# norabelrose/sparse-vae

Hardware: AMD Instinct MI355X
Metric: training tokens/sec + ELBO match vs CPU ref, 512-tok seq, 1/2/4/8 MI355X (higher is better)
Workload: dtype bf16; 1 GPU; c2: TransformerVAE 6L d512 heads 8 seq 512, batch 64/GPU, dense attention, dropout 0.1, fwd+bwd+allreduce+clip+RAdam; model=TransformerVAE-6L-d512, global_batch=64, seq_len=512, parallelism=dp1

## Files before the change

### include/svae.h

```cpp
#ifndef SVAE_H
#define SVAE_H
#include <stdint.h>
#ifdef __cplusplus
extern "C" {
#endif

typedef void* svae_stream_t;

enum svae_epi {
  SVAE_EPI_BF16 = 0,
  SVAE_EPI_F32 = 1,
  SVAE_EPI_F32_ACC = 2,
  SVAE_EPI_F32_ATOMIC = 3,
  SVAE_EPI_GELU = 4,
  SVAE_EPI_GELU_BWD = 5,
  SVAE_EPI_DROPOUT_RESID = 6,
  SVAE_EPI_ROTARY_BF16 = 7,
  SVAE_EPI_CE_STATS = 8,
  SVAE_EPI_CE_PROB = 9,
  SVAE_EPI_ROWSCALE_GATHER = 10
};

typedef struct svae_gemm_desc {
  const void* A;
  const void* B;
  int64_t lda, ldb, batch_stride_a, batch_stride_b;
  int32_t M, N, K;
  int32_t batch, splits;
  int32_t a_t, b_t;
  int32_t epi;
  void* C;
  int64_t ldc, batch_stride_c;
  const float* bias;
  const float* resid;
  int64_t ldr;
  void* aux;
  int64_t ldaux;
  float alpha;
  float drop_p;
  uint64_t seed;
  const float* rot_tab;
  int32_t rot_cols, rot_d, rot_seq;
  const int32_t* labels;
  float* label_logit;
  float* a_rowsum;
  const float* k_weight;
  const float* row_a;
  const float* row_b;
  const void* gather;
  int64_t ldg;
  float* delta;
  const float* delta_o32;
  int64_t ld_o32;
  int32_t delta_hd, delta_seq;
} svae_gemm_desc;

int svae_gemm(const svae_gemm_desc* d, svae_stream_t stream);

int svae_gemm_pair(const svae_gemm_desc* d0, const svae_gemm_desc* d1, svae_stream_t stream);

int svae_resid_ln_fwd(const float* x, const void* y, int32_t y_dtype, int64_t ldy, float drop_p, uint64_t seed,
                      const float* zrows, int32_t zmod, const float* w, const float* b, float* xo, void* h, float* mean,
                      float* rstd, int32_t rows, int32_t D, svae_stream_t stream);
int svae_layernorm_fwd(const void* x, int32_t x_dtype, const float* w, const float* b, void* y,
                       float* mean, float* rstd, int32_t rows, int32_t D, svae_stream_t stream);
int svae_layernorm_bwd(const void* dy, const void* x, int32_t x_dtype, const float* w, const float* mean,
                       const float* rstd, const float* dres, float* dx, void* dx_bf, float* part,
                       int32_t nblk, int32_t rows, int32_t D, int32_t zero_mod, svae_stream_t stream);
int svae_layernorm_bwd_drop(const void* dy, const void* x, int32_t x_dtype, const float* w, const float* mean,
                            const float* rstd, const float* dres, float* dx, void* dx_bf, float* part, int32_t nblk,
                            int32_t rows, int32_t D, int32_t zero_mod, float bf_drop_p, uint64_t bf_seed,
                            int32_t bf_zero_mod, float* zrow, void* zrow_bf, svae_stream_t stream);
int svae_layernorm_bwd_gelu(const void* dy, const void* x, int32_t x_dtype, const float* w, const float* mean,
                            const float* rstd, const void* gp, void* out_bf, float* part, int32_t nblk, int32_t rows,
                            int32_t D, svae_stream_t stream);
int svae_layernorm_fwd_z(float* x, const float* zrows, int32_t zmod, const float* w, const float* b, void* y,
                         float* mean, float* rstd, int32_t rows, int32_t D, svae_stream_t stream);
int svae_layernorm_nblk(int32_t rows);
#define SVAE_LN_MULTI_MAX 4
int svae_layernorm_fwd_multi(const float* x, const float* const* w, const float* const* b, void* const* y, int32_t n,
                             float* mean, float* rstd, int32_t rows, int32_t D, svae_stream_t stream);
int svae_layernorm_bwd_multi(const void* const* dy, const float* x, const float* const* w, const float* mean,
                             const float* rstd, const float* dres, float* dx, float* const* part, int32_t nblk,
                             int32_t n, int32_t rows, int32_t D, svae_stream_t stream);

int svae_colsum(const void* in, int32_t in_dtype, int32_t rows, int32_t cols, int64_t ld, float* out,
                int32_t accumulate, svae_stream_t stream);

#define SVAE_COLSUM_MAX 8
typedef struct svae_colsum_seg {
  const float* in;
  float* out;
  int64_t ld;
  int32_t rows, cols;
} svae_colsum_seg;
int svae_colsum_multi(const svae_colsum_seg* segs, int32_t n, svae_stream_t stream);

typedef struct svae_attn_desc {
  const void* q; const void* k; const void* v; void* o;
  int64_t sq, sk, sv, so, bq, bk, bv, bo;
  const uint8_t* key_pad;
  float* lse;
  int32_t B, H, Lq, Lk, hd, causal;
  float scale;
  const void* dout; int64_t sdo, bdo;
  float* delta;
  float* dq;
  int64_t bdq;
  void* dk; void* dv;
  int64_t sdk, sdv, bdk, bdv;
  const float* rot_tab;
  int32_t rot_d;
  float* o32;
  int64_t so32, bo32;
  float* dq_part;
  void* dq_bf;
  int64_t ldq_bf;
  int32_t window;
  int32_t delta_ready;
  void* o_lo;
  int64_t so_lo, bo_lo;
  float* fwd_ws;
  int64_t fwd_ws_elems;
} svae_attn_desc;

int svae_attn_fwd(const svae_attn_desc* d, svae_stream_t stream);
int64_t svae_attn_fwd_ws_elems(int32_t B, int32_t H, int32_t Lq, int32_t Lk, int32_t hd, int32_t causal, int32_t window);
int svae_attn_bwd(const svae_attn_desc* d, svae_stream_t stream);
int64_t svae_attn_dq_part_elems(int32_t B, int32_t H, int32_t Lq, int32_t Lk, int32_t hd);
int64_t svae_attn_dq_part_elems_w(int32_t B, int32_t H, int32_t Lq, int32_t Lk, int32_t hd, int32_t window);
int svae_dq_finalize(const float* dq, void* out, int64_t ldo, int32_t rows, int32_t D, const float* rot_tab,
                     int32_t seq, svae_stream_t stream);

int svae_embedding_fwd(const int32_t* ids, const void* table_bf, float* out, void* out_bf, int32_t rows,
                       int32_t D, svae_stream_t stream);
int svae_embedding_fwd_dual(const int32_t* ids, const void* table, float* out, float* out2, int32_t rows, int32_t D,
                            svae_stream_t stream);
int svae_embedding_bwd(const int32_t* ids, const float* dout, float* dtable, int32_t rows, int32_t D,
                       svae_stream_t stream);

int svae_reparam_kl_fwd(const float* stats, const float* eps, uint64_t seed, const int64_t* ntok,
                        float* z, void* z_bf, float* eps_out, float* raw_kl, float* kl_out, int32_t B,
                        int32_t Z, svae_stream_t stream);
int svae_reparam_kl_bwd(const float* stats, const float* eps, const float* dz, const int64_t* ntok,
                        const float* gkl, float* dstats, int32_t B, int32_t Z, svae_stream_t stream);

int svae_ce_finalize(const float* part, int32_t ntile, const float* label_logit, const int32_t* labels,
                     int32_t rows, int32_t seq, int32_t nchunks, int32_t chunk_len, float* lse, float* row_loss,
                     float* chunk_w, float* nll_out, float* red_ws, svae_stream_t stream);
int svae_ce_weighted_nll(const float* row_loss, const int32_t* labels, const float* tok_w, int32_t rows,
                         int32_t seq, int32_t nchunks, int32_t chunk_len, float* out, float* red_ws,
                         svae_stream_t stream);
int32_t svae_ce_red_ws_elems(int32_t nchunks);
int svae_ce_grad(void* logits, int64_t ld, const float* lse, const float* chunk_w, const int32_t* labels,
                 const float* gscale, float* dbias, int32_t rows, int32_t V, int32_t seq, int32_t nchunks,
                 int32_t chunk_len, svae_stream_t stream);

int svae_ce_label_logit(const void* hh, int64_t ldh, const void* W, int64_t ldw, const float* bias,
                        const int32_t* labels, int32_t rows, int32_t D, float* out, svae_stream_t stream);
int svae_ce_prob_finalize(const float* part, int32_t ntile, const float* row_off, const int32_t* labels,
                          int32_t rows, int32_t seq, int32_t nchunks, int32_t chunk_len, float* lse, float* row_loss,
                          float* chunk_w, float* nll_out, float* red_ws, svae_stream_t stream);
int svae_ce_prob_finalize_fix(const float* part, int32_t ntile, float* row_off, const int32_t* labels, int32_t rows,
                              int32_t seq, int32_t nchunks, int32_t chunk_len, float* lse, float* row_loss,
                              float* chunk_w, float* nll_out, float* red_ws, const void* hh, int64_t ldh, const void* W,
                              int64_t ldw, const float* bias, void* P, int64_t ldp, int32_t V, int32_t D,
                              int32_t* sat_ws, svae_stream_t stream);
int svae_ce_prob_bwd_prep(const void* hh, int64_t ldh, const float* lse, const float* row_off, const float* chunk_w,
                          const int32_t* labels, const float* gscale, int32_t rows, int32_t seq, int32_t nchunks,
                          int32_t chunk_len, int32_t D, void* hh_out, float* r_out, float* q_out, float* dbias,
                          svae_stream_t stream);
int svae_embedding_bwd_ce(const int32_t* ids, const float* dout, float* dtable, int32_t rows, int32_t D, int32_t seq,
                          const void* hh, const float* q, svae_stream_t stream);

int svae_dropout_bwd_cast(const float* g, void* out, float p, uint64_t seed, int64_t n, int32_t cols,
                          int64_t ld_in, svae_stream_t stream);
int svae_gelu_bwd(const float* dx, const void* gp, void* out, int64_t n, svae_stream_t stream);
int svae_prep_tokens(const int64_t* ids, const void* pad, int32_t pad_mode, int32_t B, int32_t L, int32_t* ids32,
                     int32_t* labels, void* padm, const int64_t* ntok, int64_t* ntok_out, svae_stream_t stream);
int svae_step_scalars(const float* nll, const float* kl, const float* gloss, float kl_weight, float* loss, float* gs,
                      svae_stream_t stream);
int svae_cast_bf16(const float* in, void* out, int64_t n, svae_stream_t stream);
int svae_transpose_blocks(const void* src, void* dst, const int64_t* table, int32_t nblocks, int32_t total_tiles,
                          svae_stream_t stream);
int svae_extract_rows(float* x, int64_t ld, int32_t rows, int32_t mod, int32_t D, float* out,
                      svae_stream_t stream);
int svae_zproj_bwd(const float* g, const void* z, const void* W, float* dW, float* db, float* dz, int32_t B,
                   int32_t d, int32_t Z, svae_stream_t stream);
#define SVAE_ZPROJ_MAX 32
typedef struct svae_zproj_seg {
  const float* g;
  const void* W;
  float* dW;
  float* db;
} svae_zproj_seg;
int svae_zproj_bwd_multi(const svae_zproj_seg* segs, int32_t n, const void* z, float* dz, int32_t B, int32_t d,
                         int32_t Z, svae_stream_t stream);
typedef struct svae_zproj_fwd_seg {
  const void* W;
  const float* bias;
  float* out;
} svae_zproj_fwd_seg;
int svae_zproj_fwd_multi(const svae_zproj_fwd_seg* segs, int32_t n, const void* z, int32_t B, int32_t d, int32_t Z,
                         svae_stream_t stream);

int svae_sumsq(const float* g, int64_t n, float* part, int32_t nblk, svae_stream_t stream);
int svae_radam(float* p, void* pbf, const float* g, float* m, float* v, int64_t n, const float* part,
               int32_t nblk, const float* scal, float* norm_out, svae_stream_t stream);
int svae_clip_grad(float* g, int64_t n, const float* part, int32_t nblk, float max_norm, float* norm_out,
                   svae_stream_t stream);

int svae_gemm_f32(const float* A, const float* W, float* C, int32_t M, int32_t N, int32_t K, int64_t lda, int64_t ldw,
                  int64_t ldc, const float* bias, const float* resid, int64_t ldr, int32_t epi, const float* rot_tab,
                  int32_t rot_cols, int32_t rot_d, int32_t rot_seq, svae_stream_t stream);
int svae_attn_fwd_f32(const float* q, const float* k, const float* v, float* o, int64_t sq, int64_t sk, int64_t sv,
                      int64_t so, int64_t bq, int64_t bk, int64_t bv, int64_t bo, const uint8_t* key_pad, int32_t B,
                      int32_t H, int32_t Lq, int32_t Lk, int32_t hd, int32_t causal, int32_t window, float scale,
                      svae_stream_t stream);
int svae_layernorm_fwd_f32(const float* x, const float* w, const float* b, float* y, int32_t rows, int32_t D,
                           svae_stream_t stream);

int svae_mutual_info(const float* stats, const float* eps, uint64_t seed, const float* kl, int32_t B, int32_t Z,
                     int32_t S, float* ws, float* out, svae_stream_t stream);

int svae_ce_seq_logprob(const float* part, int32_t ntile, const float* label_logit, const int32_t* labels,
                        int32_t rows, int32_t seq, float* out, svae_stream_t stream);

int svae_dec_linear(const float* X, int64_t ldx, const float* W, int64_t ldw, const float* bias, float* Y, int64_t ldy,
                    const float* resid, int64_t ldr, int32_t M, int32_t N, int32_t K, int32_t epi, const float* rot_tab,
                    int32_t rot_cols, int32_t rot_d, const int32_t* cur, float* part_ws, int64_t part_elems,
                    svae_stream_t stream);
int svae_dec_attn(const float* qkv, int64_t ldq, float* kcache, float* vcache, int32_t B, int32_t H, int32_t hd,
                  int32_t T, const int32_t* cur, int32_t window, float scale, float* O, int64_t ldo,
                  svae_stream_t stream);
int svae_dec_embed(const int64_t* out_ids, int32_t T, const int32_t* cur, const float* table, float* x, int32_t B,
                   int32_t D, svae_stream_t stream);
int svae_dec_penalty(float* logits, int64_t ldl, int32_t rows, const int32_t* row_map, const int64_t* out_ids,
                     int32_t T, const int32_t* cur, const uint8_t* live, float penalty, svae_stream_t stream);
int svae_dec_sample(const float* logits, int64_t ldl, int32_t V, int32_t rows, const int32_t* row_map,
                    int64_t* out_ids, int32_t T, const int32_t* cur, uint8_t* live, int32_t end_token,
                    float temperature, int32_t top_k, float top_p, uint64_t seed, int32_t* live_count,
                    svae_stream_t stream);
int svae_dec_advance(int32_t* cur, svae_stream_t stream);

enum svae_latent_metric { SVAE_LATENT_L2 = 0, SVAE_LATENT_COSINE = 1, SVAE_LATENT_KL = 2 };
#define SVAE_LATENT_MAX_BLOCKS 1024
int svae_latent_prepare(const float* mu, const float* scale, float* inv_var, float* logdet, float* inv_norm, int32_t N,
                        int32_t Z, svae_stream_t stream);
int svae_latent_scores(int32_t metric, const float* q_mu, const float* q_scale, const float* q_logdet,
                       const float* q_inv_norm, int32_t Q, const float* mu, const float* inv_var, const float* logdet,
                       const float* inv_norm, int32_t N, int32_t Z, float* out, svae_stream_t stream);
int64_t svae_latent_topk_ws_bytes(int32_t Q, int32_t k);
int svae_latent_topk(int32_t metric, const float* q_mu, const float* q_scale, const float* q_logdet,
                     const float* q_inv_norm, int32_t Q, const float* mu, const float* inv_var, const float* logdet,
                     const float* inv_norm, int32_t N, int32_t Z, int32_t k, void* ws, int64_t ws_bytes, float* scores,
                     int32_t* indices, svae_stream_t stream);

const char* svae_version(void);

#ifdef __cplusplus
}
#endif
#endif
```

### sparse-vae_amd/csrc/gemm.hip

```cpp
#include "common.h"
#include "../../include/svae.h"
#include <stdlib.h>
#include <algorithm>

using namespace svae;

namespace {

constexpr int BM = 128, BN = 128, BK = 64;
constexpr int TILE_BYTES = BM * BK * 2;

struct GP {
  const bf16* A; const bf16* B;
  long long lda, ldb, sA, sB;
  int M, N, K, splits, kchunk, tiles_n, tiles_m;
  void* C; long long ldc, sC;
  const float* bias;
  const float* resid; long long ldr;
  void* aux; long long ldaux;
  float alpha, drop_p;
  unsigned long long seed;
  const float* rot_tab; int rot_cols, rot_d, rot_seq;
  const int* labels; float* label_logit;
  float* a_rowsum;
  const float* k_weight;
  const float* row_a; const float* row_b;
  const bf16* gather; long long ldg;
  int epi;
  int tn2, tm2;
  int group;
  int total3;
  int relaxed;
  int dma_stagger;
  long long slab;
  float* delta; const float* delta_o32; long long ld_o32; int delta_hd, delta_seq;
};

__device__ __forceinline__ int kc_off(int row, int c) { return row * 128 + ((c ^ ((row >> 1) & 7)) << 4); }
__device__ __forceinline__ int mn_off(int k, int u) {
  const int s = (k & 3) | (((k >> 3) & 1) << 2);
  return k * 256 + ((u ^ (s << 2)) << 3);
}

template <bool TRANS>
__device__ __forceinline__ void load_tile(const bf16* __restrict__ g, long long ld, int row0, int nrows, int k0,
                                          int kend, u32x4 (&r)[4], int tid) {
  const bf16* base = TRANS ? g + (long long)k0 * ld + row0 : g + (long long)row0 * ld + k0;
  const __amdgpu_buffer_rsrc_t rsrc = __builtin_amdgcn_make_buffer_rsrc((void*)base, 0, 0x7FFFFFF0, 0x00020000);
#pragma unroll
  for (int i = 0; i < 4; ++i) {
    const int idx = tid + 256 * i;
    int row, k;
    if (!TRANS) { row = idx >> 3; k = (idx & 7) * 8; }
    else { k = idx >> 4; row = (idx & 15) * 8; }
    const bool ok = (row0 + row < nrows) && (k0 + k < kend);
    const int off = TRANS ? (k * (int)ld + row) * 2 : (row * (int)ld + k) * 2;
    r[i] = __builtin_bit_cast(u32x4, __builtin_amdgcn_raw_buffer_load_b128(rsrc, ok ? off : 0x7FFFFFF0, 0, 0));
  }
}

template <bool TRANS>
__device__ __forceinline__ void store_tile(char* lds, const u32x4 (&r)[4], int tid) {
#pragma unroll
  for (int i = 0; i < 4; ++i) {
    const int idx = tid + 256 * i;
    int off;
    if (!TRANS) off = kc_off(idx >> 3, idx & 7);
    else off = mn_off(idx >> 4, (idx & 15) * 2);
    *(u32x4*)(lds + off) = r[i];
  }
}

template <bool TRANS>
__device__ __forceinline__ bf16x8 read_frag(const char* lds, int base, int kk, int lane) {
  if (!TRANS) {
    const int row = base + (lane & 15);
    const int c = (lane >> 4) + 4 * kk;
    return *(const bf16x8*)(lds + kc_off(row, c));
  } else {
    const int q = (lane & 15) >> 2, p = lane & 3;
    const int kb = 32 * kk + 8 * (lane >> 4) + q;
    const int u = (base >> 2) + p;
    short4v lo = lds_read_tr(lds + mn_off(kb, u));
    short4v hi = lds_read_tr(lds + mn_off(kb + 4, u));
    return cat44(lo, hi);
  }
}

__device__ __forceinline__ int cs_swz(int row, int col) { return (((col >> 2) ^ (((row >> 2) & 3) << 2)) << 2) | (col & 3); }
__device__ __forceinline__ int cs_swz8(int row, int col) { return (((col >> 2) ^ (row & 7)) << 2) | (col & 3); }
template <bool SW8>
__device__ __forceinline__ int cs_at(int row, int col) { return SW8 ? cs_swz8(row, col) : cs_swz(row, col); }

__device__ __forceinline__ void group_tile(int t, int tiles_m, int tiles_n, int group, int& bm, int& bn) {
  if (group <= 1) {
    bn = t % tiles_n;
    bm = t / tiles_n;
    return;
  }
  const int per = group * tiles_n, grp = t / per, first = grp * group;
  const int gs = min(group, tiles_m - first), r = t - grp * per;
  bm = first + r % gs;
  bn = r / gs;
}

__device__ __forceinline__ void tile_coords(const GP& p, int& bm, int& bn, int& batch, int& split) {
  const int tiles = p.tiles_n * p.tiles_m;
  const int nwg = gridDim.x;
  int bid = blockIdx.x;
  if (nwg >= 16) {
    const int q = nwg / 8, r = nwg % 8, xcd = bid % 8, idx = bid / 8;
    bid = (xcd < r ? xcd * (q + 1) : r * (q + 1) + (xcd - r) * q) + idx;
  }
  const int z = bid / tiles, t = bid - z * tiles;
  group_tile(t, p.tiles_m, p.tiles_n, p.group, bm, bn);
  batch = z / p.splits;
  split = z - batch * p.splits;
}

__device__ __forceinline__ void store_bf16(bf16* dst, const f32x4& a, const f32x4& b, bool full) {
  if (full)
    *(bf16x8*)dst = (bf16x8){f2bf(a[0]), f2bf(a[1]), f2bf(a[2]), f2bf(a[3]), f2bf(b[0]), f2bf(b[1]), f2bf(b[2]), f2bf(b[3])};
  else
    *(bf16x4*)dst = (bf16x4){f2bf(a[0]), f2bf(a[1]), f2bf(a[2]), f2bf(a[3])};
}

__device__ __forceinline__ void rotary4(const GP& p, f32x4& x, int m, int n) {
  if (n >= p.rot_cols) return;
  const int pos = m % p.rot_seq;
  const int pair = (n % p.rot_d) >> 1;
  const f32x4 cs2 = *(const f32x4*)(p.rot_tab + ((long long)pos * (p.rot_d >> 1) + pair) * 2);
  const float a0 = x[0], b0 = x[1], a1 = x[2], b1 = x[3];
  x[0] = a0 * cs2[0] + (-b0) * cs2[1];
  x[1] = b0 * cs2[0] + a0 * cs2[1];
  x[2] = a1 * cs2[2] + (-b1) * cs2[3];
  x[3] = b1 * cs2[2] + a1 * cs2[3];
}

__device__ __forceinline__ void dropout4(const GP& p, f32x4& x, int m, int n) {
  const float sc = 1.0f / (1.0f - p.drop_p);
  float u[4];
  rand_uniform4(p.seed, ((unsigned long long)m * p.N + n) >> 2, u);
#pragma unroll
  for (int e = 0; e < 4; ++e) x[e] = (u[e] >= p.drop_p) ? x[e] * sc : 0.f;
}

template <int EPI, bool BIAS_DONE = false, bool SW8 = false>
__device__ __forceinline__ void epilogue_half(const GP& p, const float* cs, int m0, int n0, int bn, int rbase,
                                              long long cofs, int tid, int label_pre = -1) {
  if constexpr (EPI == SVAE_EPI_F32_ATOMIC) {
    const int col = tid & 127, n = n0 + col;
    if (n < p.N) {
      for (int it = 0; it < 32; ++it) {
        const int row = (tid >> 7) + 2 * it, m = m0 + rbase + row;
        if (m < p.M) atomicAdd((float*)p.C + cofs + (long long)m * p.ldc + n, cs[row * 128 + cs_at<SW8>(row, col)]);
      }
    }
    return;
  }
  const int cc = (tid & 15) * 8, n = n0 + cc;
  const bool ncol = n < p.N, full = n + 8 <= p.N;
  const f32x4 zero = {0.f, 0.f, 0.f, 0.f};
  f32x4 b0 = zero, b1 = zero;
  if (!BIAS_DONE && p.bias && ncol) {
    b0 = *(const f32x4*)(p.bias + n);
    if (full) b1 = *(const f32x4*)(p.bias + n + 4);
  }
  if constexpr (EPI == SVAE_EPI_CE_STATS) {
    const int row = tid >> 2, qd = tid & 3, m = m0 + rbase + row;
    float v[32];
    float mx = -INFINITY;
#pragma unroll
    for (int u = 0; u < 4; ++u) {
      const int c = 32 * u + 8 * qd;
      f32x4 x0 = *(const f32x4*)(cs + row * 128 + cs_at<SW8>(row, c));
      f32x4 x1 = *(const f32x4*)(cs + row * 128 + cs_at<SW8>(row, c + 4));
      if (!BIAS_DONE && p.bias) {
        x0 += (n0 + c < p.N) ? *(const f32x4*)(p.bias + n0 + c) : zero;
        x1 += (n0 + c + 4 < p.N) ? *(const f32x4*)(p.bias + n0 + c + 4) : zero;
      }
      if (p.C && m < p.M && n0 + c < p.N)
        store_bf16((bf16*)p.C + cofs + (long long)m * p.ldc + n0 + c, x0, x1, n0 + c + 8 <= p.N);
#pragma unroll
      for (int e = 0; e < 4; ++e) {
        const float y0 = (n0 + c + e < p.N) ? x0[e] : -INFINITY;
        const float y1 = (n0 + c + 4 + e < p.N) ? x1[e] : -INFINITY;
        v[8 * u + e] = y0;
        v[8 * u + 4 + e] = y1;
        mx = fmaxf(mx, fmaxf(y0, y1));
      }
    }
    mx = fmaxf(mx, __shfl_xor(mx, 1, 64));
    mx = fmaxf(mx, __shfl_xor(mx, 2, 64));
    float se = 0.f;
#pragma unroll
    for (int e = 0; e < 32; ++e) se += __expf(v[e] - mx);
    se += __shfl_xor(se, 1, 64);
    se += __shfl_xor(se, 2, 64);
    if (m < p.M) {
      const int lc = (BIAS_DONE ? label_pre : p.labels[m]) - n0;
      if (lc >= 0 && lc < 128 && ((lc >> 3) & 3) == qd) {
        const int idx = 8 * (lc >> 5) + (lc & 7);
#pragma unroll
        for (int e = 0; e < 32; ++e)
          if (e == idx) p.label_logit[m] = v[e];
      }
      if (qd == 0) {
        float* part = (float*)p.aux + ((long long)m * p.tiles_n + bn) * 2;
        part[0] = mx;
        part[1] = se;
      }
    }
    return;
  }
  if (!ncol) return;
#pragma unroll
  for (int it = 0; it < 4; ++it) {
    const int row = (tid >> 4) + 16 * it, m = m0 + rbase + row;
    if (m >= p.M) break;
    f32x4 x0 = *(const f32x4*)(cs + row * 128 + cs_at<SW8>(row, cc));
    f32x4 x1 = full ? *(const f32x4*)(cs + row * 128 + cs_at<SW8>(row, cc + 4)) : zero;
    const long long ci = cofs + (long long)m * p.ldc + n;
    if constexpr (EPI == SVAE_EPI_BF16) {
      store_bf16((bf16*)p.C + ci, x0 + b0, x1 + b1, full);
    } else if constexpr (EPI == SVAE_EPI_ROTARY_BF16) {
      x0 += b0;
      x1 += b1;
      rotary4(p, x0, m, n);
      if (full) rotary4(p, x1, m, n + 4);
      store_bf16((bf16*)p.C + ci, x0, x1, full);
    } else if constexpr (EPI == SVAE_EPI_F32 || EPI == SVAE_EPI_F32_ACC || EPI == SVAE_EPI_DROPOUT_RESID) {
      float* c = (float*)p.C + ci;
      if constexpr (EPI == SVAE_EPI_F32) {
        x0 += b0;
        x1 += b1;
        if (p.resid) {
          const float* r = p.resid + (long long)m * p.ldr + n;
          x0 += *(const f32x4*)r;
          if (full) x1 += *(const f32x4*)(r + 4);
        }
      } else if constexpr (EPI == SVAE_EPI_F32_ACC) {
        x0 += *(const f32x4*)c;
        if (full) x1 += *(const f32x4*)(c + 4);
      } else {
        if (p.drop_p > 0.f) {
          dropout4(p, x0, m, n);
          if (full) dropout4(p, x1, m, n + 4);
        }
        const float* r = p.resid + (long long)m * p.ldr + n;
        x0 += *(const f32x4*)r;
        if (full) x1 += *(const f32x4*)(r + 4);
      }
      *(f32x4*)c = x0;
      if (full) *(f32x4*)(c + 4) = x1;
      if constexpr (EPI == SVAE_EPI_DROPOUT_RESID) {
        if (p.aux) store_bf16((bf16*)p.aux + (long long)m * p.ldaux + n, x0, x1, full);
      } else if constexpr (EPI == SVAE_EPI_F32) {
        if (p.aux) {
          if (p.drop_p > 0.f) {
            dropout4(p, x0, m, n);
            if (full) dropout4(p, x1, m, n + 4);
          }
          store_bf16((bf16*)p.aux + (long long)m * p.ldaux + n, x0, x1, full);
        }
      }
    } else if constexpr (EPI == SVAE_EPI_GELU) {
      x0 += b0;
      x1 += b1;
      f32x4 g0, g1, d0, d1;
#pragma unroll
      for (int e = 0; e < 4; ++e) {
        float g, dg;
        gelu_pair(x0[e], g, dg);
        g0[e] = g;
        d0[e] = dg;
        gelu_pair(x1[e], g, dg);
        g1[e] = g;
        d1[e] = dg;
      }
      store_bf16((bf16*)p.C + ci, g0, g1, full);
      store_bf16((bf16*)p.aux + (long long)m * p.ldaux + n, d0, d1, full);
    } else if constexpr (EPI == SVAE_EPI_GELU_BWD) {
      const bf16* a = (const bf16*)p.aux + (long long)m * p.ldaux + n;
      bf16x8 d;
      if (full) d = *(const bf16x8*)a;
      else {
        const bf16x4 h = *(const bf16x4*)a;
        d = (bf16x8){h[0], h[1], h[2], h[3], h[0], h[1], h[2], h[3]};
      }
#pragma unroll
      for (int e = 0; e < 4; ++e) {
        x0[e] *= (float)d[e];
        x1[e] *= (float)d[e + 4];
      }
      store_bf16((bf16*)p.C + ci, x0, x1, full);
    }
  }
}

template <bool AT, bool BT, int EPI>
__global__ __launch_bounds__(256, 2) void gemm_kernel(GP p) {
  __shared__ __attribute__((aligned(16))) char smem[4 * TILE_BYTES];
  const int tid = threadIdx.x, lane = tid & 63, wave = tid >> 6;
  const int wm = wave >> 1, wn = wave & 1;

  int bm, bn, batch, split;
// ... 477 lines not shown
      se = sum_x16_x32(se);
      if (g == 0) {
        sstat[(rl * 4 + wc) * 2] = mx;
        sstat[(rl * 4 + wc) * 2 + 1] = se;
      }
      const int lc = slabel[rl] - (n0 + wc * 64);
      if (m < p.M && lc >= 0 && lc < 64 && ((lc >> 2) & 3) == g) {
        float x = 0.f;
#pragma unroll
        for (int j = 0; j < 4; ++j)
#pragma unroll
          for (int e = 0; e < 4; ++e)
            if (j == (lc >> 4) && e == (lc & 3)) x = v[j][e];
        p.label_logit[m] = x;
      }
    }
  }
  if constexpr (EPI == SVAE_EPI_CE_STATS) {
    asm volatile("s_waitcnt lgkmcnt(0)" ::: "memory");
    __builtin_amdgcn_s_barrier();
    const int row = tid >> 1, hf = tid & 1, m = m0 + row;
    if (m < p.M && n0 + 128 * hf < p.N) {
      const float* s = sstat + (row * 4 + 2 * hf) * 2;
      const float m1 = s[0], s1 = s[1], m2 = s[2], s2 = s[3];
      const float mm = fmaxf(m1, m2);
      const float e1 = m1 == -INFINITY ? 0.f : __builtin_amdgcn_exp2f((m1 - mm) * G3_LOG2E);
      const float e2 = m2 == -INFINITY ? 0.f : __builtin_amdgcn_exp2f((m2 - mm) * G3_LOG2E);
      float* part = (float*)p.aux + ((long long)m * p.tiles_n + bn * 2 + hf) * 2;
      part[0] = mm;
      part[1] = s1 * e1 + s2 * e2;
    }
  }
  if constexpr (EPI == SVAE_EPI_CE_PROB) {
    asm volatile("s_waitcnt lgkmcnt(0)" ::: "memory");
    __builtin_amdgcn_s_barrier();
    const int row = tid & 255, hf = tid >> 8, m = m0 + row;
    if (m < p.M && n0 + 128 * hf < p.N)
      ((float*)p.aux)[(long long)(bn * 2 + hf) * p.M + m] = sstat[row * 4 + 2 * hf] + sstat[row * 4 + 2 * hf + 1];
  }
}

__device__ __forceinline__ void g3_rowscale_gather_epilogue(const GP& p, const f32x4 (&acc)[8][4], const int* slabel,
                                                            const float* sra, const float* srb, int m0, int n0, int wr,
                                                            int wc, int lane) {
  const int g = lane >> 4, li = lane & 15;
  const int nb = n0 + wc * 64;
  const int cs = ((g & 1) ? 16 : 0) + ((g & 2) ? 8 : 0);
  auto ld_row = [&](int i, u32x4 (&r)[2]) {
    const int rl = wr * 128 + i * 16 + li, m = m0 + rl, lab = slabel[rl];
    const bool on = m < p.M && lab != 0 && srb[rl] != 0.f;
#pragma unroll
    for (int jp = 0; jp < 2; ++jp) {
      const int n = nb + 32 * jp + cs;
      r[jp] = (on && n + 8 <= p.N) ? *(const u32x4*)(p.gather + (long long)lab * p.ldg + n) : (u32x4){0u, 0u, 0u, 0u};
    }
  };
  u32x4 cur[2], nxt[2];
  ld_row(0, cur);
#pragma unroll
  for (int i = 0; i < 8; ++i) {
    if (i + 1 < 8) ld_row(i + 1, nxt);
    const int rl = wr * 128 + i * 16 + li, m = m0 + rl;
    const float ra = sra[rl] * p.alpha, rb = srb[rl];
#pragma unroll
    for (int jp = 0; jp < 2; ++jp) {
      const f32x4 x = acc[i][2 * jp], y = acc[i][2 * jp + 1];
      float w[8];
#pragma unroll
      for (int e = 0; e < 4; ++e) {
        const auto sw = __builtin_amdgcn_permlane16_swap(__float_as_uint(x[e]), __float_as_uint(y[e]), false, false);
        w[e] = __uint_as_float(sw[0]);
        w[4 + e] = __uint_as_float(sw[1]);
      }
      const bf16x8 gv = __builtin_bit_cast(bf16x8, cur[jp]);
      const u32x4 o = {pack_bf16x2(ra * w[0] - rb * (float)gv[0], ra * w[1] - rb * (float)gv[1]),
                       pack_bf16x2(ra * w[2] - rb * (float)gv[2], ra * w[3] - rb * (float)gv[3]),
                       pack_bf16x2(ra * w[4] - rb * (float)gv[4], ra * w[5] - rb * (float)gv[5]),
                       pack_bf16x2(ra * w[6] - rb * (float)gv[6], ra * w[7] - rb * (float)gv[7])};
      const int n = nb + 32 * jp + cs;
      if (m < p.M && n + 8 <= p.N) *(u32x4*)((bf16*)p.C + (long long)m * p.ldc + n) = o;
      else if (m < p.M && n < p.N) *(u32x2*)((bf16*)p.C + (long long)m * p.ldc + n) = (u32x2){o[0], o[1]};
    }
    if (i + 1 < 8) {
      cur[0] = nxt[0];
      cur[1] = nxt[1];
    }
  }
}

template <int EPI>
__device__ __forceinline__ void g3_reg_epilogue_ld(const GP& p, const f32x4 (&acc)[8][4], const float* sbias, int m0,
                                                   int n0, int batch, int split, int wr, int wc, int lane) {
  const long long cofs = (long long)batch * p.sC + split * p.slab;
  const int g = lane >> 4, li = lane & 15;
  const int nb = n0 + wc * 64;
  f32x4 b4[4];
#pragma unroll
  for (int j = 0; j < 4; ++j) b4[j] = *(const f32x4*)(sbias + wc * 64 + j * 16 + 4 * g);
  if constexpr (EPI == G3_EPI_BF16_DELTA) {
    const int H = p.N / p.delta_hd;
    const int hA = nb / p.delta_hd;
    auto ld_row = [&](int i, f32x4 (&r)[4]) {
      const int m = m0 + wr * 128 + i * 16 + li;
#pragma unroll
      for (int j = 0; j < 4; ++j) {
        const int n = nb + j * 16 + 4 * g;
        r[j] = (m < p.M && n < p.N) ? *(const f32x4*)(p.delta_o32 + (long long)m * p.ld_o32 + n)
                                    : (f32x4){0.f, 0.f, 0.f, 0.f};
      }
    };
    f32x4 cur[4], nxt[4];
    ld_row(0, cur);
#pragma unroll
    for (int i = 0; i < 8; ++i) {
      if (i + 1 < 8) ld_row(i + 1, nxt);
      const int m = m0 + wr * 128 + i * 16 + li;
      f32x4 x[4];
      float sA = 0.f, sB = 0.f;
#pragma unroll
      for (int j = 0; j < 4; ++j) {
        x[j] = p.alpha * acc[i][j] + b4[j];
        float dj = 0.f;
#pragma unroll
        for (int e = 0; e < 4; ++e) dj = fmaf((float)f2bf(x[j][e]), cur[j][e], dj);
        if ((nb + 16 * j) / p.delta_hd == hA) sA += dj;
        else sB += dj;
      }
      store_rows_bf16<false>((bf16*)p.C + cofs, p.ldc, m0 + wr * 128 + i * 16, p.M, nb, p.N, x, g, li);
      sA = sum_x16_x32(sA);
      sB = sum_x16_x32(sB);
      if (g == 0 && m < p.M && nb < p.N) {
        const int b = m / p.delta_seq, q = m - b * p.delta_seq;
        atomicAdd(p.delta + ((long long)b * H + hA) * p.delta_seq + q, sA);
        if ((nb + 63) / p.delta_hd != hA && hA + 1 < H) atomicAdd(p.delta + ((long long)b * H + hA + 1) * p.delta_seq + q, sB);
      }
      if (i + 1 < 8) {
#pragma unroll
        for (int j = 0; j < 4; ++j) cur[j] = nxt[j];
      }
    }
    return;
  } else if constexpr (EPI == SVAE_EPI_GELU_BWD) {
    const int cs = ((g & 1) ? 16 : 0) + ((g & 2) ? 8 : 0);
    auto ld_row = [&](int i, u32x4 (&r)[2]) {
      const int m = m0 + wr * 128 + i * 16 + li;
#pragma unroll
      for (int jp = 0; jp < 2; ++jp) {
        const int n = nb + 32 * jp + cs;
        r[jp] = (m < p.M && n + 8 <= p.N) ? *(const u32x4*)((const bf16*)p.aux + (long long)m * p.ldaux + n)
                                          : (u32x4){0u, 0u, 0u, 0u};
      }
    };
    u32x4 cur[2], nxt[2];
    ld_row(0, cur);
#pragma unroll
    for (int i = 0; i < 8; ++i) {
      if (i + 1 < 8) ld_row(i + 1, nxt);
      u32x4 o[2];
#pragma unroll
      for (int jp = 0; jp < 2; ++jp) {
        const f32x4 x = p.alpha * acc[i][2 * jp] + b4[2 * jp], y = p.alpha * acc[i][2 * jp + 1] + b4[2 * jp + 1];
        float w[8];
#pragma unroll
        for (int e = 0; e < 4; ++e) {
          const auto s = __builtin_amdgcn_permlane16_swap(__float_as_uint(x[e]), __float_as_uint(y[e]), false, false);
          w[e] = __uint_as_float(s[0]);
          w[4 + e] = __uint_as_float(s[1]);
        }
        const bf16x8 a = __builtin_bit_cast(bf16x8, cur[jp]);
        o[jp] = (u32x4){pack_bf16x2(w[0] * (float)a[0], w[1] * (float)a[1]), pack_bf16x2(w[2] * (float)a[2], w[3] * (float)a[3]),
                        pack_bf16x2(w[4] * (float)a[4], w[5] * (float)a[5]), pack_bf16x2(w[6] * (float)a[6], w[7] * (float)a[7])};
      }
      store_rows_w16<false>((bf16*)p.C + cofs, p.ldc, m0 + wr * 128 + i * 16, p.M, nb, p.N, o, g, li);
      if (i + 1 < 8) {
        cur[0] = nxt[0];
        cur[1] = nxt[1];
      }
    }
    return;
  } else {
    const float* src = EPI == SVAE_EPI_F32_ACC ? (const float*)p.C + cofs : p.resid;
    const long long lds_ = EPI == SVAE_EPI_F32_ACC ? p.ldc : p.ldr;
    const bool ld = EPI != G3_EPI_SLAB && src != nullptr;
    auto ld_row = [&](int i, f32x4 (&r)[4]) {
      const int m = m0 + wr * 128 + i * 16 + li;
#pragma unroll
      for (int j = 0; j < 4; ++j) {
        const int n = nb + j * 16 + 4 * g;
        r[j] = (ld && m < p.M && n < p.N) ? *(const f32x4*)(src + (long long)m * lds_ + n) : (f32x4){0.f, 0.f, 0.f, 0.f};
      }
    };
    f32x4 cur[4], nxt[4];
    if constexpr (EPI != G3_EPI_SLAB) ld_row(0, cur);
#pragma unroll
    for (int i = 0; i < 8; ++i) {
      if (EPI != G3_EPI_SLAB && i + 1 < 8) ld_row(i + 1, nxt);
      const int m = m0 + wr * 128 + i * 16 + li;
      f32x4 x[4];
#pragma unroll
      for (int j = 0; j < 4; ++j) {
        const int n = nb + j * 16 + 4 * g;
        x[j] = p.alpha * acc[i][j] + b4[j];
        if constexpr (EPI == SVAE_EPI_DROPOUT_RESID) {
          if (p.drop_p > 0.f) dropout4(p, x[j], m, n);
        }
        if constexpr (EPI != G3_EPI_SLAB) x[j] += cur[j];
      }
      if constexpr (EPI == SVAE_EPI_F32_ACC) {
#pragma unroll
        for (int j = 0; j < 4; ++j) {
          const int n = nb + j * 16 + 4 * g;
          if (m < p.M && n < p.N) *(f32x4*)((float*)p.C + cofs + (long long)m * p.ldc + n) = x[j];
        }
      } else {
        store_rows_f32((float*)p.C + cofs, p.ldc, m0 + wr * 128 + i * 16, p.M, nb, p.N, x, g, li);
        if constexpr (EPI == SVAE_EPI_DROPOUT_RESID) {
          if (p.aux) store_rows_bf16<false>((bf16*)p.aux, p.ldaux, m0 + wr * 128 + i * 16, p.M, nb, p.N, x, g, li);
        } else if constexpr (EPI == SVAE_EPI_F32) {
          if (p.aux) {
            if (p.drop_p > 0.f) {
#pragma unroll
              for (int j = 0; j < 4; ++j) dropout4(p, x[j], m, nb + j * 16 + 4 * g);
            }
            store_rows_bf16<false>((bf16*)p.aux, p.ldaux, m0 + wr * 128 + i * 16, p.M, nb, p.N, x, g, li);
          }
        }
      }
      if (EPI != G3_EPI_SLAB && i + 1 < 8) {
#pragma unroll
        for (int j = 0; j < 4; ++j) cur[j] = nxt[j];
      }
    }
  }
}

struct G3Tile {
  int m0, n0, bn, batch, split, kbeg, kend, nk;
  const bf16* A; const bf16* B;
};

__device__ __forceinline__ G3Tile g3_tile(const GP& p, int t3) {
  G3Tile T;
  const int tiles = p.tn2 * p.tm2;
  const int z = t3 / tiles, t = t3 - z * tiles;
  T.batch = z / p.splits;
  T.split = z - T.batch * p.splits;
  int bm, bn;
  group_tile(t, p.tm2, p.tn2, p.group, bm, bn);
  T.bn = bn;
  T.m0 = bm * 256;
  T.n0 = bn * 256;
  T.kbeg = T.split * p.kchunk;
  T.kend = min(p.K, T.kbeg + p.kchunk);
  T.nk = T.kend > T.kbeg ? (T.kend - T.kbeg + 63) / 64 : 0;
  T.A = p.A + T.batch * p.sA;
  T.B = p.B + T.batch * p.sB;
  return T;
}

constexpr int G3_EPI_STORES = 16;

#ifdef SVAE_STAMPS
__device__ unsigned long long svae_stamps[8][96][3];
__device__ unsigned long long svae_rt[1024][2];
#define G3_STAMP(k) \
  do { if (blockIdx.x < 8 && tid == 0 && ntile < 96) svae_stamps[blockIdx.x][ntile][k] = __builtin_amdgcn_s_memtime(); } while (0)
#else
#define G3_STAMP(k) ((void)0)
#endif
#ifndef SVAE_KW_FORM
#define SVAE_KW_FORM 0
#endif
#ifndef SVAE_KW_PRE
#define SVAE_KW_PRE 1
#endif

template <int EPI>
constexpr int g3_epi_vmem_ops() {
  switch (EPI) {
    case SVAE_EPI_BF16:
    case G3_EPI_BF16_DELTA:
    case SVAE_EPI_ROTARY_BF16:
    case SVAE_EPI_CE_STATS:
    case SVAE_EPI_ROWSCALE_GATHER:
    case SVAE_EPI_GELU_BWD:
      return 8 * 2;
    case SVAE_EPI_CE_PROB:
      return 8 * 2 + 1;
    case SVAE_EPI_GELU:
      return 8 * 2 * 2;
    case SVAE_EPI_F32:
    case SVAE_EPI_F32_ACC:
    case SVAE_EPI_DROPOUT_RESID:
    case G3_EPI_ACC_KW:
    case G3_EPI_F32_KW:
    case G3_EPI_SLAB:
      return 8 * 4;
    default:
      return 0;
  }
}

template <bool AT, bool BT, int EPI>
__device__ __forceinline__ void gemm256_run(const GP& p, int blk, int nwg) {
  static_assert(g3_epi_vmem_ops<EPI>() >= G3_EPI_STORES, "the relaxed first wait would not cover the prefetch DMA");
  constexpr bool IS_KW = EPI == G3_EPI_ACC_KW || EPI == G3_EPI_F32_KW;
  constexpr int KW_FORM = IS_KW ? SVAE_KW_FORM : 0;
  constexpr int KW_SLOT = KW_FORM == 2 ? 1024 : 256;
  constexpr int KW_BYTES = KW_FORM ? 2 * 8 * KW_SLOT : 0;
  constexpr int RING_OFF = KW_FORM == 3 ? KW_BYTES : 0;
  constexpr int KW_OFF = KW_FORM == 3 ? 0 : 2 * G3_STAGE + 2048 + 8192;
  __shared__ __attribute__((aligned(16))) char smem[2 * G3_STAGE + 2048 + 8192 + KW_BYTES];
  char* ring = smem + RING_OFF;
  float* sbias = (float*)(ring + 2 * G3_STAGE);
  int* slabel = (int*)(ring + 2 * G3_STAGE + 1024);
  float* sstat = (float*)(ring + 2 * G3_STAGE + 2048);
  const int tid = threadIdx.x, lane = tid & 63;
  const int wave = __builtin_amdgcn_readfirstlane(tid >> 6);
  const int wr = wave >> 2, wc = wave & 3;
  int bid = blk;
  if (nwg >= 16) {
    const int q = nwg / 8, r = nwg % 8, xcd = bid % 8, idx = bid / 8;
    bid = (xcd < r ? xcd * (q + 1) : r * (q + 1) + (xcd - r) * q) + idx;
  }
  int t3 = bid;
  if (t3 >= p.total3) return;
  G3Tile T = g3_tile(p, t3);
  char* skw = smem + KW_OFF;
  auto kw_issue = [&](int k0, int kend, int stage) {
    if constexpr (KW_FORM == 1 || KW_FORM == 3) {
      const u32x4 kwr = buffer_rsrc(p.k_weight, 0x7FFFFFF0u);
      const int kk = k0 + lane_id_fresh();
      dma4_lds(kwr, skw + (stage * 8 + wave) * KW_SLOT, kk < kend ? kk * 4 : 0x7FFFFFF0);
    } else if constexpr (KW_FORM == 2) {
      const u32x4 kwr = buffer_rsrc(p.k_weight, 0x7FFFFFF0u);
      const int l = lane_id_fresh(), kk = k0 + 4 * l;
      dma16_lds(kwr, skw + (stage * 8 + wave) * KW_SLOT, l < 16 && kk < kend ? kk * 4 : 0x7FFFFFF0);
    }
  };
  const G3Src sa = g3_src<AT>(p.lda, wave, lane), sb = g3_src<BT>(p.ldb, wave, lane);
  int g = 0;
  if (T.nk > 0) {
    g3_issue<AT, BT>(p, T.A, T.B, sa, sb, T.m0, T.n0, T.kbeg, T.kend, ring, wave);
    kw_issue(T.kbeg, T.kend, 0);
  }

  bool relaxed = false;
  int ntile = 0;
  (void)ntile;
  while (true) {
    G3_STAMP(0);
    const int t3n = t3 + nwg;
    const bool has_next = t3n < p.total3;
    float rsum[4] = {0.f, 0.f, 0.f, 0.f};
    f32x4 acc[8][4];
#pragma unroll
    for (int i = 0; i < 8; ++i)
#pragma unroll
      for (int j = 0; j < 4; ++j) acc[i][j] = (f32x4){0.f, 0.f, 0.f, 0.f};

    const bool next_dma = has_next && g3_tile(p, t3n).nk > 0;
    for (int kt = 0; kt < T.nk; ++kt, ++g) {
      if (kt == 0 && relaxed) asm volatile("s_waitcnt vmcnt(%0)" ::"n"(G3_EPI_STORES) : "memory");
      else asm volatile("s_waitcnt vmcnt(0)" ::: "memory");
      __builtin_amdgcn_s_barrier();
      const char* la = ring + (g & 1) * G3_STAGE;
      const char* lb = la + G3_T;
      char* nxt = ring + ((g + 1) & 1) * G3_STAGE;
      const bool do_rs = AT && p.a_rowsum && T.bn < 2;
      const int ks0 = p.tn2 >= 2 ? T.bn : 0, ks1 = p.tn2 >= 2 ? T.bn + 1 : 2;
      const bool kw_pre = IS_KW && KW_FORM == 0 && SVAE_KW_PRE && do_rs;
      float kw1 = 0.f;
      if (kw_pre) {
        const int kk = T.kbeg + kt * 64 + lane_id_fresh();
        const int off = kk < T.kend ? kk * 4 : 0x7FFFFFF0;
        const u32x4 kwr = buffer_rsrc(p.k_weight, 0x7FFFFFF0u);
        asm volatile("s_nop 4\n\tbuffer_load_dword %0, %1, %2, 0 offen" : "=&v"(kw1) : "v"(off), "s"(kwr) : "memory");
      }
      const bool late = (!IS_KW || KW_FORM > 0 || kw_pre) && p.dma_stagger && wr == 1 && kt + 1 < T.nk;
      if (kt + 1 < T.nk) {
        if (!late) g3_issue<AT, BT>(p, T.A, T.B, sa, sb, T.m0, T.n0, T.kbeg + (kt + 1) * 64, T.kend, nxt, wave);
        kw_issue(T.kbeg + (kt + 1) * 64, T.kend, (g + 1) & 1);
      } else if (next_dma) {
        const G3Tile TN = g3_tile(p, t3n);
        g3_issue<AT, BT>(p, TN.A, TN.B, sa, sb, TN.m0, TN.n0, TN.kbeg, TN.kend, nxt, wave);
        kw_issue(TN.kbeg, TN.kend, (g + 1) & 1);
      } else if (kw_pre) {
        const u32x4 rs = buffer_rsrc(p.A, 0x7FFFFFF0u);
#pragma unroll
        for (int i = 0; i < 8; ++i) dma16_lds(rs, nxt + (wave * 8 + i) * 1024, 0x7FFFFFF0);
      }
      bf16x8 a0[4][2], a1[4][2], b0[2][2], b1[2][2];
      auto rowsum2 = [&](const bf16x8 (&x)[2], const bf16x8 (&y)[2]) {
#pragma unroll
        for (int ks = 0; ks < 2; ++ks) {
          if (ks < ks0 || ks >= ks1) continue;
          f32x4 k0 = {1.f, 1.f, 1.f, 1.f}, k1 = k0;
          if constexpr (KW_FORM > 0) {
            const float* kws = (const float*)(skw + ((g & 1) * 8 + wave) * KW_SLOT) + 32 * ks + 8 * (lane >> 4);
            k0 = *(const f32x4*)kws;
            k1 = *(const f32x4*)(kws + 4);
          } else if constexpr (IS_KW) {
            if (kw_pre) {
              const int src0 = (32 * ks + 8 * (lane_id_fresh() >> 4)) * 4;
#pragma unroll
              for (int e = 0; e < 4; ++e) {
                k0[e] = __builtin_bit_cast(float, __builtin_amdgcn_ds_bpermute(src0 + 4 * e, __builtin_bit_cast(int, kw1)));
                k1[e] = __builtin_bit_cast(float, __builtin_amdgcn_ds_bpermute(src0 + 16 + 4 * e, __builtin_bit_cast(int, kw1)));
              }
            } else {
              const int kk = T.kbeg + kt * 64 + 32 * ks + 8 * (lane_id_fresh() >> 4);
              const int off = kk < T.kend ? kk * 4 : 0x7FFFFFF0;
              const u32x4 kwr = buffer_rsrc(p.k_weight, 0x7FFFFFF0u);
              asm volatile("s_nop 4\n\tbuffer_load_dwordx4 %0, %2, %3, 0 offen\n\t"
                           "buffer_load_dwordx4 %1, %2, %3, 0 offen offset:16\n\ts_waitcnt vmcnt(0)"
                           : "=&v"(k0), "=&v"(k1) : "v"(off), "s"(kwr) : "memory");
            }
          }
#pragma unroll
          for (int e = 0; e < 8; ++e) {
            const float kwe = e < 4 ? k0[e] : k1[e - 4];
            rsum[0] = fmaf((float)x[ks][e], kwe, rsum[0]);
            rsum[1] = fmaf((float)y[ks][e], kwe, rsum[1]);
          }
        }
      };
#pragma unroll
      for (int i = 0; i < 4; ++i)
#pragma unroll
        for (int ks = 0; ks < 2; ++ks) a0[i][ks] = g3_afrag<AT>(la, wr * 128 + i * 16, ks, lane);
#pragma unroll
      for (int j = 0; j < 2; ++j)
#pragma unroll
        for (int ks = 0; ks < 2; ++ks) b0[j][ks] = g3_bfrag<BT>(lb, wc * 64 + j * 16, ks, lane);
#pragma unroll
      for (int j = 0; j < 2; ++j)
#pragma unroll
        for (int ks = 0; ks < 2; ++ks) b1[j][ks] = g3_bfrag<BT>(lb, wc * 64 + 32 + j * 16, ks, lane);
#pragma unroll
      for (int ks = 0; ks < 2; ++ks)
#pragma unroll
        for (int i = 0; i < 4; ++i)
#pragma unroll
          for (int j = 0; j < 2; ++j) acc[i][j] = mfma16(b0[j][ks], a0[i][ks], acc[i][j]);
      if (late) {
        __builtin_amdgcn_sched_barrier(0);
        g3_issue<AT, BT>(p, T.A, T.B, sa, sb, T.m0, T.n0, T.kbeg + (kt + 1) * 64, T.kend, nxt, wave);
        __builtin_amdgcn_sched_barrier(0);
      }
      if constexpr (!AT) {
#pragma unroll
        for (int i = 0; i < 4; ++i)
#pragma unroll
          for (int ks = 0; ks < 2; ++ks) a1[i][ks] = g3_afrag<AT>(la, wr * 128 + 64 + i * 16, ks, lane);
      }
#pragma unroll
      for (int ks = 0; ks < 2; ++ks)
#pragma unroll
        for (int i = 0; i < 4; ++i)
#pragma unroll
          for (int j = 0; j < 2; ++j) acc[i][2 + j] = mfma16(b1[j][ks], a0[i][ks], acc[i][2 + j]);
      if constexpr (AT) {
        if (kw_pre) asm volatile("s_waitcnt vmcnt(8)" : "+v"(kw1) :: "memory");
        if (do_rs) {
          if (wc == 0) rowsum2(a0[0], a0[1]);
          else if (wc == 1) rowsum2(a0[2], a0[3]);
        }
#pragma unroll
        for (int i = 0; i < 4; ++i)
#pragma unroll
          for (int ks = 0; ks < 2; ++ks) a1[i][ks] = g3_afrag<AT>(la, wr * 128 + 64 + i * 16, ks, lane);
      }
#pragma unroll
      for (int ks = 0; ks < 2; ++ks)
#pragma unroll
        for (int i = 0; i < 4; ++i)
#pragma unroll
          for (int j = 0; j < 2; ++j) acc[4 + i][2 + j] = mfma16(b1[j][ks], a1[i][ks], acc[4 + i][2 + j]);
#pragma unroll
      for (int ks = 0; ks < 2; ++ks)
#pragma unroll
        for (int i = 0; i < 4; ++i)
#pragma unroll
          for (int j = 0; j < 2; ++j) acc[4 + i][j] = mfma16(b0[j][ks], a1[i][ks], acc[4 + i][j]);
      if constexpr (AT) {
        if (do_rs) {
          if (wc == 2) rowsum2(a1[0], a1[1]);
          else if (wc == 3) rowsum2(a1[2], a1[3]);
        }
      }
    }
    G3_STAMP(1);
    if (tid < 256) {
      const int n = T.n0 + tid, m = T.m0 + tid;
      sbias[tid] = (p.bias && n < p.N) ? p.bias[n] : 0.f;
      if (EPI == SVAE_EPI_CE_STATS || EPI == SVAE_EPI_CE_PROB || EPI == SVAE_EPI_ROWSCALE_GATHER)
        slabel[tid] = m < p.M ? p.labels[m] : 0;
      if (EPI == SVAE_EPI_CE_PROB) sstat[1024 + tid] = (m < p.M && p.labels[m] != 0) ? p.row_a[m] : INFINITY;
      if (EPI == SVAE_EPI_ROWSCALE_GATHER) sstat[1024 + tid] = m < p.M ? p.row_a[m] : 0.f;
      if (EPI == SVAE_EPI_ROWSCALE_GATHER) sstat[1280 + tid] = m < p.M ? p.row_b[m] : 0.f;
    }
    asm volatile("s_waitcnt lgkmcnt(0)" ::: "memory");
    __builtin_amdgcn_s_barrier();
    if constexpr (AT) {
      if (p.a_rowsum && T.bn < 2) {
#pragma unroll
        for (int h = 0; h < 2; ++h) {
          const float t = sum_x16_x32(rsum[h]);
          const int m = T.m0 + wr * 128 + (2 * wc + h) * 16 + (lane & 15);
          if ((lane >> 4) == 0 && m < p.M) atomicAdd(p.a_rowsum + m, t);
        }
      }
    }
    if constexpr (EPI == SVAE_EPI_BF16 || EPI == SVAE_EPI_GELU || EPI == SVAE_EPI_CE_STATS ||
                  EPI == SVAE_EPI_ROTARY_BF16 || EPI == SVAE_EPI_CE_PROB)
      g3_reg_epilogue<EPI>(p, acc, sbias, slabel, sstat, T.m0, T.n0, T.bn, T.batch, T.split, wr, wc, tid, lane);
    else if constexpr (EPI == SVAE_EPI_ROWSCALE_GATHER)
      g3_rowscale_gather_epilogue(p, acc, slabel, sstat + 1024, sstat + 1280, T.m0, T.n0, wr, wc, lane);
    else if constexpr (EPI == SVAE_EPI_F32 || EPI == SVAE_EPI_F32_ACC || EPI == SVAE_EPI_DROPOUT_RESID ||
                       EPI == SVAE_EPI_GELU_BWD || EPI == G3_EPI_BF16_DELTA)
      g3_reg_epilogue_ld<EPI>(p, acc, sbias, T.m0, T.n0, T.batch, T.split, wr, wc, lane);
    else if constexpr (EPI == G3_EPI_ACC_KW)
      g3_reg_epilogue_ld<SVAE_EPI_F32_ACC>(p, acc, sbias, T.m0, T.n0, T.batch, T.split, wr, wc, lane);
    else if constexpr (EPI == G3_EPI_F32_KW || EPI == G3_EPI_SLAB)
      g3_reg_epilogue_ld<G3_EPI_SLAB>(p, acc, sbias, T.m0, T.n0, T.batch, T.split, wr, wc, lane);
    else
      static_assert(EPI == G3_EPI_SLAB, "no gemm256 epilogue for this EPI");
    relaxed = p.relaxed && T.m0 + 256 <= p.M && T.n0 + 256 <= p.N;
    G3_STAMP(2);
    ++ntile;
    if (!has_next) break;
    const bool prefetched = T.nk > 0;
    t3 = t3n;
    T = g3_tile(p, t3);
    if (!prefetched && T.nk > 0) {
      g3_issue<AT, BT>(p, T.A, T.B, sa, sb, T.m0, T.n0, T.kbeg, T.kend, ring + (g & 1) * G3_STAGE, wave);
      kw_issue(T.kbeg, T.kend, g & 1);
    }
  }
}

template <bool AT, bool BT, int EPI>
__global__ __launch_bounds__(512, 1) void gemm256_kernel(GP p) {
#ifdef SVAE_STAMPS
  if (threadIdx.x == 0 && blockIdx.x < 1024) svae_rt[blockIdx.x][0] = __builtin_amdgcn_s_memrealtime();
#endif
  gemm256_run<AT, BT, EPI>(p, blockIdx.x, gridDim.x);
#ifdef SVAE_STAMPS
  if (threadIdx.x == 0 && blockIdx.x < 1024) svae_rt[blockIdx.x][1] = __builtin_amdgcn_s_memrealtime();
#endif
}

struct GP2 {
  GP p[2];
  int nb0;
};

template <bool AT, bool BT, int EPI>
__global__ __launch_bounds__(512, 1) void gemm256_pair_kernel(GP2 q) {
  const int b = blockIdx.x;
  const int sel = b < q.nb0 ? 0 : 1;
  gemm256_run<AT, BT, EPI>(q.p[sel], sel ? b - q.nb0 : b, sel ? (int)gridDim.x - q.nb0 : q.nb0);
}

constexpr int SK_BN = 32, SK_WAVES = 16;

template <int EPI>
__global__ __launch_bounds__(1024) void gemm_skinny_kernel(GP p) {
  __shared__ __attribute__((aligned(16))) float red[SK_WAVES][64][SK_BN + 4];
  const int tid = threadIdx.x, lane = tid & 63, li = lane & 15, g = lane >> 4;
  const int wave = __builtin_amdgcn_readfirstlane(tid >> 6);
  const int n0 = blockIdx.x * SK_BN;
  const int nks = (p.K + 31) / 32;
  const int per = (nks + SK_WAVES - 1) / SK_WAVES;
  const int ks0 = wave * per, ks1 = min(nks, ks0 + per);
  f32x4 acc[4][2];
#pragma unroll
  for (int i = 0; i < 4; ++i) acc[i][0] = acc[i][1] = (f32x4){0.f, 0.f, 0.f, 0.f};
  auto load = [&](int ks, bf16x8 (&a)[4], bf16x8 (&b)[2]) {
    const int k = ks * 32 + 8 * g;
    const bool kok = k < p.K;
#pragma unroll
    for (int i = 0; i < 4; ++i) {
      const int m = 16 * i + li;
      u32x4 v = {0u, 0u, 0u, 0u};
      if (kok && m < p.M) v = *(const u32x4*)(p.A + (long long)m * p.lda + k);
      a[i] = __builtin_bit_cast(bf16x8, v);
    }
#pragma unroll
    for (int jj = 0; jj < 2; ++jj) {
      const int n = n0 + 16 * jj + li;
      u32x4 v = {0u, 0u, 0u, 0u};
      if (kok && n < p.N) v = *(const u32x4*)(p.B + (long long)n * p.ldb + k);
      b[jj] = __builtin_bit_cast(bf16x8, v);
    }
  };
  if (ks0 < ks1) {
    bf16x8 a[4], b[2], an[4], bn[2];
    load(ks0, a, b);
    for (int ks = ks0; ks < ks1; ++ks) {
      if (ks + 1 < ks1) load(ks + 1, an, bn);
#pragma unroll
      for (int i = 0; i < 4; ++i)
#pragma unroll
        for (int jj = 0; jj < 2; ++jj) acc[i][jj] = mfma16(b[jj], a[i], acc[i][jj]);
      if (ks + 1 < ks1) {
#pragma unroll
        for (int i = 0; i < 4; ++i) a[i] = an[i];
        b[0] = bn[0];
        b[1] = bn[1];
      }
    }
  }
#pragma unroll
  for (int i = 0; i < 4; ++i)
#pragma unroll
    for (int jj = 0; jj < 2; ++jj) *(f32x4*)&red[wave][16 * i + li][16 * jj + 4 * g] = acc[i][jj];
  __syncthreads();
  const int row = tid >> 3, c4 = (tid & 7) * 4, m = row, n = n0 + c4;
  if (tid >= 512 || m >= p.M || n >= p.N) return;
  f32x4 x = *(const f32x4*)&red[0][row][c4];
#pragma unroll
  for (int w = 1; w < SK_WAVES; ++w) x += *(const f32x4*)&red[w][row][c4];
  x *= p.alpha;
  if (p.bias) x += *(const f32x4*)(p.bias + n);
  if constexpr (EPI == SVAE_EPI_F32 || EPI == SVAE_EPI_DROPOUT_RESID) {
    if constexpr (EPI == SVAE_EPI_DROPOUT_RESID) {
      if (p.drop_p > 0.f) dropout4(p, x, m, n);
    }
    if (p.resid) x += *(const f32x4*)(p.resid + (long long)m * p.ldr + n);
    *(f32x4*)((float*)p.C + (long long)m * p.ldc + n) = x;
    if (p.aux) {
      if (EPI == SVAE_EPI_F32 && p.drop_p > 0.f) dropout4(p, x, m, n);
      *(bf16x4*)((bf16*)p.aux + (long long)m * p.ldaux + n) = (bf16x4){f2bf(x[0]), f2bf(x[1]), f2bf(x[2]), f2bf(x[3])};
    }
  } else if constexpr (EPI == SVAE_EPI_GELU) {
    f32x2 g0, d0, g1, d1;
    gelu_pair2((f32x2){x[0], x[1]}, g0, d0);
    gelu_pair2((f32x2){x[2], x[3]}, g1, d1);
    *(bf16x4*)((bf16*)p.C + (long long)m * p.ldc + n) = (bf16x4){f2bf(g0[0]), f2bf(g0[1]), f2bf(g1[0]), f2bf(g1[1])};
    *(bf16x4*)((bf16*)p.aux + (long long)m * p.ldaux + n) = (bf16x4){f2bf(d0[0]), f2bf(d0[1]), f2bf(d1[0]), f2bf(d1[1])};
  } else if constexpr (EPI == SVAE_EPI_GELU_BWD) {
    const bf16x4 a4 = *(const bf16x4*)((const bf16*)p.aux + (long long)m * p.ldaux + n);
    *(bf16x4*)((bf16*)p.C + (long long)m * p.ldc + n) =
        (bf16x4){f2bf(x[0] * (float)a4[0]), f2bf(x[1] * (float)a4[1]), f2bf(x[2] * (float)a4[2]), f2bf(x[3] * (float)a4[3])};
  } else {
    *(bf16x4*)((bf16*)p.C + (long long)m * p.ldc + n) = (bf16x4){f2bf(x[0]), f2bf(x[1]), f2bf(x[2]), f2bf(x[3])};
  }
}

struct SlabRed {
  const float* slab;
  float* C;
  int M, N;
  long long ldc;
  int splits;
};
__device__ __forceinline__ void slab_reduce_range(const SlabRed& r, int blk, int nblk) {
  const int N4 = r.N / 4;
  const long long total = (long long)r.M * N4, plane = (long long)r.M * r.N;
  for (long long i = (long long)blk * 256 + threadIdx.x; i < total; i += (long long)nblk * 256) {
    const long long m = i / N4;
    const int n = (int)(i - m * N4) * 4;
    const float* src = r.slab + m * r.N + n;
    f32x4 acc = *(const f32x4*)src;
    for (int s = 1; s < r.splits; ++s) acc += *(const f32x4*)(src + s * plane);
    f32x4* dst = (f32x4*)(r.C + m * r.ldc + n);
    *dst = *dst + acc;
  }
}
__global__ __launch_bounds__(256) void slab_reduce_kernel(SlabRed r) { slab_reduce_range(r, blockIdx.x, gridDim.x); }
__global__ __launch_bounds__(256) void slab_reduce2_kernel(SlabRed r0, SlabRed r1, int nb0) {
  if ((int)blockIdx.x < nb0) slab_reduce_range(r0, blockIdx.x, nb0);
  else slab_reduce_range(r1, blockIdx.x - nb0, (int)gridDim.x - nb0);
}

}

static SlabRed slab_red(const svae_gemm_desc* d) {
  return SlabRed{(const float*)d->aux, (float*)d->C, d->M, d->N, (long long)d->ldc, d->splits};
}
static long long slab_blocks(const svae_gemm_desc* d) {
  return std::min(4096LL, ((long long)d->M * (d->N / 4) + 255) / 256);
}
static int launch_slab_reduce(const svae_gemm_desc* d, hipStream_t s) {
  hipLaunchKernelGGL(slab_reduce_kernel, dim3((unsigned)slab_blocks(d)), dim3(256), 0, s, slab_red(d));
  SVAE_LAUNCH_CHECK();
  return SVAE_OK;
}

static int validate_desc(const svae_gemm_desc* d) {
  if (!d || !d->A || !d->B || (!d->C && d->epi != SVAE_EPI_CE_STATS)) return SVAE_EINVAL;
  const bool epi_new = d->epi == SVAE_EPI_CE_PROB || d->epi == SVAE_EPI_ROWSCALE_GATHER;
  if (d->M <= 0 || d->N <= 0 || d->K <= 0 || d->batch <= 0 || d->splits <= 0) return SVAE_EINVAL;
  if ((d->K % 8 && !(d->a_t && d->b_t)) || d->lda % 8 || d->ldb % 8) return SVAE_EINVAL;
  if (d->a_t && d->M % 8) return SVAE_EINVAL;
  if (d->b_t && d->N % 8) return SVAE_EINVAL;
  if (((uintptr_t)d->A | (uintptr_t)d->B) & 15) return SVAE_EINVAL;
  if (d->batch_stride_a % 8 || d->batch_stride_b % 8) return SVAE_EINVAL;
  if (d->epi < 0 || d->epi > SVAE_EPI_ROWSCALE_GATHER) return SVAE_EINVAL;
  if (epi_new && (d->a_t || d->splits != 1 || d->batch != 1 || !d->labels || !d->row_a)) return SVAE_EINVAL;
  if (d->epi == SVAE_EPI_CE_PROB && !d->aux) return SVAE_EINVAL;
  if (d->epi == SVAE_EPI_ROWSCALE_GATHER && (!d->row_b || !d->gather || d->ldg % 8 || ((uintptr_t)d->gather & 15)))
    return SVAE_EINVAL;
  if (d->k_weight && (!d->a_rowsum || !d->a_t || (d->splits != 1 && !(d->epi == SVAE_EPI_F32_ATOMIC && d->aux))))
    return SVAE_EINVAL;
  if (d->epi == SVAE_EPI_ROTARY_BF16 && (!d->rot_tab || d->rot_d <= 0 || d->rot_seq <= 0)) return SVAE_EINVAL;
  if ((d->epi == SVAE_EPI_GELU || d->epi == SVAE_EPI_GELU_BWD || d->epi == SVAE_EPI_CE_STATS) && !d->aux)
    return SVAE_EINVAL;
  if (d->epi == SVAE_EPI_DROPOUT_RESID && !d->resid) return SVAE_EINVAL;
  if ((d->epi == SVAE_EPI_DROPOUT_RESID || d->epi == SVAE_EPI_F32) && d->aux &&
      (d->batch != 1 || d->ldaux % 8 || ((uintptr_t)d->aux & 15)))
    return SVAE_EINVAL;
  if (d->epi == SVAE_EPI_CE_STATS && (!d->labels || !d->label_logit || d->splits != 1)) return SVAE_EINVAL;
  if (d->splits > 1 && d->epi != SVAE_EPI_F32_ATOMIC) return SVAE_EINVAL;
  if (d->a_rowsum && !d->a_t) return SVAE_EINVAL;
  if (d->N % 4 || d->ldc % 8 || ((uintptr_t)d->C & 15) || (d->resid && (d->ldr % 4 || ((uintptr_t)d->resid & 15))))
    return SVAE_EINVAL;
  if ((d->epi == SVAE_EPI_GELU || d->epi == SVAE_EPI_GELU_BWD) && (d->ldaux % 8 || ((uintptr_t)d->aux & 15)))
    return SVAE_EINVAL;
  if (d->epi == SVAE_EPI_ROTARY_BF16 && (d->rot_d % 4 || d->rot_cols % 4)) return SVAE_EINVAL;

  return SVAE_OK;
}

static void fill_gp(const svae_gemm_desc* d, GP& p) {
  p.A = (const bf16*)d->A; p.B = (const bf16*)d->B;
  p.lda = d->lda; p.ldb = d->ldb; p.sA = d->batch_stride_a; p.sB = d->batch_stride_b;
  p.M = d->M; p.N = d->N; p.K = d->K; p.splits = d->splits;
  int kchunk = (d->K + d->splits - 1) / d->splits;
  kchunk = (kchunk + BK - 1) / BK * BK;
  p.kchunk = kchunk;
  p.tiles_n = (d->N + BN - 1) / BN;
  p.tiles_m = (d->M + BM - 1) / BM;
  p.C = d->C; p.ldc = d->ldc; p.sC = d->batch_stride_c;
  p.bias = d->bias; p.resid = d->resid; p.ldr = d->ldr;
  p.aux = d->aux; p.ldaux = d->ldaux;
  p.alpha = d->alpha; p.drop_p = d->drop_p; p.seed = d->seed;
  p.rot_tab = d->rot_tab; p.rot_cols = d->rot_cols; p.rot_d = d->rot_d; p.rot_seq = d->rot_seq;
  p.labels = d->labels; p.label_logit = d->label_logit;
  p.a_rowsum = d->a_rowsum;
  p.k_weight = d->k_weight;
  p.row_a = d->row_a; p.row_b = d->row_b;
  p.gather = (const bf16*)d->gather; p.ldg = d->ldg;
  p.epi = d->epi;
  p.slab = 0;
  p.dma_stagger = 0;
  p.delta = d->delta; p.delta_o32 = d->delta_o32; p.ld_o32 = d->ld_o32;
  p.delta_hd = d->delta_hd; p.delta_seq = d->delta_seq;
}

__global__ __launch_bounds__(256) void gemm_delta_kernel(const bf16* __restrict__ C, long long ldc,
                                                         const float* __restrict__ o32, long long ldo, int M, int H,
                                                         int hd, int seq, float* __restrict__ delta) {
  const int gw = blockIdx.x * 4 + (threadIdx.x >> 6), lane = threadIdx.x & 63;
  if (gw >= M * H) return;
  const int m = gw / H, h = gw - m * H;
  float s = 0.f;
  for (int c = lane * 4; c < hd; c += 256) {
    const bf16x4 a = *(const bf16x4*)(C + (long long)m * ldc + h * hd + c);
    const f32x4 o = *(const f32x4*)(o32 + (long long)m * ldo + h * hd + c);
#pragma unroll
    for (int e = 0; e < 4; ++e) s = fmaf((float)a[e], o[e], s);
  }
  s = wave_sum(s);
  const int b = m / seq, q = m - b * seq;
  if (lane == 0) delta[((long long)b * H + h) * seq + q] = s;
}

static int gemm_run(const svae_gemm_desc* d, svae_stream_t stream, bool* fused_delta);

SVAE_EXPORT int svae_gemm(const svae_gemm_desc* d, svae_stream_t stream) {
  if (!d || !d->delta) return gemm_run(d, stream, nullptr);
  if (d->epi != SVAE_EPI_BF16 || d->splits != 1 || d->batch != 1 || d->a_t || !d->delta_o32 || !d->C ||
      d->delta_hd <= 0 || d->delta_hd % 16 || d->N % d->delta_hd || d->delta_seq <= 0 || d->M % d->delta_seq ||
      d->ld_o32 < d->N || d->ld_o32 % 4 || ((uintptr_t)d->delta_o32 & 15) || ((uintptr_t)d->C & 7))
    return SVAE_EINVAL;
  bool fused = false;
  if (const int rc = gemm_run(d, stream, &fused)) return rc;
  if (!fused) {
    const int H = d->N / d->delta_hd;
    hipLaunchKernelGGL(gemm_delta_kernel, dim3((unsigned)(((long long)d->M * H + 3) / 4)), dim3(256), 0,
                       (hipStream_t)stream, (const bf16*)d->C, (long long)d->ldc, d->delta_o32, (long long)d->ld_o32,
                       d->M, H, d->delta_hd, d->delta_seq, d->delta);
    SVAE_LAUNCH_CHECK();
  }
  return SVAE_OK;
}

static int gemm_run(const svae_gemm_desc* d, svae_stream_t stream, bool* fused_delta) {
  if (const int rc = validate_desc(d)) return rc;
  const bool epi_new = d->epi == SVAE_EPI_CE_PROB || d->epi == SVAE_EPI_ROWSCALE_GATHER;
  GP p;
  fill_gp(d, p);
  const bool slab = d->epi == SVAE_EPI_F32_ATOMIC && d->splits > 1 && d->aux;
  int epi_run = d->epi;
  if (slab) {
    if (d->batch != 1 || ((uintptr_t)d->aux & 15) || d->N % 4) return SVAE_EINVAL;
    p.C = d->aux; p.ldc = d->N; p.sC = 0; p.slab = (long long)d->M * d->N;
    p.bias = nullptr; p.resid = nullptr; p.aux = nullptr;
    epi_run = SVAE_EPI_F32;
  }

  const long long nblocks = (long long)p.tiles_n * p.tiles_m * d->batch * d->splits;
  if (nblocks > 0x7FFFFFFF) return SVAE_EINVAL;
  dim3 grid((unsigned)nblocks);
  hipStream_t s = (hipStream_t)stream;
  static const int skinny_env = [] { const char* e = getenv("SVAE_GEMM_SKINNY"); return e ? atoi(e) : 1; }();
  if (skinny_env && d->M <= 64 && !d->a_t && !d->b_t && d->batch == 1 && d->splits == 1 && !d->a_rowsum &&
      d->C && d->K % 8 == 0 && d->lda % 8 == 0 && d->ldb % 8 == 0 && ((uintptr_t)d->A & 15) == 0 &&
      ((uintptr_t)d->B & 15) == 0 &&
      (d->epi == SVAE_EPI_BF16 || d->epi == SVAE_EPI_F32 || d->epi == SVAE_EPI_GELU || d->epi == SVAE_EPI_GELU_BWD ||
       d->epi == SVAE_EPI_DROPOUT_RESID)) {
    const dim3 gs((unsigned)((d->N + SK_BN - 1) / SK_BN));
    switch (d->epi) {
      case SVAE_EPI_BF16: hipLaunchKernelGGL(gemm_skinny_kernel<SVAE_EPI_BF16>, gs, dim3(1024), 0, s, p); break;
      case SVAE_EPI_F32: hipLaunchKernelGGL(gemm_skinny_kernel<SVAE_EPI_F32>, gs, dim3(1024), 0, s, p); break;
      case SVAE_EPI_GELU: hipLaunchKernelGGL(gemm_skinny_kernel<SVAE_EPI_GELU>, gs, dim3(1024), 0, s, p); break;
      case SVAE_EPI_GELU_BWD: hipLaunchKernelGGL(gemm_skinny_kernel<SVAE_EPI_GELU_BWD>, gs, dim3(1024), 0, s, p); break;
      default: hipLaunchKernelGGL(gemm_skinny_kernel<SVAE_EPI_DROPOUT_RESID>, gs, dim3(1024), 0, s, p); break;
    }
    SVAE_LAUNCH_CHECK();
    return SVAE_OK;
  }
  const int lay = (d->a_t ? 2 : 0) | (d->b_t ? 1 : 0);
  static const int forced = [] { const char* e = getenv("SVAE_GEMM_IMPL"); return e ? atoi(e) : 0; }();
  const int kslice = (d->K + d->splits - 1) / d->splits;
  p.tn2 = (d->N + 255) / 256;
  p.tm2 = (d->M + 255) / 256;
  static const int group_env = [] { const char* e = getenv("SVAE_GEMM_GROUP"); return e ? atoi(e) : -1; }();
  p.group = group_env >= 0 ? group_env : (p.tn2 >= 32 ? 4 : 0);
  const long long blocks256 = (long long)p.tn2 * p.tm2 * d->batch * d->splits;
  const bool acc_epi = d->epi == SVAE_EPI_F32_ACC;
  const bool ok3 = !(d->a_t && !d->b_t) || acc_epi;
  int impl = forced ? forced : ((ok3 && blocks256 >= 192) ? 3 : ((kslice <= 2048 && !(d->a_t && d->b_t)) ? 2 : 1));
  if (epi_new || d->k_weight || (d->a_t && !d->b_t && acc_epi && blocks256 >= 192)) impl = 3;
  if (d->k_weight) {
    if (d->epi == SVAE_EPI_F32_ACC && d->splits == 1) epi_run = G3_EPI_ACC_KW;
    else if (slab) epi_run = G3_EPI_F32_KW;
    else return SVAE_EINVAL;
  }
  if (impl == 3 && !ok3) impl = 1;
  if (impl == 3 && epi_run == SVAE_EPI_F32_ATOMIC) impl = (kslice <= 2048 && !(d->a_t && d->b_t)) ? 2 : 1;
  if (impl == 3) {
    if (slab && epi_run == SVAE_EPI_F32 && d->a_t && d->b_t) epi_run = G3_EPI_SLAB;
    int kc3 = (d->K + d->splits - 1) / d->splits;
    p.kchunk = (kc3 + 63) / 64 * 64;
    static const int persist_env = [] { const char* e = getenv("SVAE_GEMM_PERSIST"); return e ? atoi(e) : 1; }();
    static const int ncu = [] {
      int dev = 0, n = 0;
      if (hipGetDevice(&dev) != hipSuccess || hipDeviceGetAttribute(&n, hipDeviceAttributeMultiprocessorCount, dev) != hipSuccess)
        n = 256;
      return n > 0 ? n : 256;
    }();
    p.total3 = (int)blocks256;
    const long long nb3 = persist_env ? std::min<long long>(blocks256, ncu) : blocks256;
    static const int relax_env = [] { const char* e = getenv("SVAE_GEMM_RELAX"); return e ? atoi(e) : 1; }();
    p.relaxed = relax_env && !(d->epi == SVAE_EPI_CE_STATS && !d->C);
    static const int stagger_env = [] { const char* e = getenv("SVAE_GEMM_STAGGER"); return e ? atoi(e) : 1; }();
    p.dma_stagger = stagger_env;
    dim3 grid3((unsigned)nb3);
    if (fused_delta && epi_run == SVAE_EPI_BF16 && d->delta_hd >= 64) {
      const long long n = (long long)d->M * (d->N / d->delta_hd);
      if (hipMemsetAsync(d->delta, 0, n * sizeof(float), s) != hipSuccess) return SVAE_ELAUNCH;
      epi_run = G3_EPI_BF16_DELTA;
      *fused_delta = true;
    }
#define SVAE_GEMM3_CASE(E)                                                                                   \
  case E:                                                                                                    \
    if (d->a_t && !d->b_t) {                                                                                 \
      if constexpr (E == SVAE_EPI_F32_ACC) hipLaunchKernelGGL((gemm256_kernel<true, false, E>), grid3, dim3(512), 0, s, p); \
      else return SVAE_EINVAL;                                                                               \
    } else if (d->a_t) hipLaunchKernelGGL((gemm256_kernel<true, true, E>), grid3, dim3(512), 0, s, p);       \
    else if (d->b_t) hipLaunchKernelGGL((gemm256_kernel<false, true, E>), grid3, dim3(512), 0, s, p);        \
    else hipLaunchKernelGGL((gemm256_kernel<false, false, E>), grid3, dim3(512), 0, s, p);                   \
    break;
    switch (epi_run) {
      SVAE_GEMM3_CASE(SVAE_EPI_BF16)
      SVAE_GEMM3_CASE(SVAE_EPI_F32)
      SVAE_GEMM3_CASE(SVAE_EPI_F32_ACC)
      SVAE_GEMM3_CASE(SVAE_EPI_GELU)
      SVAE_GEMM3_CASE(SVAE_EPI_GELU_BWD)
      SVAE_GEMM3_CASE(SVAE_EPI_DROPOUT_RESID)
      SVAE_GEMM3_CASE(SVAE_EPI_ROTARY_BF16)
      SVAE_GEMM3_CASE(SVAE_EPI_CE_STATS)
      case G3_EPI_ACC_KW:
        if (d->b_t) hipLaunchKernelGGL((gemm256_kernel<true, true, G3_EPI_ACC_KW>), grid3, dim3(512), 0, s, p);
        else hipLaunchKernelGGL((gemm256_kernel<true, false, G3_EPI_ACC_KW>), grid3, dim3(512), 0, s, p);
        break;
      case G3_EPI_SLAB:
        hipLaunchKernelGGL((gemm256_kernel<true, true, G3_EPI_SLAB>), grid3, dim3(512), 0, s, p);
        break;
      case G3_EPI_F32_KW:
        if (!d->b_t) return SVAE_EINVAL;
        hipLaunchKernelGGL((gemm256_kernel<true, true, G3_EPI_F32_KW>), grid3, dim3(512), 0, s, p);
        break;
      case SVAE_EPI_CE_PROB:
        hipLaunchKernelGGL((gemm256_kernel<false, false, SVAE_EPI_CE_PROB>), grid3, dim3(512), 0, s, p);
        break;
      case G3_EPI_BF16_DELTA:
        if (d->b_t) hipLaunchKernelGGL((gemm256_kernel<false, true, G3_EPI_BF16_DELTA>), grid3, dim3(512), 0, s, p);
        else hipLaunchKernelGGL((gemm256_kernel<false, false, G3_EPI_BF16_DELTA>), grid3, dim3(512), 0, s, p);
        break;
      case SVAE_EPI_ROWSCALE_GATHER:
        if (d->b_t) hipLaunchKernelGGL((gemm256_kernel<false, true, SVAE_EPI_ROWSCALE_GATHER>), grid3, dim3(512), 0, s, p);
        else hipLaunchKernelGGL((gemm256_kernel<false, false, SVAE_EPI_ROWSCALE_GATHER>), grid3, dim3(512), 0, s, p);
        break;
      default: return SVAE_EINVAL;
    }
#undef SVAE_GEMM3_CASE
    SVAE_LAUNCH_CHECK();
    return slab ? launch_slab_reduce(d, s) : SVAE_OK;
  }
  if (impl == 2) {
    int kchunk2 = (d->K + d->splits - 1) / d->splits;
    p.kchunk = (kchunk2 + BK2 - 1) / BK2 * BK2;
#define SVAE_GEMM2_CASE(E)                                                                             \
  case E:                                                                                              \
    if (lay == 0) hipLaunchKernelGGL((gemm_glds_kernel<false, false, E>), grid, dim3(256), 0, s, p);    \
    else if (lay == 1) hipLaunchKernelGGL((gemm_glds_kernel<false, true, E>), grid, dim3(256), 0, s, p); \
    else if (lay == 2) hipLaunchKernelGGL((gemm_glds_kernel<true, false, E>), grid, dim3(256), 0, s, p); \
    else hipLaunchKernelGGL((gemm_glds_kernel<true, true, E>), grid, dim3(256), 0, s, p);                \
    break;
    switch (epi_run) {
      SVAE_GEMM2_CASE(SVAE_EPI_BF16)
      SVAE_GEMM2_CASE(SVAE_EPI_F32)
      SVAE_GEMM2_CASE(SVAE_EPI_F32_ACC)
      SVAE_GEMM2_CASE(SVAE_EPI_F32_ATOMIC)
      SVAE_GEMM2_CASE(SVAE_EPI_GELU)
      SVAE_GEMM2_CASE(SVAE_EPI_GELU_BWD)
      SVAE_GEMM2_CASE(SVAE_EPI_DROPOUT_RESID)
      SVAE_GEMM2_CASE(SVAE_EPI_ROTARY_BF16)
      SVAE_GEMM2_CASE(SVAE_EPI_CE_STATS)
      default: return SVAE_EINVAL;
    }
#undef SVAE_GEMM2_CASE
    SVAE_LAUNCH_CHECK();
    return slab ? launch_slab_reduce(d, s) : SVAE_OK;
  }
#define SVAE_GEMM_CASE(E)                                                                             \
  case E:                                                                                             \
    if (lay == 0) hipLaunchKernelGGL((gemm_kernel<false, false, E>), grid, dim3(256), 0, s, p);        \
    else if (lay == 1) hipLaunchKernelGGL((gemm_kernel<false, true, E>), grid, dim3(256), 0, s, p);    \
    else if (lay == 2) hipLaunchKernelGGL((gemm_kernel<true, false, E>), grid, dim3(256), 0, s, p);    \
    else hipLaunchKernelGGL((gemm_kernel<true, true, E>), grid, dim3(256), 0, s, p);                   \
    break;
  switch (epi_run) {
    SVAE_GEMM_CASE(SVAE_EPI_BF16)
    SVAE_GEMM_CASE(SVAE_EPI_F32)
    SVAE_GEMM_CASE(SVAE_EPI_F32_ACC)
    SVAE_GEMM_CASE(SVAE_EPI_F32_ATOMIC)
    SVAE_GEMM_CASE(SVAE_EPI_GELU)
    SVAE_GEMM_CASE(SVAE_EPI_GELU_BWD)
    SVAE_GEMM_CASE(SVAE_EPI_DROPOUT_RESID)
    SVAE_GEMM_CASE(SVAE_EPI_ROTARY_BF16)
    SVAE_GEMM_CASE(SVAE_EPI_CE_STATS)
    default: return SVAE_EINVAL;
  }
#undef SVAE_GEMM_CASE
  SVAE_LAUNCH_CHECK();
  return slab ? launch_slab_reduce(d, s) : SVAE_OK;
}

SVAE_EXPORT int svae_gemm_pair(const svae_gemm_desc* d0, const svae_gemm_desc* d1, svae_stream_t stream) {
  const svae_gemm_desc* d[2] = {d0, d1};
  GP2 q;
  long long nb[2];
  for (int i = 0; i < 2; ++i) {
    if (const int rc = validate_desc(d[i])) return rc;
    if (!d[i]->a_t || !d[i]->b_t || d[i]->epi != SVAE_EPI_F32_ATOMIC || d[i]->splits < 2 || !d[i]->aux ||
        d[i]->batch != 1 || d[i]->k_weight || ((uintptr_t)d[i]->aux & 15))
      return SVAE_EINVAL;
    GP& p = q.p[i];
    fill_gp(d[i], p);
    p.C = d[i]->aux; p.ldc = d[i]->N; p.sC = 0; p.slab = (long long)d[i]->M * d[i]->N;
    p.bias = nullptr; p.resid = nullptr; p.aux = nullptr;
    const int kc3 = (d[i]->K + d[i]->splits - 1) / d[i]->splits;
    p.kchunk = (kc3 + 63) / 64 * 64;
    p.tn2 = (d[i]->N + 255) / 256;
    p.tm2 = (d[i]->M + 255) / 256;
    p.group = 0;
    nb[i] = (long long)p.tn2 * p.tm2 * d[i]->splits;
    if (nb[i] > (1 << 24)) return SVAE_EINVAL;
    p.total3 = (int)nb[i];
    p.relaxed = 1;
  }
  q.nb0 = (int)((nb[0] + 7) / 8 * 8);
  hipStream_t s = (hipStream_t)stream;
  hipLaunchKernelGGL((gemm256_pair_kernel<true, true, G3_EPI_SLAB>), dim3((unsigned)(q.nb0 + nb[1])), dim3(512), 0, s,
                     q);
  SVAE_LAUNCH_CHECK();
  static const int two_env = [] { const char* e = getenv("SVAE_SLAB2"); return e ? atoi(e) : 1; }();
  if (!two_env) {
    if (const int rc = launch_slab_reduce(d0, s)) return rc;
    return launch_slab_reduce(d1, s);
  }
  const long long b0 = slab_blocks(d0), b1 = slab_blocks(d1);
  hipLaunchKernelGGL(slab_reduce2_kernel, dim3((unsigned)(b0 + b1)), dim3(256), 0, s, slab_red(d0), slab_red(d1), (int)b0);
  SVAE_LAUNCH_CHECK();
  return SVAE_OK;
}

#ifdef SVAE_STAMPS
extern "C" __attribute__((visibility("default"))) int svae_debug_stamps(unsigned long long* host) {
  return hipMemcpyFromSymbol(host, HIP_SYMBOL(svae_stamps), sizeof(svae_stamps)) == hipSuccess ? 0 : -1;
}
extern "C" __attribute__((visibility("default"))) int svae_debug_rt(unsigned long long* host) {
  return hipMemcpyFromSymbol(host, HIP_SYMBOL(svae_rt), sizeof(svae_rt)) == hipSuccess ? 0 : -1;
}
extern "C" __attribute__((visibility("default"))) int svae_debug_stamps_clear() {
  static unsigned long long zeros[8 * 96 * 3];
  return hipMemcpyToSymbol(HIP_SYMBOL(svae_stamps), zeros, sizeof(zeros)) == hipSuccess ? 0 : -1;
}
#endif
```

### sparse-vae_amd/sparse_vae/_native.py

```python
import ctypes
import os

import torch

_HERE = os.path.dirname(os.path.abspath(__file__))
LIB_PATH = os.environ.get('SVAE_LIB') or os.path.join(_HERE, 'libsvae.so')

c_void_p, c_int32, c_int64, c_float, c_uint64 = (ctypes.c_void_p, ctypes.c_int32, ctypes.c_int64,
                                                  ctypes.c_float, ctypes.c_uint64)
c_fptr = ctypes.c_void_p

EPI_BF16, EPI_F32, EPI_F32_ACC, EPI_F32_ATOMIC, EPI_GELU, EPI_GELU_BWD, EPI_DROPOUT_RESID, \
    EPI_ROTARY_BF16, EPI_CE_STATS, EPI_CE_PROB, EPI_ROWSCALE_GATHER = range(11)

LATENT_L2, LATENT_COSINE, LATENT_KL = range(3)
LATENT_METRICS = {'l2': LATENT_L2, 'cosine': LATENT_COSINE, 'kl': LATENT_KL}
LATENT_MAX_BLOCKS = 1024


class GemmDesc(ctypes.Structure):
    _fields_ = [
        ('A', c_void_p), ('B', c_void_p),
        ('lda', c_int64), ('ldb', c_int64), ('batch_stride_a', c_int64), ('batch_stride_b', c_int64),
        ('M', c_int32), ('N', c_int32), ('K', c_int32),
        ('batch', c_int32), ('splits', c_int32),
        ('a_t', c_int32), ('b_t', c_int32),
        ('epi', c_int32),
        ('C', c_void_p),
        ('ldc', c_int64), ('batch_stride_c', c_int64),
        ('bias', c_void_p), ('resid', c_void_p), ('ldr', c_int64),
        ('aux', c_void_p), ('ldaux', c_int64),
        ('alpha', c_float), ('drop_p', c_float), ('seed', c_uint64),
        ('rot_tab', c_void_p), ('rot_cols', c_int32), ('rot_d', c_int32), ('rot_seq', c_int32),
        ('labels', c_void_p), ('label_logit', c_void_p),
        ('a_rowsum', c_void_p),
        ('k_weight', c_void_p), ('row_a', c_void_p), ('row_b', c_void_p), ('gather', c_void_p), ('ldg', c_int64),
        ('delta', c_void_p), ('delta_o32', c_void_p), ('ld_o32', c_int64), ('delta_hd', c_int32), ('delta_seq', c_int32),
    ]


class AttnDesc(ctypes.Structure):
    _fields_ = [
        ('q', c_void_p), ('k', c_void_p), ('v', c_void_p), ('o', c_void_p),
        ('sq', c_int64), ('sk', c_int64), ('sv', c_int64), ('so', c_int64),
        ('bq', c_int64), ('bk', c_int64), ('bv', c_int64), ('bo', c_int64),
        ('key_pad', c_void_p), ('lse', c_void_p),
        ('B', c_int32), ('H', c_int32), ('Lq', c_int32), ('Lk', c_int32), ('hd', c_int32), ('causal', c_int32),
        ('scale', c_float),
        ('dout', c_void_p), ('sdo', c_int64), ('bdo', c_int64),
        ('delta', c_void_p), ('dq', c_void_p), ('bdq', c_int64),
        ('dk', c_void_p), ('dv', c_void_p),
        ('sdk', c_int64), ('sdv', c_int64), ('bdk', c_int64), ('bdv', c_int64),
        ('rot_tab', c_void_p), ('rot_d', c_int32),
        ('o32', c_void_p), ('so32', c_int64), ('bo32', c_int64),
        ('dq_part', c_void_p), ('dq_bf', c_void_p), ('ldq_bf', c_int64),
        ('window', c_int32),
        ('delta_ready', c_int32),
        ('o_lo', c_void_p), ('so_lo', c_int64), ('bo_lo', c_int64),
        ('fwd_ws', c_void_p), ('fwd_ws_elems', c_int64),
    ]


COLSUM_MAX = 8
LN_MULTI_MAX = 4


ZPROJ_MAX = 32


class ZprojSeg(ctypes.Structure):
    _fields_ = [('g', c_void_p), ('W', c_void_p), ('dW', c_void_p), ('db', c_void_p)]


class ZprojFwdSeg(ctypes.Structure):
    _fields_ = [('W', c_void_p), ('bias', c_void_p), ('out', c_void_p)]


class ColsumSeg(ctypes.Structure):
    _fields_ = [('inp', c_void_p), ('out', c_void_p), ('ld', c_int64), ('rows', c_int32), ('cols', c_int32)]


_SIGS = {
    'svae_gemm': [ctypes.POINTER(GemmDesc), c_void_p],
    'svae_gemm_pair': [ctypes.POINTER(GemmDesc), ctypes.POINTER(GemmDesc), c_void_p],
    'svae_resid_ln_fwd': [c_void_p, c_void_p, c_int32, c_int64, c_float, c_uint64, c_void_p, c_int32, c_void_p,
                          c_void_p, c_void_p, c_void_p, c_void_p, c_void_p, c_int32, c_int32, c_void_p],
    'svae_layernorm_fwd': [c_void_p, c_int32, c_void_p, c_void_p, c_void_p, c_void_p, c_void_p, c_int32, c_int32,
                           c_void_p],
    'svae_layernorm_bwd': [c_void_p, c_void_p, c_int32, c_void_p, c_void_p, c_void_p, c_void_p, c_void_p, c_void_p,
                           c_void_p, c_int32, c_int32, c_int32, c_int32, c_void_p],
    'svae_layernorm_bwd_drop': [c_void_p, c_void_p, c_int32, c_void_p, c_void_p, c_void_p, c_void_p, c_void_p,
                                c_void_p, c_void_p, c_int32, c_int32, c_int32, c_int32, c_float, c_uint64, c_int32,
                                c_void_p, c_void_p, c_void_p],
    'svae_layernorm_bwd_gelu': [c_void_p, c_void_p, c_int32, c_void_p, c_void_p, c_void_p, c_void_p, c_void_p,
                                c_void_p, c_int32, c_int32, c_int32, c_void_p],
    'svae_layernorm_nblk': [c_int32],
    'svae_colsum': [c_void_p, c_int32, c_int32, c_int32, c_int64, c_void_p, c_int32, c_void_p],
    'svae_colsum_multi': [c_void_p, c_int32, c_void_p],
    'svae_attn_fwd': [ctypes.POINTER(AttnDesc), c_void_p],
    'svae_attn_bwd': [ctypes.POINTER(AttnDesc), c_void_p],
    'svae_attn_dq_part_elems': [c_int32, c_int32, c_int32, c_int32, c_int32],
    'svae_attn_dq_part_elems_w': [c_int32, c_int32, c_int32, c_int32, c_int32, c_int32],
    'svae_attn_fwd_ws_elems': [c_int32, c_int32, c_int32, c_int32, c_int32, c_int32, c_int32],
    'svae_transpose_blocks': [c_void_p, c_void_p, c_void_p, c_int32, c_int32, c_void_p],
    'svae_dq_finalize': [c_void_p, c_void_p, c_int64, c_int32, c_int32, c_void_p, c_int32, c_void_p],
    'svae_embedding_fwd': [c_void_p, c_void_p, c_void_p, c_void_p, c_int32, c_int32, c_void_p],
    'svae_embedding_fwd_dual': [c_void_p, c_void_p, c_void_p, c_void_p, c_int32, c_int32, c_void_p],
    'svae_embedding_bwd': [c_void_p, c_void_p, c_void_p, c_int32, c_int32, c_void_p],
    'svae_reparam_kl_fwd': [c_void_p, c_void_p, c_uint64, c_void_p, c_void_p, c_void_p, c_void_p, c_void_p,
                            c_void_p, c_int32, c_int32, c_void_p],
    'svae_reparam_kl_bwd': [c_void_p, c_void_p, c_void_p, c_void_p, c_void_p, c_void_p, c_int32, c_int32, c_void_p],
    'svae_ce_finalize': [c_void_p, c_int32, c_void_p, c_void_p, c_int32, c_int32, c_int32, c_int32, c_void_p,
                         c_void_p, c_void_p, c_void_p, c_void_p, c_void_p],
    'svae_ce_weighted_nll': [c_void_p, c_void_p, c_void_p, c_int32, c_int32, c_int32, c_int32, c_void_p, c_void_p,
                             c_void_p],
    'svae_ce_red_ws_elems': [c_int32],
    'svae_clip_grad': [c_void_p, c_int64, c_void_p, c_int32, c_float, c_void_p, c_void_p],
    'svae_ce_label_logit': [c_void_p, c_int64, c_void_p, c_int64, c_void_p, c_void_p, c_int32, c_int32, c_void_p,
                            c_void_p],
    'svae_ce_prob_finalize': [c_void_p, c_int32, c_void_p, c_void_p, c_int32, c_int32, c_int32, c_int32, c_void_p,
                              c_void_p, c_void_p, c_void_p, c_void_p, c_void_p],
    'svae_ce_prob_finalize_fix': [c_void_p, c_int32, c_void_p, c_void_p, c_int32, c_int32, c_int32, c_int32, c_void_p,
                                  c_void_p, c_void_p, c_void_p, c_void_p, c_void_p, c_int64, c_void_p, c_int64, c_void_p,
                                  c_void_p, c_int64, c_int32, c_int32, c_void_p, c_void_p],
    'svae_ce_prob_bwd_prep': [c_void_p, c_int64, c_void_p, c_void_p, c_void_p, c_void_p, c_void_p, c_int32, c_int32,
                              c_int32, c_int32, c_int32, c_void_p, c_void_p, c_void_p, c_void_p, c_void_p],
    'svae_embedding_bwd_ce': [c_void_p, c_void_p, c_void_p, c_int32, c_int32, c_int32, c_void_p, c_void_p, c_void_p],
    'svae_ce_grad': [c_void_p, c_int64, c_void_p, c_void_p, c_void_p, c_void_p, c_void_p, c_int32, c_int32, c_int32,
                     c_int32, c_int32, c_void_p],
    'svae_dropout_bwd_cast': [c_void_p, c_void_p, c_float, c_uint64, c_int64, c_int32, c_int64, c_void_p],
    'svae_gelu_bwd': [c_void_p, c_void_p, c_void_p, c_int64, c_void_p],
    'svae_prep_tokens': [c_void_p, c_void_p, c_int32, c_int32, c_int32, c_void_p, c_void_p, c_void_p, c_void_p,
                         c_void_p, c_void_p],
    'svae_step_scalars': [c_void_p, c_void_p, c_void_p, c_float, c_void_p, c_void_p, c_void_p],
    'svae_zproj_bwd_multi': [c_void_p, c_int32, c_void_p, c_void_p, c_int32, c_int32, c_int32, c_void_p],
    'svae_zproj_fwd_multi': [c_void_p, c_int32, c_void_p, c_int32, c_int32, c_int32, c_void_p],
    'svae_layernorm_fwd_multi': [c_void_p, c_void_p, c_void_p, c_void_p, c_int32, c_void_p, c_void_p, c_int32, c_int32,
                                 c_void_p],
    'svae_layernorm_bwd_multi': [c_void_p, c_void_p, c_void_p, c_void_p, c_void_p, c_void_p, c_void_p, c_void_p,
                                 c_int32, c_int32, c_int32, c_int32, c_void_p],
    'svae_layernorm_fwd_z': [c_void_p, c_void_p, c_int32, c_void_p, c_void_p, c_void_p, c_void_p, c_void_p, c_int32,
                             c_int32, c_void_p],
    'svae_cast_bf16': [c_void_p, c_void_p, c_int64, c_void_p],
    'svae_extract_rows': [c_void_p, c_int64, c_int32, c_int32, c_int32, c_void_p, c_void_p],
    'svae_zproj_bwd': [c_void_p, c_void_p, c_void_p, c_void_p, c_void_p, c_void_p, c_int32, c_int32, c_int32, c_void_p],
    'svae_sumsq': [c_void_p, c_int64, c_void_p, c_int32, c_void_p],
    'svae_radam': [c_void_p, c_void_p, c_void_p, c_void_p, c_void_p, c_int64, c_void_p, c_int32, c_void_p,
                   c_void_p, c_void_p],
    'svae_gemm_f32': [c_void_p, c_void_p, c_void_p, c_int32, c_int32, c_int32, c_int64, c_int64, c_int64, c_void_p,
                      c_void_p, c_int64, c_int32, c_void_p, c_int32, c_int32, c_int32, c_void_p],
    'svae_attn_fwd_f32': [c_void_p, c_void_p, c_void_p, c_void_p, c_int64, c_int64, c_int64, c_int64, c_int64, c_int64,
                          c_int64, c_int64, c_void_p, c_int32, c_int32, c_int32, c_int32, c_int32, c_int32, c_int32,
                          c_float, c_void_p],
    'svae_layernorm_fwd_f32': [c_void_p, c_void_p, c_void_p, c_void_p, c_int32, c_int32, c_void_p],
    'svae_ce_seq_logprob': [c_void_p, c_int32, c_void_p, c_void_p, c_int32, c_int32, c_void_p, c_void_p],
    'svae_dec_linear': [c_void_p, c_int64, c_void_p, c_int64, c_void_p, c_void_p, c_int64, c_void_p, c_int64, c_int32,
                        c_int32, c_int32, c_int32, c_void_p, c_int32, c_int32, c_void_p, c_void_p, c_int64, c_void_p],
    'svae_dec_attn': [c_void_p, c_int64, c_void_p, c_void_p, c_int32, c_int32, c_int32, c_int32, c_void_p, c_int32,
                      c_float, c_void_p, c_int64, c_void_p],
    'svae_dec_embed': [c_void_p, c_int32, c_void_p, c_void_p, c_void_p, c_int32, c_int32, c_void_p],
    'svae_dec_penalty': [c_void_p, c_int64, c_int32, c_void_p, c_void_p, c_int32, c_void_p, c_void_p, c_float,
                         c_void_p],
    'svae_dec_sample': [c_void_p, c_int64, c_int32, c_int32, c_void_p, c_void_p, c_int32, c_void_p, c_void_p, c_int32,
                        c_float, c_int32, c_float, c_uint64, c_void_p, c_void_p],
    'svae_dec_advance': [c_void_p, c_void_p],
    'svae_mutual_info': [c_void_p, c_void_p, c_uint64, c_void_p, c_int32, c_int32, c_int32, c_void_p, c_void_p,
                         c_void_p],
    'svae_latent_prepare': [c_void_p, c_void_p, c_void_p, c_void_p, c_void_p, c_int32, c_int32, c_void_p],
    'svae_latent_scores': [c_int32, c_void_p, c_void_p, c_void_p, c_void_p, c_int32, c_void_p, c_void_p, c_void_p,
                           c_void_p, c_int32, c_int32, c_void_p, c_void_p],
    'svae_latent_topk_ws_bytes': [c_int32, c_int32],
    'svae_latent_topk': [c_int32, c_void_p, c_void_p, c_void_p, c_void_p, c_int32, c_void_p, c_void_p, c_void_p,
                         c_void_p, c_int32, c_int32, c_int32, c_void_p, c_int64, c_void_p, c_void_p, c_void_p],
    'svae_version': [],
}


def _load():
    if not os.path.exists(LIB_PATH):
        raise RuntimeError(f'libsvae.so not found at {LIB_PATH}: build it with `make -C sparse-vae_amd` '
                           f'(or __graft_entry__.build()). There is no CPU fallback.')
    lib = ctypes.CDLL(LIB_PATH)
    for name, argtypes in _SIGS.items():
        fn = getattr(lib, name)
        fn.argtypes = argtypes
        fn.restype = {'svae_version': ctypes.c_char_p, 'svae_attn_dq_part_elems': c_int64,
                      'svae_attn_dq_part_elems_w': c_int64, 'svae_attn_fwd_ws_elems': c_int64,
                      'svae_latent_topk_ws_bytes': c_int64}.get(name, ctypes.c_int)
    return lib


lib = _load()
EXPORTED = tuple(_SIGS)


def check(status, name):
    if status != 0:
        raise RuntimeError(f'{name} failed with status {status}')


def ptr(t):
    return None if t is None else t.data_ptr()


def stream():
    return torch.cuda.current_stream().cuda_stream
```

### sparse-vae_amd/sparse_vae/engine.py

```python
import math
import os
from collections import OrderedDict

import torch

from . import kernels as K
from ._native import COLSUM_MAX, LN_MULTI_MAX, ZPROJ_MAX
from ._native import EPI_BF16, EPI_F32, EPI_F32_ACC, EPI_GELU, EPI_GELU_BWD, EPI_DROPOUT_RESID, \
    EPI_ROTARY_BF16, EPI_CE_STATS, EPI_F32_ATOMIC, EPI_CE_PROB, EPI_ROWSCALE_GATHER

bf16, f32 = torch.bfloat16, torch.float32
ALIGN = 64
CE_CHUNK_NUMEL = 2 ** 30


def _attn_entries(pre, d, learned):
    out = []
    if learned:
        out.append((pre + 'learned_queries', (1, learned, d)))
        names = ['k_linear', 'v_linear']
    else:
        names = ['q_linear', 'k_linear', 'v_linear']
    out += [(pre + n + '.weight', (d, d)) for n in names]
    out += [(pre + n + '.bias', (d,)) for n in names]
    out += [(pre + 'output_linear.weight', (d, d)), (pre + 'output_linear.bias', (d,))]
    return out


def _ctx_ln_entries(pre, d):
    return [(pre + 'context_layer_norm.weight', (d,)), (pre + 'context_layer_norm.bias', (d,))]


def _layer_entries(pre, d, learned=None, cross=False, ctx_ln=True):
    out = _attn_entries(pre + 'attention.', d, learned)
    out += [(pre + 'attn_layer_norm.weight', (d,)), (pre + 'attn_layer_norm.bias', (d,))]
    if cross:
        out += _attn_entries(pre + 'cross_attention.', d, None)
        out += [(pre + 'cross_attn_layer_norm.weight', (d,)), (pre + 'cross_attn_layer_norm.bias', (d,))]
        if ctx_ln:
            out += _ctx_ln_entries(pre, d)
    out += [(pre + 'ffn.0.weight', (4 * d, d)), (pre + 'ffn.0.bias', (4 * d,)), (pre + 'ffn.2.weight', (d, 4 * d)),
            (pre + 'ffn_layer_norm.weight', (d,)), (pre + 'ffn_layer_norm.bias', (d,))]
    return out


def _pos_linear_entries(pre, d):
    return [(pre + 'pos_linear.weight', (d, d)), (pre + 'pos_linear.bias', (d,))]


def ctx_ln_batched(hp):
    return hp.enc_layers - 2 >= 2 and os.environ.get('SVAE_CTX_LN_BATCH', '1') != '0'


def layout_entries(hp):
    d, V, Z, N = hp.d_model, hp.vocab_size, hp.latent_depth, hp.num_latents
    live = [('output_layer.0.weight', (d, d)), ('output_layer.0.bias', (d,)),
            ('output_layer.2.weight', (d,)), ('output_layer.2.bias', (d,)), ('output_layer.3.bias', (V,))]
    dead = []
    for i in reversed(range(hp.num_layers)):
        live += _layer_entries(f'decoder_layers.{i}.', d)
        live += [(f'z_projections.{i}.weight', (d, Z)), (f'z_projections.{i}.bias', (d,))]
        dead += _pos_linear_entries(f'decoder_layers.{i}.attention.', d)
    live += [('q_of_z_given_x.linear.weight', (2 * Z, d)), ('q_of_z_given_x.linear.bias', (2 * Z,))]
    live += _layer_entries('encoder.bottleneck.', d, learned=1)
    dead += _pos_linear_entries('encoder.bottleneck.attention.', d)
    nmid = hp.enc_layers - 2
    batched = ctx_ln_batched(hp)
    for j in reversed(range(nmid)):
        live += _layer_entries(f'encoder.middle_layers.{j}.', d, cross=True, ctx_ln=not batched)
        dead += _pos_linear_entries(f'encoder.middle_layers.{j}.attention.', d)
        dead += _pos_linear_entries(f'encoder.middle_layers.{j}.cross_attention.', d)
    if batched:
        for j in reversed(range(nmid)):
            live += _ctx_ln_entries(f'encoder.middle_layers.{j}.', d)
    live += _layer_entries('encoder.first_layer.', d, learned=N)
    dead += _pos_linear_entries('encoder.first_layer.attention.', d)
    live += [('input_layer.0.weight', (V, d))]
    return live, dead


class FlatParams:

    def __init__(self, hp, device):
        live, dead = layout_entries(hp)
        self.ctx_batched = ctx_ln_batched(hp)
        self.offsets = OrderedDict()
        off = 0
        for name, shape in live + dead:
            n = math.prod(shape)
            self.offsets[name] = (off, shape)
            off += -(-n // ALIGN) * ALIGN
            if name == live[-1][0]:
                self.n_live = off
        self.total = off
        self.live_names = [n for n, _ in live]
        self.device = torch.device(device)
        self.master = torch.zeros(self.total, dtype=f32, device=self.device)
        self.shadow = torch.zeros(self.total, dtype=bf16, device=self.device) if self.device.type == 'cuda' else None
        self.shadow_t = torch.zeros_like(self.shadow) if self.shadow is not None else None
        self.t_blocks = OrderedDict()
        self._t_table = None
        self.grad = torch.zeros(self.total, dtype=f32, device=self.device)
        self.shadow_version = -1

    def end(self, name):
        off, shape = self.offsets[name]
        return off + -(-math.prod(shape) // ALIGN) * ALIGN

    def view(self, name, buf=None):
        off, shape = self.offsets[name]
        buf = self.master if buf is None else buf
        return buf[off:off + math.prod(shape)].view(shape)

    def w(self, name):
        return self.view(name, self.shadow)

    def f(self, name):
        return self.view(name)

    def g(self, name):
        return self.view(name, self.grad)

    def wT(self, name, rows, cols):
        key = (name, rows, cols)
        off = self.offsets[name][0]
        if key not in self.t_blocks:
            assert rows % 8 == 0 and cols % 8 == 0, key
            for o, r, c in self.t_blocks.values():
                assert off + rows * cols <= o or o + r * c <= off, f'overlapping transposed blocks at {name}'
            self.t_blocks[key] = (off, rows, cols)
            self._t_table = None
            self.refresh_transposed([key])
        return self.shadow_t[off:off + rows * cols].view(cols, rows)

    def refresh_transposed(self, keys=None):
        if not self.t_blocks:
            return
        if keys is None and self._t_table is not None:
            table, nb, tiles = self._t_table
        else:
            rows_tab, tiles = [], 0
            for k in (keys if keys is not None else self.t_blocks):
                o, r, c = self.t_blocks[k]
                rows_tab.append([o, r, c, tiles])
                tiles += -(-r // 64) * -(-c // 64)
            table = torch.tensor(rows_tab, dtype=torch.int64).to(self.device)
            nb = len(rows_tab)
            if keys is None:
                self._t_table = (table, nb, tiles)
        K.transpose_blocks(self.shadow, self.shadow_t, table, nb, tiles)

    def sync_shadow(self, force=False):
        if force or self.master._version != self.shadow_version:
            K.cast_bf16(self.master, self.shadow)
            self.refresh_transposed()
            self.shadow_version = self.master._version


class Workspace:

    def __init__(self, device):
        self.device = device
        self.bufs = {}
        self.busy = {}

    def fence(self, t):
        ev = self.busy.pop(t.untyped_storage().data_ptr(), None)
        if ev is not None:
            torch.cuda.current_stream().wait_event(ev)

    def get(self, name, shape, dtype=bf16, zero=False):
        t = self.bufs.get(name)
        if t is None or t.shape != torch.Size(shape) or t.dtype != dtype:
            t = torch.empty(shape, dtype=dtype, device=self.device)
            self.bufs[name] = t
        if self.busy:
            self.fence(t)
        if zero:
            t.zero_()
        return t


def rotary_table(positions, d, max_pos=10000):
    half = d // 2
    freqs = torch.arange(half, dtype=f32)
    pos = torch.arange(0, positions, dtype=f32)
    theta = max_pos ** (-freqs / half)
    ang = pos[:, None] * theta
    return torch.stack([ang.cos(), ang.sin()], dim=-1).contiguous()


def _mix_seed(a, b):
    x = (a * 0x9E3779B97F4A7C15 + b * 0xBF58476D1CE4E5B9 + 0x94D049BB133111EB) & 0xFFFFFFFFFFFFFFFF
    x ^= x >> 31
    return x


class VAEEngine:
    def __init__(self, hp, flat: FlatParams):
        self.hp = hp
        self.P = flat
        self.ws = Workspace(flat.device)
        self.d = hp.d_model
        self.H = hp.num_heads
        self.He = hp.d_model // 64
        assert self.d % self.H == 0 and self.d % 64 == 0
        self.hd = self.d // self.H
        self._rot = {}
        self.window = getattr(hp, 'attn_window', 0)
        self.saved = None
        self.probe = None
        self.head_mode = os.environ.get('SVAE_HEAD', 'prob')
        assert self.head_mode in ('prob', 'logits'), self.head_mode
        self.dw_pair = os.environ.get('SVAE_DW_PAIR', '1') != '0'
        self.fuse_ln = os.environ.get('SVAE_FUSE_LN', '0') != '0'
        self.delta_fused = os.environ.get('SVAE_DELTA_FUSED', '0') != '0'
        self.o32_mode = os.environ.get('SVAE_ATTN_O32', '0') != '0'
        self.resid_bf16 = os.environ.get('SVAE_RESID_BF16', '1') != '0'
        self.head_g2 = os.environ.get('SVAE_HEAD_G2', '1') != '0'
        self.ln_gelu = os.environ.get('SVAE_LN_GELU', '1') != '0'
        self.small_fused = os.environ.get('SVAE_SMALL_FUSED', '1') != '0'
        self.zp_batch = os.environ.get('SVAE_ZPROJ_BATCH', '1') != '0'
        self.zf_batch = os.environ.get('SVAE_ZPROJ_FWD_BATCH', '1') != '0'
        self._zp_pending, self._zp_ctx = [], None
        self.cs_batch = os.environ.get('SVAE_COLSUM_BATCH', '1') != '0'
        self._cs_pending = []
        self.ncu = (torch.cuda.get_device_properties(flat.device).multi_processor_count
                    if flat.device.type == 'cuda' else 256)
        self.side = None
        if flat.device.type == 'cuda' and os.environ.get('SVAE_DW_STREAM', '0') != '0':
            self.side = torch.cuda.Stream(device=flat.device)

    def rot(self, L, window=0):
        need = max(L, self.hp.num_latents)
        base = 2 * window * 32 if window else 10000
        t = self._rot.get(base)
        if t is None or t.shape[0] < need:
            t = rotary_table(max(need, 512), self.d, base).to(self.P.device)
            self._rot[base] = t
        return t

    def _ln_fwd(self, name, x, rows, tag, zsplice=None):
        D = self.d
        y = self.ws.get(tag + '.y', (rows, D))
        mean = self.ws.get(tag + '.mean', (rows,), f32)
        rstd = self.ws.get(tag + '.rstd', (rows,), f32)
        if zsplice is not None:
            K.layernorm_fwd_z(x, zsplice[0], zsplice[1], self.P.f(name + '.weight'), self.P.f(name + '.bias'), y, mean,
                              rstd, rows, D)
        else:
            K.layernorm_fwd(x, self.P.f(name + '.weight'), self.P.f(name + '.bias'), y, mean, rstd, rows, D)
        return y, (x, mean, rstd)

    def _ln_bwd(self, name, dy, st, rows, dres, dx, dx_bf=None, bf_drop=None, zsplice=None, gelu=None):
        x, mean, rstd = st
        D = self.d
        wg = self.P.grad[self.P.offsets[name + '.weight'][0]:][:2 * D]
        if not self.cs_batch:
            part = self.ws.get('ln.part', (1024 * 2 * D,), f32)
            if gelu is not None:
                K.layernorm_bwd_gelu(dy, x, self.P.f(name + '.weight'), mean, rstd, gelu, dx_bf, wg, rows, D, part)
                return
            K.layernorm_bwd(dy, x, self.P.f(name + '.weight'), mean, rstd, dres, dx, dx_bf, wg, rows, D, part,
                            bf_drop=bf_drop, zsplice=zsplice)
            return
        if len(self._cs_pending) == COLSUM_MAX:
            self.flush_colsum()
        k, n1 = len(self._cs_pending), 1024 * 2 * D
        part = self.ws.get('ln.parts', (COLSUM_MAX * n1,), f32)[k * n1:(k + 1) * n1]
        if gelu is not None:
            K.layernorm_bwd_gelu(dy, x, self.P.f(name + '.weight'), mean, rstd, gelu, dx_bf, wg, rows, D, part,
                                 defer=self._cs_pending)
            return
        K.layernorm_bwd(dy, x, self.P.f(name + '.weight'), mean, rstd, dres, dx, dx_bf, wg, rows, D, part,
                        bf_drop=bf_drop, zsplice=zsplice, defer=self._cs_pending)

    def flush_zproj(self):
        if self._zp_pending:
            z_bf, dz, B, d, Z = self._zp_ctx
            K.zproj_bwd_multi(self._zp_pending, z_bf, dz, B, d, Z)
            self._zp_pending = []

    def flush_colsum(self):
        if self._cs_pending:
            K.colsum_multi(self._cs_pending)
            self._cs_pending = []

    def _dw(self, dY, X, wname, rows, n_out, n_in, ldy=None, ldx=None, bias=None, on_side=True):
        bg = None
        if bias is not None:
            off = self.P.offsets[bias][0]
            bg = self.P.grad[off:off + n_out]
        side = self.side if on_side else None
        if side is None:
            K.linear_dw(dY, X, self.P.g(wname), rows, n_out, n_in, ldy, ldx, bgrad=bg)
            return
        side.wait_stream(torch.cuda.current_stream())
        with torch.cuda.stream(side):
            K.linear_dw(dY, X, self.P.g(wname), rows, n_out, n_in, ldy, ldx, bgrad=bg)
        ev = torch.cuda.Event()
        ev.record(side)
        self.ws.busy[dY.untyped_storage().data_ptr()] = ev

    def _head_dw_splits(self, V, d):
        env = int(os.environ.get('SVAE_HEAD_DW_SPLITS', '0') or 0)
        if env > 0:
            return env
        tiles = -(-V // 256) * -(-d // 256)
        ncu = self.ncu
        eff = lambda s: tiles * s / (ncu * -(-(tiles * s) // ncu))
        return 2 if tiles >= ncu and eff(2) > eff(1) + 0.1 else 1

    def _dw_pair(self, j0, j1):
        if self.side is not None or not self.dw_pair:
            for j in (j0, j1):
                self._dw(*j[:6], *(tuple(j[6:]) + (None,) * (9 - len(j))))
            return
        args = []
        for j in (j0, j1):
            dY, X, wname, rows, n_out, n_in = j[:6]
            ldy, ldx, bias = tuple(j[6:]) + (None,) * (9 - len(j))
            bg = None
            if bias is not None:
                off = self.P.offsets[bias][0]
                bg = self.P.grad[off:off + n_out]
            args.append((dY, X, self.P.g(wname), rows, n_out, n_in, ldy, ldx, bg))
        K.linear_dw_pair(*args)

    def join_side(self):
        if self.side is not None:
            torch.cuda.current_stream().wait_stream(self.side)
            self.ws.busy.clear()

    def _db(self, dY, bname, rows, cols, ld=None):
        off = self.P.offsets[bname][0]
        K.colsum(dY, rows, cols, ld or cols, self.P.grad[off:off + cols])

    def layer_fwd(self, pre, x, B, Sx, L, pad, *, learned=0, cross=False, causal=False, ctx=None, heads, hd,
                  drop_p=0.0, seed=0, tag, out=None, window=0, fuse=False, h_in=None, next_ln=None, out_bf=None,
                  zsplice=None, ctx_ln=None):
        d, ws, P = self.d, self.ws, self.P
        rows_x = B * Sx
        rot = self.rot(max(Sx, L), window)
        st = {'pre': pre, 'B': B, 'Sx': Sx, 'L': L, 'learned': learned, 'cross': cross, 'causal': causal,
              'heads': heads, 'hd': hd, 'drop_p': drop_p, 'seed': seed, 'x': x, 'tag': tag, 'window': window}
        a = pre + 'attention.'
        fuse = fuse and not cross
        if h_in is not None:
            h, st['ln_a'] = h_in
        else:
            h, st['ln_a'] = self._ln_fwd(pre + 'attn_layer_norm', x, rows_x, tag + '.ln_a', zsplice=zsplice)
        st['h'] = h
        pad_k = pad if Sx == L else None
        if learned:
            Lq = learned
            kv = ws.get(tag + '.kv', (rows_x, 2 * d))
            K.gemm(h, P.w(a + 'k_linear.weight'), kv, rows_x, 2 * d, d, epi=EPI_ROTARY_BF16,
                   bias=P.f(a + 'k_linear.bias'), rot=rot, rot_cols=d, rot_d=d, rot_seq=Sx)
            q = P.w(a + 'learned_queries').view(Lq, d)
            qargs = dict(sq=d, bq=0)
            kt, vt, sk = kv, kv[:, d:], 2 * d
            st['kv'] = kv
        else:
            Lq = Sx
            qkv = ws.get(tag + '.qkv', (rows_x, 3 * d))
            K.gemm(h, P.w(a + 'q_linear.weight'), qkv, rows_x, 3 * d, d, epi=EPI_ROTARY_BF16,
                   bias=P.f(a + 'q_linear.bias'), rot=rot, rot_cols=2 * d, rot_d=d, rot_seq=Sx)
            q = qkv
            qargs = dict(sq=3 * d, bq=Sx * 3 * d)
            kt, vt, sk = qkv[:, d:], qkv[:, 2 * d:], 3 * d
            st['qkv'] = qkv
        rows_q = B * Lq
        O = ws.get(tag + '.O', (rows_q, d))
        Ox = self._o_extra(tag + '.O', rows_q, d, Lq)
        lse = ws.get(tag + '.lse', (B, heads, Lq), f32)
        K.attention(q, kt, vt, O, lse, B=B, H=heads, Lq=Lq, Lk=Sx, hd=hd, so=d, bo=Lq * d, sk=sk, sv=sk,
                    bk=Sx * sk, bv=Sx * sk, key_pad=pad_k, causal=causal, window=window, **Ox, **qargs)
        st.update(O=O, Ox=Ox, lse=lse, Lq=Lq, pad_k=pad_k)
        resid = Lq == Sx
        x1 = ws.get(tag + '.x1', (rows_q, d), f32)
        if fuse:
            ya = ws.get('fuse.y', (rows_q, d), f32)
            K.gemm(O, P.w(a + 'output_linear.weight'), ya, rows_q, d, d, epi=EPI_F32, bias=P.f(a + 'output_linear.bias'))
            nm = pre + 'ffn_layer_norm'
            h2 = ws.get(tag + '.ln_f.y', (rows_q, d))
            mf, rf = ws.get(tag + '.ln_f.mean', (rows_q,), f32), ws.get(tag + '.ln_f.rstd', (rows_q,), f32)
            K.resid_ln_fwd(x if resid else None, ya, h2, rows_q, d, w=P.f(nm + '.weight'), b=P.f(nm + '.bias'), mean=mf,
                           rstd=rf, xo=x1)
            st['ln_f'] = (x1, mf, rf)
        else:
            K.gemm(O, P.w(a + 'output_linear.weight'), x1, rows_q, d, d, epi=EPI_F32,
                   bias=P.f(a + 'output_linear.bias'), resid=x if resid else None, ldr=d)
        st['resid'] = resid
        st['x1'] = x1
        xc = x1
        if cross:
            c = pre + 'cross_attention.'
            rows_c = B * L
            if ctx_ln is not None:
                cx, st['ln_ctx'] = ctx_ln
                st['ctx_deferred'] = True
            else:
                cx, st['ln_ctx'] = self._ln_fwd(pre + 'context_layer_norm', ctx, rows_c, tag + '.ln_ctx')
            hq, st['ln_cross'] = self._ln_fwd(pre + 'cross_attn_layer_norm', x1, rows_q, tag + '.ln_cross')
            qc = ws.get(tag + '.qc', (rows_q, d))
            K.gemm(hq, P.w(c + 'q_linear.weight'), qc, rows_q, d, d, epi=EPI_ROTARY_BF16, bias=P.f(c + 'q_linear.bias'),
                   rot=rot, rot_cols=d, rot_d=d, rot_seq=Lq)
            kvc = ws.get(tag + '.kvc', (rows_c, 2 * d))
            K.gemm(cx, P.w(c + 'k_linear.weight'), kvc, rows_c, 2 * d, d, epi=EPI_ROTARY_BF16,
                   bias=P.f(c + 'k_linear.bias'), rot=rot, rot_cols=d, rot_d=d, rot_seq=L)
            Oc = ws.get(tag + '.Oc', (rows_q, d))
            Ocx = self._o_extra(tag + '.Oc', rows_q, d, Lq)
            lsec = ws.get(tag + '.lsec', (B, heads, Lq), f32)
            K.attention(qc, kvc, kvc[:, d:], Oc, lsec, B=B, H=heads, Lq=Lq, Lk=L, hd=hd, sq=d, bq=Lq * d, sk=2 * d,
                        sv=2 * d, bk=L * 2 * d, bv=L * 2 * d, so=d, bo=Lq * d, key_pad=pad, causal=False, **Ocx)
            st['Ocx'] = Ocx
            x2 = ws.get(tag + '.x2', (rows_q, d), f32)
            K.gemm(Oc, P.w(c + 'output_linear.weight'), x2, rows_q, d, d, epi=EPI_F32,
                   bias=P.f(c + 'output_linear.bias'), resid=x1, ldr=d)
            st.update(cx=cx, hq=hq, qc=qc, kvc=kvc, Oc=Oc, lsec=lsec, x2=x2, pad_ctx=pad)
            xc = x2
        if not fuse:
            h2, st['ln_f'] = self._ln_fwd(pre + 'ffn_layer_norm', xc, rows_q, tag + '.ln_f')
        gprime = ws.get(tag + '.gprime', (rows_q, 4 * d))
        f = ws.get(tag + '.f', (rows_q, 4 * d))
        K.gemm(h2, P.w(pre + 'ffn.0.weight'), f, rows_q, 4 * d, d, epi=EPI_GELU, bias=P.f(pre + 'ffn.0.bias'),
               aux=gprime, ldaux=4 * d)
        if fuse:
            yf = ws.get('fuse.y', (rows_q, d), f32)
            K.gemm(f, P.w(pre + 'ffn.2.weight'), yf, rows_q, d, 4 * d, epi=EPI_F32)
            if next_ln is not None:
                nm, zrows, zmod, ntag = next_ln
                out = ws.get(tag + '.out', (rows_q, d), f32) if out is None else out
                hn = ws.get(ntag + '.ln_a.y', (rows_q, d))
                mn, rn = ws.get(ntag + '.ln_a.mean', (rows_q,), f32), ws.get(ntag + '.ln_a.rstd', (rows_q,), f32)
                K.resid_ln_fwd(xc, yf, hn, rows_q, d, w=P.f(nm + '.weight'), b=P.f(nm + '.bias'), mean=mn, rstd=rn,
                               xo=out, drop_p=drop_p, seed=seed, zrows=zrows, zmod=zmod)
                st['next_h'] = (hn, (out, mn, rn))
            else:
                assert out_bf is not None, 'the last fused layer writes the bf16 copy of its output'
                K.resid_ln_fwd(xc, yf, out_bf, rows_q, d, xo=out, drop_p=drop_p, seed=seed)
        else:
            out = ws.get(tag + '.out', (rows_q, d), f32) if out is None else out
            K.gemm(f, P.w(pre + 'ffn.2.weight'), out, rows_q, d, 4 * d, epi=EPI_DROPOUT_RESID, resid=xc, ldr=d,
                   drop_p=drop_p, seed=seed, aux=out_bf, ldaux=d if out_bf is not None else 0)
        st.update(h2=h2, gprime=gprime, f=f, xc=xc, rows_q=rows_q)
        return out, st

    def _o_extra(self, tag, rows_q, d, Lq):
        if self.delta_fused or self.o32_mode:
            return dict(o32=self.ws.get(tag + '32', (rows_q, d), f32), so32=d, bo32=Lq * d)
        return dict(o_lo=self.ws.get(tag + 'lo', (rows_q, d)), so_lo=d, bo_lo=Lq * d)

    def _dq_part(self, B, H, Lq, Lk, hd, window=0):
        n = K.attn_dq_part_elems(B, H, Lq, Lk, hd, window)
        t = self.ws.bufs.get('b.dqpart')
        return t if t is not None and t.numel() >= n else self.ws.get('b.dqpart', (n,), f32)

    def layer_bwd(self, st, dout, dx_out, *, dx_accumulate=False, dctx=None, g2_ready=False, next_drop=None,
                  zsplice=None):
        d, ws, P = self.d, self.ws, self.P
        pre, B, Sx, L, Lq = st['pre'], st['B'], st['Sx'], st['L'], st['Lq']
        heads, hd = st['heads'], st['hd']
        rows_x, rows_q = B * Sx, st['rows_q']
        rot = self.rot(max(Sx, L), st['window'])
        a = pre + 'attention.'
        g2 = ws.get('b.g2', (rows_q, d))
        if not g2_ready:
            K.dropout_bwd_cast(dout, g2, st['drop_p'], st['seed'], rows_q, d)
        dpre = ws.get('b.dpre', (rows_q, 4 * d))
        K.gemm(g2, P.wT(pre + 'ffn.2.weight', d, 4 * d), dpre, rows_q, 4 * d, d, epi=EPI_GELU_BWD, aux=st['gprime'],
               ldaux=4 * d)
        self._dw_pair((g2, st['f'], pre + 'ffn.2.weight', rows_q, d, 4 * d),
                      (dpre, st['h2'], pre + 'ffn.0.weight', rows_q, 4 * d, d, None, None, pre + 'ffn.0.bias'))
        dh2 = ws.get('b.dh2', (rows_q, d))
        K.gemm(dpre, P.wT(pre + 'ffn.0.weight', 4 * d, d), dh2, rows_q, d, 4 * d, epi=EPI_BF16)
        dxc = ws.get('b.dxc', (rows_q, d), f32)
        gxc = ws.get('b.gxc', (rows_q, d))
        self._ln_bwd(pre + 'ffn_layer_norm', dh2, st['ln_f'], rows_q, dout, dxc, gxc)
        dx1, gx1 = dxc, gxc
        if st['cross']:
            c = pre + 'cross_attention.'
            rows_c = B * L
            dOc = ws.get('b.dO', (rows_q, d))
            delta = ws.get('b.delta', (B, heads, Lq), f32)
            K.gemm(gxc, P.wT(c + 'output_linear.weight', d, d), dOc, rows_q, d, d, epi=EPI_BF16, delta=delta if self.delta_fused else None,
                   delta_o32=st['Ocx'].get('o32'), ld_o32=d, delta_hd=hd, delta_seq=Lq)
            dqc = ws.get('b.dqc', (rows_q, d))
            dkvc = ws.get('b.dkvc', (rows_c, 2 * d))
            K.attention(st['qc'], st['kvc'], st['kvc'][:, d:], st['Oc'], st['lsec'], B=B, H=heads, Lq=Lq, Lk=L,
                        hd=hd, sq=d, bq=Lq * d, sk=2 * d, sv=2 * d, bk=L * 2 * d, bv=L * 2 * d, so=d, bo=Lq * d,
                        key_pad=st['pad_ctx'], causal=False, backward=True, delta_ready=self.delta_fused,
                        dout=dOc, sdo=d, bdo=Lq * d, delta=delta, dq_bf=dqc, ldq_bf=d, dk=dkvc, dv=dkvc[:, d:],
                        sdk=2 * d, sdv=2 * d, bdk=L * 2 * d, bdv=L * 2 * d, rot=rot, rot_d=d, **st['Ocx'],
                        dq_part=self._dq_part(B, heads, Lq, L, hd))
            self._dw_pair((gxc, st['Oc'], c + 'output_linear.weight', rows_q, d, d, None, None,
                           c + 'output_linear.bias'),
                          (dqc, st['hq'], c + 'q_linear.weight', rows_q, d, d, None, None, c + 'q_linear.bias'))
            dhq = ws.get('b.dhq', (rows_q, d))
            K.gemm(dqc, P.wT(c + 'q_linear.weight', d, d), dhq, rows_q, d, d, epi=EPI_BF16)
            self._dw(dkvc, st['cx'], c + 'k_linear.weight', rows_c, 2 * d, d, bias=c + 'k_linear.bias')
            dcx = ws.get('b.dcx.' + st['tag'] if st.get('ctx_deferred') else 'b.dcx', (rows_c, d))
            K.gemm(dkvc, P.wT(c + 'k_linear.weight', 2 * d, d), dcx, rows_c, d, 2 * d, epi=EPI_BF16)
            dx1 = ws.get('b.dx1', (rows_q, d), f32)
            gx1 = ws.get('b.gx1', (rows_q, d))
            self._ln_bwd(pre + 'cross_attn_layer_norm', dhq, st['ln_cross'], rows_q, dxc, dx1, gx1)
            if st.get('ctx_deferred'):
                st['dcx'] = dcx
            else:
                self._ln_bwd(pre + 'context_layer_norm', dcx, st['ln_ctx'], rows_c, dctx, dctx)
        wo_dw = (gx1, st['O'], a + 'output_linear.weight', rows_q, d, d, None, None, a + 'output_linear.bias')
        dO = ws.get('b.dO', (rows_q, d))
        delta = ws.get('b.delta', (B, heads, Lq), f32)
        K.gemm(gx1, P.wT(a + 'output_linear.weight', d, d), dO, rows_q, d, d, epi=EPI_BF16, delta=delta if self.delta_fused else None,
               delta_o32=st['Ox'].get('o32'), ld_o32=d, delta_hd=hd, delta_seq=Lq)
        if st['learned']:
            kv = st['kv']
            dq32 = ws.get('b.dq32', (B * Lq, d), f32)
            dkv = ws.get('b.dkv', (rows_x, 2 * d))
            K.attention(P.w(a + 'learned_queries').view(Lq, d), kv, kv[:, d:], st['O'], st['lse'], B=B, H=heads,
                        Lq=Lq, Lk=Sx, hd=hd, sq=d, bq=0, sk=2 * d, sv=2 * d, bk=Sx * 2 * d, bv=Sx * 2 * d, so=d,
                        bo=Lq * d, key_pad=st['pad_k'], causal=False, backward=True, dout=dO, sdo=d, bdo=Lq * d,
                        delta=delta, delta_ready=self.delta_fused, dq=dq32, bdq=Lq * d, dk=dkv, dv=dkv[:, d:], sdk=2 * d, sdv=2 * d,
                        bdk=Sx * 2 * d, bdv=Sx * 2 * d, rot=rot, rot_d=d, **st['Ox'],
                        dq_part=self._dq_part(B, heads, Lq, Sx, hd))
            K.colsum(dq32, B, Lq * d, Lq * d, P.g(a + 'learned_queries').view(-1))
            self._dw_pair(wo_dw, (dkv, st['h'], a + 'k_linear.weight', rows_x, 2 * d, d, None, None,
                                  a + 'k_linear.bias'))
            dh = ws.get('b.dh', (rows_x, d))
            K.gemm(dkv, P.wT(a + 'k_linear.weight', 2 * d, d), dh, rows_x, d, 2 * d, epi=EPI_BF16)
        else:
            qkv = st['qkv']
            dqkv = ws.get('b.dqkv', (rows_x, 3 * d))
            K.attention(qkv, qkv[:, d:], qkv[:, 2 * d:], st['O'], st['lse'], B=B, H=heads, Lq=Lq, Lk=Sx, hd=hd,
                        sq=3 * d, bq=Sx * 3 * d, sk=3 * d, sv=3 * d, bk=Sx * 3 * d, bv=Sx * 3 * d, so=d, bo=Lq * d,
                        key_pad=st['pad_k'], causal=st['causal'], window=st['window'], backward=True, dout=dO,
                        sdo=d, bdo=Lq * d,
                        delta=delta, delta_ready=self.delta_fused, dq_bf=dqkv, ldq_bf=3 * d, dk=dqkv[:, d:], dv=dqkv[:, 2 * d:], sdk=3 * d,
                        sdv=3 * d, bdk=Sx * 3 * d, bdv=Sx * 3 * d, rot=rot, rot_d=d, **st['Ox'],
                        dq_part=self._dq_part(B, heads, Lq, Sx, hd, st['window']))
            self._dw_pair(wo_dw, (dqkv, st['h'], a + 'q_linear.weight', rows_x, 3 * d, d, None, None,
                                  a + 'q_linear.bias'))
            dh = ws.get('b.dh', (rows_x, d))
            K.gemm(dqkv, P.wT(a + 'q_linear.weight', 3 * d, d), dh, rows_x, d, 3 * d, epi=EPI_BF16)
        if st['resid']:
            self._ln_bwd(pre + 'attn_layer_norm', dh, st['ln_a'], rows_x, dx1, dx_out,
                         dx_bf=ws.get('b.g2', (rows_x, d)) if next_drop is not None else None, bf_drop=next_drop,
                         zsplice=zsplice)
            if dx_accumulate:
                raise NotImplementedError('residual + accumulate is handled by the caller')
        else:
            self._ln_bwd(pre + 'attn_layer_norm', dh, st['ln_a'], rows_x, dx_out if dx_accumulate else None, dx_out)

    def forward(self, ids, ntok, *, pad=True, eps=None, seed=0, kl_weight=1.0, dropout=0.1, need_logits=False):
        hp, d, ws, P = self.hp, self.d, self.ws, self.P
        if not ids.is_cuda:
            raise RuntimeError('VAEEngine needs device tensors (no CPU fallback)')
        P.sync_shadow()
        B, L = ids.shape
        T, V, Z, N = B * L, hp.vocab_size, hp.latent_depth, hp.num_latents
        ids32 = ws.get('ids', (B, L), torch.int32)
        padm = None
        if pad is not None and pad is not False:
            padm = ws.get('pad', (B, L), torch.uint8)
        labels = ws.get('labels', (B, L), torch.int32)
        ntok64 = ws.get('ntok', (B,), torch.int64)
        if (self.small_fused and ids.dtype == torch.int64 and ids.is_contiguous() and isinstance(ntok, torch.Tensor) and ntok.is_cuda
                and ntok.dtype == torch.int64 and ntok.is_contiguous() and ntok.numel() == B
                and (padm is None or pad is True or (pad.dtype == torch.bool and pad.is_contiguous()))):
            K.prep_tokens(ids, pad if padm is not None else None, B, L, ids32, labels, padm, ntok, ntok64)
        else:
            ids32.copy_(ids)
            if padm is not None:
                padm.copy_(ids.eq(0) if pad is True else pad)
            labels[:, :-1].copy_(ids32[:, 1:])
            labels[:, -1] = 0
            ntok64.copy_(ntok)
        sv = {'B': B, 'L': L, 'dropout': dropout, 'seed': seed}

        x_emb = ws.get('x_emb', (T, d), f32)
        K.embedding_fwd(ids32, P.f('input_layer.0.weight'), x_emb, T, d, out2=ws.get('x_dec0', (T, d), f32))

        enc_bf, stats, sv['enc_layers'] = self._encode(x_emb, B, L, padm, dropout, seed)

        zf = ws.get('z', (B, Z), f32)
        zb = ws.get('z_bf', (B, Z))
        eps_buf = ws.get('eps', (B, Z), f32)
        raw_kl = ws.get('raw_kl', (B,), f32)
        kl = ws.get('kl', (2,), f32)
        if eps is not None:
            eps_buf.copy_(eps.reshape(B, Z))
        K.reparam_fwd(stats, eps_buf if eps is not None else None, _mix_seed(seed, 7), ntok64, zf, zb, eps_buf,
                      raw_kl, kl, B, Z)
        sv.update(enc_bf=enc_bf, stats=stats, z_bf=zb, eps=eps_buf)

        xf, sv['dec_layers'] = self._decode(x_emb, zb, padm, B, L, dropout, seed, x_ready=True)

        gp0 = ws.get('h0_gprime', (T, d))
        h0 = ws.get('h0', (T, d))
        K.gemm(xf, P.w('output_layer.0.weight'), h0, T, d, d, epi=EPI_GELU, bias=P.f('output_layer.0.bias'),
               aux=gp0, ldaux=d)
        hh, ln_h = self._ln_fwd('output_layer.2', h0, T, 'head.ln')
        nchunks, chunk_len = K.ce_chunking(B, L, V, CE_CHUNK_NUMEL)
        lse = ws.get('ce.lse', (T,), f32)
        row_loss = ws.get('ce.row_loss', (T,), f32)
        chunk_w = ws.get('ce.chunk_w', (max(8, nchunks),), f32)
        nll = ws.get('nll', (1,), f32)
        ntile = -(-V // 128)
        head = 'logits' if need_logits else self.head_mode
        W, bias = P.w('input_layer.0.weight'), P.f('output_layer.3.bias')
        logits = ws.get('logits', (T, V))
        probe = self.probe
        if probe is not None:
            e0 = torch.cuda.Event(enable_timing=True)
            e0.record()
        if head == 'prob':
            coff = ws.get('ce.off', (T,), f32)
            K.ce_label_logit(hh, W, bias, labels, T, d, coff)
            part = ws.get('ce.psum', (ntile, T), f32)
            K.gemm(hh, W, logits, T, V, d, epi=EPI_CE_PROB, bias=bias, aux=part, labels=labels, row_a=coff)
        else:
            coff = None
            part = ws.get('ce.part', (T, ntile, 2), f32)
            lab_logit = ws.get('ce.label_logit', (T,), f32)
            K.gemm(hh, W, logits, T, V, d, epi=EPI_CE_STATS, bias=bias, aux=part, labels=labels, label_logit=lab_logit)
        if probe is not None:
            e1 = torch.cuda.Event(enable_timing=True)
            e1.record()
            probe.append((e0, e1))
        if head == 'prob':
            sat = ws.get('ce.sat', (T + 1,), torch.int32)
            K.ce_prob_finalize(part, ntile, coff, labels, T, L, nchunks, chunk_len, lse, row_loss, chunk_w, nll,
                               fix=(hh, W, bias, logits, sat))
        else:
            K.ce_finalize(part, ntile, lab_logit, labels, T, L, nchunks, chunk_len, lse, row_loss, chunk_w, nll)
        sv.update(xf=xf, gp0=gp0, h0=h0, hh=hh, ln_h=ln_h, logits=logits, lse=lse, chunk_w=chunk_w,
                  nchunks=nchunks, chunk_len=chunk_len, labels=labels, ids32=ids32, ntok=ntok64, x_emb=x_emb,
                  row_loss=row_loss, head=head, coff=coff)
        if self.small_fused:
            lbuf = ws.get('loss', (1,), f32)
            K.step_scalars(kl_weight, nll=nll, kl=kl, loss=lbuf)
            loss = lbuf[0]
        else:
            loss = nll[0] + kl_weight * kl[0]
        self.saved = sv
        return {'loss': loss, 'nll': nll[0], 'kl': kl[0], 'train_kl': kl[1], 'raw_kl': raw_kl,
                'mu': stats[:, :Z], 'logvar': stats[:, Z:], 'stats': stats, 'kl_buf': kl, 'z': zf, 'eps': eps_buf,
                'logits': logits if need_logits else None,
                'ce_saturated': sat[0] if head == 'prob' else None}

    def weighted_nll(self, tok_w):
        sv = self.saved
        out = torch.empty(1, dtype=f32, device=self.P.device)
        B, L = sv['B'], sv['L']
        K.ce_weighted_nll(sv['row_loss'], sv['labels'], tok_w, B * L, L, sv['nchunks'], sv['chunk_len'], out)
        return out[0]

    def _encode(self, x_emb, B, L, padm, dropout, seed):
        hp, d, ws, P = self.hp, self.d, self.ws, self.P
        N, Z = hp.num_latents, hp.latent_depth
        lay = []
        z, st = self.layer_fwd('encoder.first_layer.', x_emb, B, L, L, padm, learned=N, heads=self.He, hd=64,
                               drop_p=dropout, seed=_mix_seed(seed, 1000), tag='e0')
        lay.append(st)
        nmid = hp.enc_layers - 2
        cxs = self._ctx_ln_fwd(x_emb, B * L, nmid) if P.ctx_batched else [None] * nmid
        for j in range(nmid):
            z, st = self.layer_fwd(f'encoder.middle_layers.{j}.', z, B, N, L, padm, cross=True, ctx=x_emb,
                                   heads=self.He, hd=64, drop_p=dropout, seed=_mix_seed(seed, 1001 + j), tag=f'e{j + 1}',
                                   ctx_ln=cxs[j])
            lay.append(st)
        enc, st = self.layer_fwd('encoder.bottleneck.', z, B, N, L, padm, learned=1, heads=self.He, hd=64,
                                 drop_p=dropout, seed=_mix_seed(seed, 1999), tag='eb')
        lay.append(st)
        enc_bf = ws.get('enc_bf', (B, d))
        K.cast_bf16(enc, enc_bf)
        stats = ws.get('stats', (B, 2 * Z), f32)
        K.gemm(enc_bf, P.w('q_of_z_given_x.linear.weight'), stats, B, 2 * Z, d, epi=EPI_F32,
               bias=P.f('q_of_z_given_x.linear.bias'))
        return enc_bf, stats, lay

    def _ctx_ln_fwd(self, x, rows, nmid):
        D, ws, P = self.d, self.ws, self.P
        mean = ws.get('ctx.ln.mean', (rows,), f32)
        rstd = ws.get('ctx.ln.rstd', (rows,), f32)
        out = []
        for j0 in range(0, nmid, LN_MULTI_MAX):
            js = range(j0, min(nmid, j0 + LN_MULTI_MAX))
            names = [f'encoder.middle_layers.{j}.context_layer_norm' for j in js]
            ys = [ws.get(f'e{j + 1}.ln_ctx.y', (rows, D)) for j in js]
            K.layernorm_fwd_multi(x, [P.f(n + '.weight') for n in names], [P.f(n + '.bias') for n in names], ys, mean,
                                  rstd, rows, D)
            out += [(y, (x, mean, rstd)) for y in ys]
        return out

    def _ctx_ln_bwd(self, sts, dctx):
        D, P = self.d, self.P
        for j0 in range(0, len(sts), LN_MULTI_MAX):
            grp = sts[j0:j0 + LN_MULTI_MAX]
            x, mean, rstd = grp[0]['ln_ctx']
            rows = x.shape[0]
            names = [g['pre'] + 'context_layer_norm' for g in grp]
            wgs = [P.grad[P.offsets[n + '.weight'][0]:][:2 * D] for n in names]
            n1 = 1024 * 2 * D
            if self.cs_batch:
                if len(self._cs_pending) + len(grp) > COLSUM_MAX:
                    self.flush_colsum()
                k = len(self._cs_pending)
                part = self.ws.get('ln.parts', (COLSUM_MAX * n1,), f32)[k * n1:(k + len(grp)) * n1]
                defer = self._cs_pending
            else:
                part = self.ws.get('ln.partm', (LN_MULTI_MAX * n1,), f32)
                defer = None
            K.layernorm_bwd_multi([g['dcx'] for g in grp], x, [P.f(n + '.weight') for n in names], mean, rstd, dctx,
                                  dctx, wgs, rows, D, part, defer=defer)

    def _inputs(self, ids, pad):
        B, L = ids.shape
        ids32 = self.ws.get('ids', (B, L), torch.int32)
        ids32.copy_(ids)
        padm = None
        if pad is not None and pad is not False:
            padm = self.ws.get('pad', (B, L), torch.uint8)
            padm.copy_(ids.eq(0) if pad is True else pad)
        return ids32, padm

    def mutual_info(self, out, eps=None, num_samples=10):
        stats = out['stats']
        B, Z = stats.shape[0], stats.shape[1] // 2
        if eps is not None:
            eps = eps.to(stats.device, f32).reshape(num_samples, B, Z).contiguous()
        ws = self.ws.get('mi_ws', (2 * num_samples * B,), f32)
        res = torch.empty((), dtype=f32, device=stats.device)
        seed = int(torch.randint(0, 2 ** 62, (1,)).item())
        K.mutual_info(stats, out['kl_buf'], B, Z, seed, res, ws, eps=eps, S=num_samples)
        return res

    def posterior(self, ids, pad=True):
        if not ids.is_cuda:
            raise RuntimeError('VAEEngine needs device tensors (no CPU fallback)')
        self.P.sync_shadow()
        B, L = ids.shape
        ids32, padm = self._inputs(ids, pad)
        x_emb = self.ws.get('x_emb', (B * L, self.d), f32)
        K.embedding_fwd(ids32, self.P.f('input_layer.0.weight'), x_emb, B * L, self.d)
        _, stats, _ = self._encode(x_emb, B, L, padm, 0.0, 0)
        return stats

    def seq_log_prob(self, x_emb, labels, z, pad=None, max_tokens=32768):
        hp, d, ws, P = self.hp, self.d, self.ws, self.P
        if not x_emb.is_cuda:
            raise RuntimeError('VAEEngine needs device tensors (no CPU fallback)')
        P.sync_shadow()
        G, Bt, L = x_emb.shape[0], x_emb.shape[1], x_emb.shape[2]
        V, Z = hp.vocab_size, hp.latent_depth
        out = torch.empty(G, Bt, dtype=f32, device=P.device)
        ntile = -(-V // 128)
        if Bt * L <= max_tokens:
            gstep, bstep = max(1, max_tokens // (Bt * L)), Bt
        else:
            gstep, bstep = 1, max(1, max_tokens // L)
        for g0 in range(0, G, gstep):
            g1 = min(G, g0 + gstep)
            for b0 in range(0, Bt, bstep):
                b1 = min(Bt, b0 + bstep)
                ng, nb = g1 - g0, b1 - b0
                B = ng * nb
                T = B * L
                padm = None
                if pad is not None:
                    padm = ws.get('pad', (B, L), torch.uint8)
                    padm.view(ng, nb, L).copy_(pad[g0:g1, b0:b1])
                lab = ws.get('labels', (B, L), torch.int32)
                lab.view(ng, nb, L)[:, :, :-1].copy_(labels[g0:g1, b0:b1])
                lab[:, -1] = 0
                xe = ws.get('x_emb', (T, d), f32)
                xe.view(ng, nb, L, d).copy_(x_emb[g0:g1, b0:b1])
                zf = ws.get('z_f32', (B, Z), f32)
                zf.view(ng, nb, Z).copy_(z[g0:g1, b0:b1])
                zb = ws.get('z_bf', (B, Z))
                K.cast_bf16(zf, zb)
                xf, _ = self._decode(xe, zb, padm, B, L, 0.0, 0)
                hh = self._head_hidden(xf, T)
                part = ws.get('ce.part', (T, ntile, 2), f32)
                lab_logit = ws.get('ce.label_logit', (T,), f32)
                K.gemm(hh, P.w('input_layer.0.weight'), None, T, V, d, epi=EPI_CE_STATS,
                       bias=P.f('output_layer.3.bias'), aux=part, labels=lab, label_logit=lab_logit)
                res = ws.get('seq_lp', (B,), f32)
                K.ce_seq_logprob(part, ntile, lab_logit, lab, T, L, res)
                out[g0:g1, b0:b1].copy_(res.view(ng, nb))
        return out

    def _head_hidden(self, xf, T):
        d, ws, P = self.d, self.ws, self.P
        gp0 = ws.get('h0_gprime', (T, d))
        h0 = ws.get('h0', (T, d))
        K.gemm(xf, P.w('output_layer.0.weight'), h0, T, d, d, epi=EPI_GELU, bias=P.f('output_layer.0.bias'),
               aux=gp0, ldaux=d)
        hh, _ = self._ln_fwd('output_layer.2', h0, T, 'head.ln')
        return hh

    def _decode(self, x_emb, zb, padm, B, L, dropout, seed, x_ready=False):
        hp, d, ws, P = self.hp, self.d, self.ws, self.P
        T, Z = B * L, hp.latent_depth
        if self.window and L % 32:
            raise ValueError(f'sparse decoder attention needs seq_len % 32 == 0 (SparseAttention block_size 32, '
                             f'sparse_attention.py:81), got {L}')
        fuse = self.fuse_ln
        xs = ws.get('x_dec0', (T, d), f32)
        if not x_ready:
            xs.copy_(x_emb)
        xf = ws.get('xf_bf', (T, d))
        dec = []
        h_in = None
        zf_batch = self.zf_batch and not fuse and d % 8 == 0 and Z <= 1024
        if zf_batch:
            zall = ws.get('zproj_all', (hp.num_layers, B, d), f32)
            segs = [(P.w(f'z_projections.{i}.weight'), P.f(f'z_projections.{i}.bias'), zall[i])
                    for i in range(hp.num_layers)]
            for c0 in range(0, len(segs), ZPROJ_MAX):
                K.zproj_fwd_multi(segs[c0:c0 + ZPROJ_MAX], zb, B, d, Z)
        else:
            K.gemm(zb, P.w('z_projections.0.weight'), xs, B, d, Z, ldc=L * d, epi=EPI_F32,
                   bias=P.f('z_projections.0.bias'))
        for i in range(hp.num_layers):
            last = i + 1 == hp.num_layers
            if fuse:
                nxt = None
                if not last:
                    zrows = ws.get('zrows', (B, d), f32)
                    K.gemm(zb, P.w(f'z_projections.{i + 1}.weight'), zrows, B, d, Z, epi=EPI_F32,
                           bias=P.f(f'z_projections.{i + 1}.bias'))
                    nxt = (f'decoder_layers.{i + 1}.attn_layer_norm', zrows, L, f'd{i + 1}')
                out = None if last else ws.get(f'x_dec{i + 1}', (T, d), f32)
            else:
                if i > 0 and not zf_batch:
                    K.gemm(zb, P.w(f'z_projections.{i}.weight'), xs, B, d, Z, ldc=L * d, epi=EPI_F32,
                           bias=P.f(f'z_projections.{i}.bias'))
                nxt, out = None, ws.get(f'x_dec{i + 1}', (T, d), f32)
            xs, st = self.layer_fwd(f'decoder_layers.{i}.', xs, B, L, L, padm, causal=True, heads=self.H,
                                    hd=self.hd, drop_p=dropout, seed=_mix_seed(seed, i), tag=f'd{i}', out=out,
                                    window=self.window, fuse=fuse, h_in=h_in, next_ln=nxt,
                                    out_bf=xf if last and (fuse or self.resid_bf16) else None,
                                    zsplice=(zall[i], L) if zf_batch else None)
            h_in = st.pop('next_h', None)
            dec.append(st)
        if not fuse and not self.resid_bf16:
            K.cast_bf16(xs, xf)
        return xf, dec

    def reconstruct_f32(self, x_emb, z, pad=None):
        hp, d, P = self.hp, self.d, self.P
        dev = P.device
        B, L = x_emb.shape[0], x_emb.shape[1]
        T, V, Z, H, hd = B * L, hp.vocab_size, hp.latent_depth, self.H, self.hd
        rot = self.rot(L, self.window)
        padm = None
        if pad is not None:
            padm = torch.empty(B, L, dtype=torch.uint8, device=dev)
            padm.copy_(pad)
        x = x_emb.reshape(T, d).clone()
        h = torch.empty(T, d, device=dev)
        qkv = torch.empty(T, 3 * d, device=dev)
        o = torch.empty(T, d, device=dev)
        x1 = torch.empty(T, d, device=dev)
        f = torch.empty(T, 4 * d, device=dev)
        for i in range(hp.num_layers):
            pre = f'decoder_layers.{i}.'
            a = pre + 'attention.'
            K.gemm_f32(z, P.f(f'z_projections.{i}.weight'), x, B, d, Z, ldc=L * d, bias=P.f(f'z_projections.{i}.bias'))
            K.layernorm_fwd_f32(x, P.f(pre + 'attn_layer_norm.weight'), P.f(pre + 'attn_layer_norm.bias'), h, T, d)
            K.gemm_f32(h, P.f(a + 'q_linear.weight'), qkv, T, 3 * d, d, epi=EPI_ROTARY_BF16, bias=P.f(a + 'q_linear.bias'),
                       rot=rot, rot_cols=2 * d, rot_d=d, rot_seq=L)
            K.attention_f32(qkv, qkv[:, d:], qkv[:, 2 * d:], o, B=B, H=H, Lq=L, Lk=L, hd=hd, sq=3 * d, sk=3 * d,
                            sv=3 * d, so=d, bq=L * 3 * d, bk=L * 3 * d, bv=L * 3 * d, bo=L * d, key_pad=padm, causal=True,
                            window=self.window)
            K.gemm_f32(o, P.f(a + 'output_linear.weight'), x1, T, d, d, bias=P.f(a + 'output_linear.bias'), resid=x, ldr=d)
            K.layernorm_fwd_f32(x1, P.f(pre + 'ffn_layer_norm.weight'), P.f(pre + 'ffn_layer_norm.bias'), h, T, d)
            K.gemm_f32(h, P.f(pre + 'ffn.0.weight'), f, T, 4 * d, d, epi=EPI_GELU, bias=P.f(pre + 'ffn.0.bias'))
            K.gemm_f32(f, P.f(pre + 'ffn.2.weight'), x, T, d, 4 * d, resid=x1, ldr=d)
        h0 = torch.empty(T, d, device=dev)
        K.gemm_f32(x, P.f('output_layer.0.weight'), h0, T, d, d, epi=EPI_GELU, bias=P.f('output_layer.0.bias'))
        K.layernorm_fwd_f32(h0, P.f('output_layer.2.weight'), P.f('output_layer.2.bias'), h, T, d)
        logits = torch.empty(B, L, V, device=dev)
        K.gemm_f32(h, P.f('input_layer.0.weight'), logits, T, V, d, bias=P.f('output_layer.3.bias'))
        return logits

    def reconstruct(self, x_emb, z, pad=None):
        hp, d, ws, P = self.hp, self.d, self.ws, self.P
        P.sync_shadow()
        B, L = x_emb.shape[0], x_emb.shape[1]
        T, V, Z = B * L, hp.vocab_size, hp.latent_depth
        padm = None
        if pad is not None:
            padm = ws.get('pad', (B, L), torch.uint8)
            padm.copy_(pad)
        zb = ws.get('z_bf', (B, Z))
        K.cast_bf16(z, zb)
        xf, _ = self._decode(x_emb.reshape(T, d), zb, padm, B, L, 0.0, 0)
        gp0 = ws.get('h0_gprime', (T, d))
        h0 = ws.get('h0', (T, d))
        K.gemm(xf, P.w('output_layer.0.weight'), h0, T, d, d, epi=EPI_GELU, bias=P.f('output_layer.0.bias'),
               aux=gp0, ldaux=d)
        hh, _ = self._ln_fwd('output_layer.2', h0, T, 'head.ln')
        logits = torch.empty(B, L, V, dtype=bf16, device=P.device)
        K.gemm(hh, P.w('input_layer.0.weight'), logits, T, V, d, epi=EPI_BF16, bias=P.f('output_layer.3.bias'))
        return logits

    def backward(self, gloss, kl_weight, ready=None):
        sv, hp, d, ws, P = self.saved, self.hp, self.d, self.ws, self.P
        user_ready = ready

        def ready(end):
            if user_ready is not None:
                self.flush_colsum()
                self.flush_zproj()
                self.join_side()
                user_ready(end)
        if sv is None:
            raise RuntimeError('backward() without a saved forward')
        B, L = sv['B'], sv['L']
        T, V, Z, N = B * L, hp.vocab_size, hp.latent_depth, hp.num_latents
        gs = ws.get('gscale', (2,), f32)
        gl = gloss.reshape(1)
        if self.small_fused and gl.is_cuda and gl.dtype == f32:
            K.step_scalars(kl_weight, gloss=gl, gs=gs)
        else:
            gs[0:1].copy_(gl)
            gs[1:2].copy_(gl * kl_weight)

        logits = sv['logits']
        dhh = ws.get('b.dhh', (T, d))
        nch, clen = sv['nchunks'], sv['chunk_len']
        if sv['head'] == 'prob':
            hh = sv['hh']
            hh_r = ws.get('b.hh_r', (T, d))
            r_t = ws.get('b.ce_r', (T,), f32)
            q_t = ws.get('b.ce_q', (T,), f32)
            dbias = P.g('output_layer.3.bias')
            K.ce_prob_bwd_prep(hh, sv['lse'], sv['coff'], sv['chunk_w'], sv['labels'], gs[0:1], T, L, nch, clen, d, hh_r,
                               r_t, q_t, dbias)
            s = self._head_dw_splits(V, d)
            if s == 1:
                K.gemm(logits, hh_r, P.g('input_layer.0.weight'), V, d, T, a_t=True, b_t=True, lda=V, ldb=d, ldc=d,
                       epi=EPI_F32_ACC, a_rowsum=dbias, k_weight=r_t)
            else:
                slab = ws.get('b.head_dw_slab', (s * V * d,), f32)
                K.gemm(logits, hh_r, P.g('input_layer.0.weight'), V, d, T, a_t=True, b_t=True, lda=V, ldb=d, ldc=d,
                       epi=EPI_F32_ATOMIC, splits=s, aux=slab, a_rowsum=dbias, k_weight=r_t)
            W = P.w('input_layer.0.weight')
            K.gemm(logits, P.wT('input_layer.0.weight', V, d), dhh, T, d, V, epi=EPI_ROWSCALE_GATHER,
                   labels=sv['labels'], row_a=r_t, row_b=q_t, gather=W, ldg=d)
            sv['ce_q'] = q_t
        else:
            K.ce_grad(logits, V, sv['lse'], sv['chunk_w'], sv['labels'], gs[0:1], T, V, L, nch, clen)
            self._dw(logits, sv['hh'], 'input_layer.0.weight', T, V, d, bias='output_layer.3.bias', on_side=False)
            K.gemm(logits, P.wT('input_layer.0.weight', V, d), dhh, T, d, V, epi=EPI_BF16)
        dpre0 = ws.get('b.dpre0', (T, d))
        if self.ln_gelu:
            self._ln_bwd('output_layer.2', dhh, sv['ln_h'], T, None, None, dx_bf=dpre0, gelu=sv['gp0'])
        else:
            dh0 = ws.get('b.dh0', (T, d), f32)
            self._ln_bwd('output_layer.2', dhh, sv['ln_h'], T, None, dh0)
            K.gelu_bwd(dh0, sv['gp0'], dpre0, T * d)
        self._dw(dpre0, sv['xf'], 'output_layer.0.weight', T, d, d, bias='output_layer.0.bias')
        dx = ws.get('b.dx_dec', (T, d), f32)
        top = sv['dec_layers'][-1]
        g2_pre = self.head_g2 and top['rows_q'] == T
        K.gemm(dpre0, P.wT('output_layer.0.weight', d, d), dx, T, d, d, epi=EPI_F32,
               aux=ws.get('b.g2', (T, d)) if g2_pre else None, ldaux=d if g2_pre else 0,
               drop_p=top['drop_p'] if g2_pre else 0.0, seed=top['seed'] if g2_pre else 0)
        ready(P.end('output_layer.3.bias'))

        dz = ws.get('b.dz', (B, Z), f32, zero=True)
        dzh = ws.get('b.dzh', (B, d), f32)
        dzh_bf = ws.get('b.dzh_bf', (B, d))
        dx_prev = ws.get('b.dx_prev', (T, d), f32)
        g2_ready = g2_pre
        for i in reversed(range(hp.num_layers)):
            st = sv['dec_layers'][i]
            nd = None
            if i > 0 and st['resid'] and sv['dec_layers'][i - 1]['rows_q'] == T:
                nst = sv['dec_layers'][i - 1]
                nd = (nst['drop_p'], nst['seed'], L)
            dzh_i = ws.get('b.dzh_all', (hp.num_layers, B, d), f32)[i] if self.zp_batch else dzh
            zs = (L, dzh_i, None) if st['resid'] and st['rows_q'] == T else None
            self.layer_bwd(st, dx, dx_prev, g2_ready=g2_ready, next_drop=nd, zsplice=zs)
            g2_ready = nd is not None
            wz, bz = f'z_projections.{i}.weight', f'z_projections.{i}.bias'
            if zs is not None and self.zp_batch:
                if len(self._zp_pending) == ZPROJ_MAX:
                    self.flush_zproj()
                self._zp_ctx = (sv['z_bf'], dz, B, d, Z)
                self._zp_pending.append((dzh_i, P.w(wz), P.g(wz), P.g(bz)))
            elif zs is not None:
                K.zproj_bwd(dzh, sv['z_bf'], P.w(wz), P.g(wz), P.g(bz), dz, B, d, Z)
            else:
                self.flush_zproj()
                K.extract_rows(dx_prev, d, T, L, d, dzh)
                K.cast_bf16(dzh, dzh_bf)
                self._dw(dzh_bf, sv['z_bf'], wz, B, d, Z, bias=bz)
                K.gemm(dzh_bf, P.w(wz), dz, B, Z, d, b_t=True, epi=EPI_F32_ATOMIC, splits=max(1, min(8, d // 64)))
            ready(P.end(f'z_projections.{i}.bias'))
            dx, dx_prev = dx_prev, dx
        self.flush_zproj()
        dx_emb = dx

        dstats = ws.get('b.dstats', (B, 2 * Z), f32)
        K.reparam_bwd(sv['stats'], sv['eps'], dz, sv['ntok'], gs[1:2], dstats, B, Z)
        dstats_bf = ws.get('b.dstats_bf', (B, 2 * Z))
        K.cast_bf16(dstats, dstats_bf)
        self._dw(dstats_bf, sv['enc_bf'], 'q_of_z_given_x.linear.weight', B, 2 * Z, d)
        self._db(dstats, 'q_of_z_given_x.linear.bias', B, 2 * Z)
        denc = ws.get('b.denc', (B, d), f32)
        K.gemm(dstats_bf, P.w('q_of_z_given_x.linear.weight'), denc, B, d, 2 * Z, b_t=True, epi=EPI_F32)
        ready(P.end('q_of_z_given_x.linear.bias'))

        enc = sv['enc_layers']
        dcur = denc
        for k in reversed(range(1, len(enc))):
            st = enc[k]
            nxt = ws.get(f'b.denc{k}', (B * N, d), f32)
            self.layer_bwd(st, dcur, nxt, dctx=dx_emb)
            ready(P.end(st['pre'] + 'ffn_layer_norm.bias'))
            dcur = nxt
        deferred = [st for st in enc if st.get('ctx_deferred')]
        if deferred:
            self._ctx_ln_bwd(deferred[::-1], dx_emb)
            ready(P.end(deferred[0]['pre'] + 'context_layer_norm.bias'))
        st0 = enc[0]
        if st0['resid']:
            tmp = ws.get('b.dfirst', (T, d), f32)
            self.layer_bwd(st0, dcur, tmp)
            self.join_side()
            K.embedding_bwd(sv['ids32'], tmp, P.g('input_layer.0.weight'), T, d)
        else:
            self.layer_bwd(st0, dcur, dx_emb, dx_accumulate=True)

        ready(P.end('encoder.first_layer.ffn_layer_norm.bias'))
        self.join_side()
        self._embedding_bwd(sv, dx_emb, T, d)
        ready(P.n_live)
        self.flush_colsum()
        self.join_side()

    def _embedding_bwd(self, sv, dx, T, d):
        if sv['head'] == 'prob':
            K.embedding_bwd_ce(sv['ids32'], dx, self.P.g('input_layer.0.weight'), T, d, sv['L'], sv['hh'], sv['ce_q'])
        else:
            K.embedding_bwd(sv['ids32'], dx, self.P.g('input_layer.0.weight'), T, d)
```

### sparse-vae_amd/sparse_vae/kernels.py

```python
import ctypes
import os

import torch

from . import _native as N
from ._native import lib, check, ptr, stream

bf16, f32 = torch.bfloat16, torch.float32

_gemm_desc = N.GemmDesc()


def _dev(*ts):
    for t in ts:
        if t is not None and not t.is_cuda:
            raise RuntimeError('libsvae kernels need device tensors (no CPU fallback)')


def gemm(A, B, C, M, N_, K, *, a_t=False, b_t=False, lda=None, ldb=None, ldc=None, epi=N.EPI_BF16, bias=None,
         resid=None, ldr=0, aux=None, ldaux=0, alpha=1.0, splits=1, drop_p=0.0, seed=0, rot=None, rot_cols=0,
         rot_d=0, rot_seq=0, labels=None, label_logit=None, batch=1, sA=0, sB=0, sC=0, a_rowsum=None, k_weight=None,
         row_a=None, row_b=None, gather=None, ldg=0, delta=None, delta_o32=None, ld_o32=0, delta_hd=0, delta_seq=0):
    d = _fill_desc(_gemm_desc, A, B, C, M, N_, K, a_t=a_t, b_t=b_t, lda=lda, ldb=ldb, ldc=ldc, epi=epi, bias=bias,
                   resid=resid, ldr=ldr, aux=aux, ldaux=ldaux, alpha=alpha, splits=splits, drop_p=drop_p, seed=seed,
                   rot=rot, rot_cols=rot_cols, rot_d=rot_d, rot_seq=rot_seq, labels=labels, label_logit=label_logit,
                   batch=batch, sA=sA, sB=sB, sC=sC, a_rowsum=a_rowsum, k_weight=k_weight, row_a=row_a, row_b=row_b,
                   gather=gather, ldg=ldg)
    if delta is not None:
        _dev(delta, delta_o32)
        assert delta.dtype == f32 and delta_o32.dtype == f32 and delta.numel() >= M * (N_ // delta_hd)
    d.delta, d.delta_o32, d.ld_o32 = ptr(delta), ptr(delta_o32), ld_o32
    d.delta_hd, d.delta_seq = delta_hd, delta_seq
    check(lib.svae_gemm(ctypes.byref(d), stream()), 'svae_gemm')


def _fill_desc(d, A, B, C, M, N_, K, *, a_t=False, b_t=False, lda=None, ldb=None, ldc=None, epi=N.EPI_BF16,
               bias=None, resid=None, ldr=0, aux=None, ldaux=0, alpha=1.0, splits=1, drop_p=0.0, seed=0, rot=None,
               rot_cols=0, rot_d=0, rot_seq=0, labels=None, label_logit=None, batch=1, sA=0, sB=0, sC=0,
               a_rowsum=None, k_weight=None, row_a=None, row_b=None, gather=None, ldg=0):
    _dev(A, B, C)
    assert A.dtype == bf16 and B.dtype == bf16
    d.A, d.B = A.data_ptr(), B.data_ptr()
    d.lda = lda if lda is not None else (M if a_t else K)
    d.ldb = ldb if ldb is not None else (N_ if b_t else K)
    d.batch_stride_a, d.batch_stride_b = sA, sB
    d.M, d.N, d.K = M, N_, K
    d.batch, d.splits = batch, splits
    d.a_t, d.b_t = int(a_t), int(b_t)
    d.epi = epi
    d.C = ptr(C)
    d.ldc = ldc if ldc is not None else N_
    d.batch_stride_c = sC
    d.bias = ptr(bias)
    d.resid = ptr(resid)
    d.ldr = ldr
    d.aux = ptr(aux)
    d.ldaux = ldaux
    d.alpha = alpha
    d.drop_p = drop_p
    d.seed = seed & 0xFFFFFFFFFFFFFFFF
    d.rot_tab = ptr(rot)
    d.rot_cols, d.rot_d, d.rot_seq = rot_cols, rot_d, rot_seq
    d.labels = ptr(labels)
    d.label_logit = ptr(label_logit)
    d.a_rowsum = ptr(a_rowsum)
    d.k_weight = ptr(k_weight)
    d.row_a, d.row_b = ptr(row_a), ptr(row_b)
    d.gather, d.ldg = ptr(gather), ldg
    d.delta, d.delta_o32, d.ld_o32, d.delta_hd, d.delta_seq = None, None, 0, 0, 0
    return d


_pair_desc = (N.GemmDesc(), N.GemmDesc())


def gemm_pair(g0, g1):
    d0 = _fill_desc(_pair_desc[0], *g0[0], **g0[1])
    d1 = _fill_desc(_pair_desc[1], *g1[0], **g1[1])
    check(lib.svae_gemm_pair(ctypes.byref(d0), ctypes.byref(d1), stream()), 'svae_gemm_pair')


def auto_splits(M, N_, K, target=512):
    t256 = -(-M // 256) * -(-N_ // 256)
    if t256 >= 192:
        return 1
    if t256 >= 4:
        s3 = min(256 // t256, max(1, K // 512))
        if t256 * s3 >= 192:
            return s3
    tiles = -(-M // 128) * -(-N_ // 128)
    if tiles >= 256 or K < 1024:
        return 1
    s = min(-(-target // tiles), K // 512)
    return max(1, s)


def linear_dw(dY, X, Wgrad, rows, n_out, n_in, ldy=None, ldx=None, bgrad=None):
    s = auto_splits(n_out, n_in, rows)
    slab = _slab_workspace(s * n_out * n_in, dY.device) if s > 1 else None
    gemm(dY, X, Wgrad, n_out, n_in, rows, a_t=True, b_t=True, lda=ldy or n_out, ldb=ldx or n_in, ldc=n_in,
         epi=N.EPI_F32_ATOMIC if s > 1 else N.EPI_F32_ACC, splits=s, a_rowsum=bgrad, aux=slab)


def pair_splits(shapes):
    tiles = [-(-m // 256) * -(-n // 256) for m, n, _ in shapes]
    rows = [r for _, _, r in shapes]
    if not all(tiles):
        return None
    if os.environ.get('SVAE_DW_PAIR_EQUAL', '0') != '0':
        c = min([256 // sum(tiles)] + [r // 512 for r in rows])
        return (c, c) if c >= 2 else None
    cap = [r // 512 for r in rows]
    if min(cap) < 2:
        return None
    work = sum(t * r for t, r in zip(tiles, rows))
    slice_rows = max(512.0, work / 256.0)
    sp = [min(c, max(2, round(r / slice_rows))) for r, c in zip(rows, cap)]
    while sum(t * x for t, x in zip(tiles, sp)) > 256:
        i = min((k for k in range(2) if sp[k] > 2), key=lambda k: rows[k] / sp[k], default=None)
        if i is None:
            return None
        sp[i] -= 1
    sp = [-(-r // (-(-(-(-r // x)) // 64) * 64)) for r, x in zip(rows, sp)]
    longest = max(r / x for r, x in zip(rows, sp))
    for k in range(2):
        while sp[k] > 2 and rows[k] / (sp[k] - 1) <= longest:
            sp[k] -= 1
    return tuple(sp)


def linear_dw_pair(j0, j1):
    sp = pair_splits([(j[4], j[5], j[3]) for j in (j0, j1)])
    if sp is None:
        linear_dw(*j0[:8], bgrad=j0[8])
        linear_dw(*j1[:8], bgrad=j1[8])
        return
    n0, n1 = sp[0] * j0[4] * j0[5], sp[1] * j1[4] * j1[5]
    slab = _slab_workspace(n0 + n1, j0[0].device)
    gs = []
    for j, aux, s in ((j0, slab[:n0], sp[0]), (j1, slab[n0:n0 + n1], sp[1])):
        dY, X, Wg, rows, n_out, n_in, ldy, ldx, bg = j
        gs.append(((dY, X, Wg, n_out, n_in, rows),
                   dict(a_t=True, b_t=True, lda=ldy or n_out, ldb=ldx or n_in, ldc=n_in, epi=N.EPI_F32_ATOMIC,
                        splits=s, a_rowsum=bg, aux=aux)))
    gemm_pair(*gs)


_slabs = {}


def _slab_workspace(n, device):
    t = _slabs.get(device)
    if t is None or t.numel() < n:
        t = torch.empty(n, dtype=torch.float32, device=device)
        _slabs[device] = t
    return t


def resid_ln_fwd(x, y, h, rows, D, *, w=None, b=None, mean=None, rstd=None, xo=None, drop_p=0.0, seed=0, zrows=None,
                 zmod=0):
    _dev(h, *(t for t in (x, y, xo, zrows, w, b, mean, rstd) if t is not None))
    assert h.dtype == bf16 and (y is None or y.dtype in (bf16, f32)) and (x is None or x.dtype == f32)
    for t in (x, xo, zrows, h, w, b):
        assert t is None or t.is_contiguous(), 'resid_ln_fwd: x, xo, zrows, h, w, b must be contiguous'
    check(lib.svae_resid_ln_fwd(ptr(x), ptr(y), 1 if y is not None and y.dtype == bf16 else 0,
                                y.stride(0) if y is not None else 0, float(drop_p), int(seed) & (2 ** 64 - 1),
                                ptr(zrows), int(zmod), ptr(w), ptr(b), ptr(xo), h.data_ptr(), ptr(mean), ptr(rstd), rows,
                                D, stream()), 'svae_resid_ln_fwd')


def layernorm_fwd(x, w, b, y, mean, rstd, rows, D):
    _dev(x, w, b, y, mean, rstd)
    check(lib.svae_layernorm_fwd(x.data_ptr(), 0 if x.dtype == f32 else 1, w.data_ptr(), b.data_ptr(), y.data_ptr(),
                                 mean.data_ptr(), rstd.data_ptr(), rows, D, stream()), 'svae_layernorm_fwd')


def layernorm_bwd(dy, x, w, mean, rstd, dres, dx, dx_bf, wgrad2, rows, D, part_ws, bf_drop=None, zsplice=None,
                  defer=None):
    nblk = lib.svae_layernorm_nblk(rows)
    part = part_ws[: nblk * 2 * D]
    if bf_drop is None and zsplice is None:
        check(lib.svae_layernorm_bwd(dy.data_ptr(), x.data_ptr(), 0 if x.dtype == f32 else 1, w.data_ptr(),
                                     mean.data_ptr(), rstd.data_ptr(), ptr(dres), dx.data_ptr(), ptr(dx_bf),
                                     part.data_ptr(), nblk, rows, D, 0, stream()), 'svae_layernorm_bwd')
    else:
        p, seed, zmod = bf_drop if bf_drop is not None else (0.0, 0, 0)
        zm, zrow, zrow_bf = zsplice if zsplice is not None else (0, None, None)
        check(lib.svae_layernorm_bwd_drop(dy.data_ptr(), x.data_ptr(), 0 if x.dtype == f32 else 1, w.data_ptr(),
                                          mean.data_ptr(), rstd.data_ptr(), ptr(dres), dx.data_ptr(), ptr(dx_bf),
                                          part.data_ptr(), nblk, rows, D, int(zm), float(p),
                                          int(seed) & 0xFFFFFFFFFFFFFFFF, int(zmod), ptr(zrow), ptr(zrow_bf),
                                          stream()), 'svae_layernorm_bwd_drop')
    if defer is not None:
        defer.append((part, nblk, 2 * D, 2 * D, wgrad2))
    else:
        colsum(part, nblk, 2 * D, 2 * D, wgrad2, accumulate=True)


def layernorm_bwd_gelu(dy, x, w, mean, rstd, gp, out_bf, wgrad2, rows, D, part_ws, defer=None):
    nblk = lib.svae_layernorm_nblk(rows)
    part = part_ws[: nblk * 2 * D]
    check(lib.svae_layernorm_bwd_gelu(dy.data_ptr(), x.data_ptr(), 0 if x.dtype == f32 else 1, w.data_ptr(),
                                      mean.data_ptr(), rstd.data_ptr(), gp.data_ptr(), out_bf.data_ptr(),
                                      part.data_ptr(), nblk, rows, D, stream()), 'svae_layernorm_bwd_gelu')
    if defer is not None:
        defer.append((part, nblk, 2 * D, 2 * D, wgrad2))
    else:
        colsum(part, nblk, 2 * D, 2 * D, wgrad2, accumulate=True)


def _ptrs(ts):
    return (ctypes.c_void_p * N.LN_MULTI_MAX)(*[t.data_ptr() for t in ts])


def layernorm_fwd_multi(x, ws, bs, ys, mean, rstd, rows, D):
    n = len(ys)
    assert 0 < n <= N.LN_MULTI_MAX and len(ws) == n and len(bs) == n and x.dtype == f32
    _dev(x, mean, rstd, *ws, *bs, *ys)
    check(lib.svae_layernorm_fwd_multi(x.data_ptr(), _ptrs(ws), _ptrs(bs), _ptrs(ys), n, mean.data_ptr(),
                                       rstd.data_ptr(), rows, D, stream()), 'svae_layernorm_fwd_multi')


def layernorm_bwd_multi(dys, x, ws, mean, rstd, dres, dx, wgrads, rows, D, part_ws, defer=None):
    n = len(dys)
    assert 0 < n <= N.LN_MULTI_MAX and len(ws) == n and len(wgrads) == n and x.dtype == f32
    _dev(x, mean, rstd, dx, *dys, *ws)
    nblk = lib.svae_layernorm_nblk(rows)
    parts = [part_ws[j * nblk * 2 * D:(j + 1) * nblk * 2 * D] for j in range(n)]
    assert parts[-1].numel() == nblk * 2 * D
    check(lib.svae_layernorm_bwd_multi(_ptrs(dys), x.data_ptr(), _ptrs(ws), mean.data_ptr(), rstd.data_ptr(),
                                       ptr(dres), dx.data_ptr(), _ptrs(parts), nblk, n, rows, D, stream()),
          'svae_layernorm_bwd_multi')
    for part, wg in zip(parts, wgrads):
        if defer is not None:
            defer.append((part, nblk, 2 * D, 2 * D, wg))
        else:
            colsum(part, nblk, 2 * D, 2 * D, wg, accumulate=True)


_colsum_segs = (N.ColsumSeg * N.COLSUM_MAX)()


def colsum_multi(segs):
    assert 0 < len(segs) <= N.COLSUM_MAX
    for i, (inp, rows, cols, ld, out) in enumerate(segs):
        _dev(inp, out)
        assert inp.dtype == f32 and out.dtype == f32
        _colsum_segs[i].inp, _colsum_segs[i].out = inp.data_ptr(), out.data_ptr()
        _colsum_segs[i].ld, _colsum_segs[i].rows, _colsum_segs[i].cols = ld, rows, cols
    check(lib.svae_colsum_multi(ctypes.addressof(_colsum_segs), len(segs), stream()), 'svae_colsum_multi')


def colsum(inp, rows, cols, ld, out, accumulate=True):
    check(lib.svae_colsum(inp.data_ptr(), 0 if inp.dtype == f32 else 1, rows, cols, ld, out.data_ptr(),
                          int(accumulate), stream()), 'svae_colsum')


_attn_desc = N.AttnDesc()


def attention(q, k, v, o, lse, *, B, H, Lq, Lk, hd, sq, sk, sv, so, bq, bk, bv, bo, key_pad=None, causal=False,
              window=0, scale=None, backward=False, dout=None, sdo=0, bdo=0, delta=None, dq=None, bdq=0, dk=None, dv=None,
              sdk=0, sdv=0, bdk=0, bdv=0, rot=None, rot_d=0, o32=None, so32=0, bo32=0, dq_part=None, dq_bf=None,
              ldq_bf=0, delta_ready=False, o_lo=None, so_lo=0, bo_lo=0):
    d = _attn_desc
    d.q, d.k, d.v, d.o = q.data_ptr(), k.data_ptr(), v.data_ptr(), o.data_ptr()
    d.sq, d.sk, d.sv, d.so, d.bq, d.bk, d.bv, d.bo = sq, sk, sv, so, bq, bk, bv, bo
    d.key_pad = ptr(key_pad)
    d.lse = lse.data_ptr()
    d.B, d.H, d.Lq, d.Lk, d.hd, d.causal = B, H, Lq, Lk, hd, int(causal)
    d.window = int(window)
    d.delta_ready = int(bool(delta_ready))
    d.scale = hd ** -0.5 if scale is None else scale
    d.o32, d.so32, d.bo32 = ptr(o32), so32, bo32
    d.o_lo, d.so_lo, d.bo_lo = ptr(o_lo), so_lo, bo_lo
    if backward:
        d.fwd_ws, d.fwd_ws_elems = None, 0
        d.dout, d.sdo, d.bdo = dout.data_ptr(), sdo, bdo
        d.delta, d.bdq = delta.data_ptr(), bdq
        d.dk, d.dv, d.sdk, d.sdv, d.bdk, d.bdv = dk.data_ptr(), dv.data_ptr(), sdk, sdv, bdk, bdv
        d.rot_tab, d.rot_d = ptr(rot), rot_d
        if dq_part is None:
            dq_part = torch.empty(attn_dq_part_elems(B, H, Lq, Lk, hd, window), device=q.device, dtype=torch.float32)
        assert dq_part.numel() >= attn_dq_part_elems(B, H, Lq, Lk, hd, window) and dq_part.dtype == torch.float32
        d.dq_part, d.dq_bf, d.ldq_bf = dq_part.data_ptr(), ptr(dq_bf), ldq_bf
        d.dq = ptr(dq)
        check(lib.svae_attn_bwd(ctypes.byref(d), stream()), 'svae_attn_bwd')
    else:
        d.dout = None
        n = lib.svae_attn_fwd_ws_elems(B, H, Lq, Lk, hd, int(causal), int(window))
        if n > 0:
            ws = _fwd_workspace(n, q.device)
            d.fwd_ws, d.fwd_ws_elems = ws.data_ptr(), ws.numel()
        else:
            d.fwd_ws, d.fwd_ws_elems = None, 0
        check(lib.svae_attn_fwd(ctypes.byref(d), stream()), 'svae_attn_fwd')


_fwd_ws = {}


def _fwd_workspace(n, device):
    t = _fwd_ws.get(device)
    if t is None or t.numel() < n:
        t = torch.empty(n, dtype=torch.float32, device=device)
        _fwd_ws[device] = t
    return t


def attn_dq_part_elems(B, H, Lq, Lk, hd, window=0):
    return lib.svae_attn_dq_part_elems_w(B, H, Lq, Lk, hd, int(window))


def dq_finalize(dq, out, ldo, rows, D, rot=None, seq=0):
    check(lib.svae_dq_finalize(dq.data_ptr(), out.data_ptr(), ldo, rows, D, ptr(rot), seq, stream()),
          'svae_dq_finalize')


def embedding_fwd(ids, table, out, rows, D, out2=None):
    if out2 is not None:
        _dev(ids, table, out, out2)
        check(lib.svae_embedding_fwd_dual(ids.data_ptr(), table.data_ptr(), out.data_ptr(), out2.data_ptr(), rows, D,
                                          stream()), 'svae_embedding_fwd_dual')
        return
    check(lib.svae_embedding_fwd(ids.data_ptr(), table.data_ptr(), out.data_ptr(), None, rows, D, stream()),
          'svae_embedding_fwd')


def embedding_bwd(ids, dout, dtable, rows, D):
    check(lib.svae_embedding_bwd(ids.data_ptr(), dout.data_ptr(), dtable.data_ptr(), rows, D, stream()),
          'svae_embedding_bwd')


def reparam_fwd(stats, eps, seed, ntok, z, z_bf, eps_out, raw_kl, kl_out, B, Z):
    check(lib.svae_reparam_kl_fwd(stats.data_ptr(), ptr(eps), seed & 0xFFFFFFFFFFFFFFFF, ntok.data_ptr(),
                                  z.data_ptr(), ptr(z_bf), ptr(eps_out), raw_kl.data_ptr(), kl_out.data_ptr(), B, Z,
                                  stream()), 'svae_reparam_kl_fwd')


def reparam_bwd(stats, eps, dz, ntok, gkl, dstats, B, Z):
    check(lib.svae_reparam_kl_bwd(stats.data_ptr(), eps.data_ptr(), ptr(dz), ntok.data_ptr(), gkl.data_ptr(),
                                  dstats.data_ptr(), B, Z, stream()), 'svae_reparam_kl_bwd')


def ce_red_ws(device, nchunks):
    n = max(1024, lib.svae_ce_red_ws_elems(nchunks))
    t = _ce_red.get(device)
    if t is None or t.numel() < n:
        t = _ce_red[device] = torch.empty(n, dtype=f32, device=device)
    return t


_ce_red = {}


def ce_finalize(part, ntile, label_logit, labels, rows, seq, nchunks, chunk_len, lse, row_loss, chunk_w, nll):
    assert chunk_w.numel() >= nchunks and chunk_w.dtype == f32
    red = ce_red_ws(part.device, nchunks)
    check(lib.svae_ce_finalize(part.data_ptr(), ntile, label_logit.data_ptr(), labels.data_ptr(), rows, seq,
                               nchunks, chunk_len, lse.data_ptr(), row_loss.data_ptr(), chunk_w.data_ptr(),
                               nll.data_ptr(), red.data_ptr(), stream()), 'svae_ce_finalize')


def ce_weighted_nll(row_loss, labels, tok_w, rows, seq, nchunks, chunk_len, out):
    _dev(row_loss, labels, tok_w, out)
    assert tok_w.dtype == f32 and tok_w.is_contiguous()
    red = ce_red_ws(row_loss.device, nchunks)
    check(lib.svae_ce_weighted_nll(row_loss.data_ptr(), labels.data_ptr(), tok_w.data_ptr(), rows, seq, nchunks,
                                   chunk_len, out.data_ptr(), red.data_ptr(), stream()), 'svae_ce_weighted_nll')


def ce_chunking(B, L, V, chunk_numel=2 ** 30):
    chunks = -(-(B * (L - 1) * V) // chunk_numel)
    chunk_len = -(-(L - 1) // chunks)
    return -(-(L - 1) // chunk_len), chunk_len


def ce_label_logit(hh, W, bias, labels, rows, D, out):
    _dev(hh, W, labels, out)
    check(lib.svae_ce_label_logit(hh.data_ptr(), hh.stride(0), W.data_ptr(), W.stride(0), ptr(bias), labels.data_ptr(),
                                  rows, D, out.data_ptr(), stream()), 'svae_ce_label_logit')


def ce_prob_finalize(part, ntile, row_off, labels, rows, seq, nchunks, chunk_len, lse, row_loss, chunk_w, nll,
                     fix=None):
    assert chunk_w.numel() >= nchunks and chunk_w.dtype == f32
    red = ce_red_ws(part.device, nchunks)
    if fix is None:
        check(lib.svae_ce_prob_finalize(part.data_ptr(), ntile, row_off.data_ptr(), labels.data_ptr(), rows, seq,
                                        nchunks, chunk_len, lse.data_ptr(), row_loss.data_ptr(), chunk_w.data_ptr(),
                                        nll.data_ptr(), red.data_ptr(), stream()), 'svae_ce_prob_finalize')
        return
    hh, W, bias, P, sat = fix
    _dev(hh, W, P, sat)
    assert sat.dtype == torch.int32 and sat.numel() >= rows + 1 and P.shape[0] >= rows
    check(lib.svae_ce_prob_finalize_fix(part.data_ptr(), ntile, row_off.data_ptr(), labels.data_ptr(), rows, seq,
                                        nchunks, chunk_len, lse.data_ptr(), row_loss.data_ptr(), chunk_w.data_ptr(),
                                        nll.data_ptr(), red.data_ptr(), hh.data_ptr(), hh.stride(0), W.data_ptr(),
                                        W.stride(0), ptr(bias), P.data_ptr(), P.stride(0), W.shape[0], hh.shape[1],
                                        sat.data_ptr(), stream()), 'svae_ce_prob_finalize_fix')


def ce_prob_bwd_prep(hh, lse, row_off, chunk_w, labels, gscale, rows, seq, nchunks, chunk_len, D, hh_out, r_out,
                     q_out, dbias=None):
    _dev(hh, lse, row_off, chunk_w, labels, gscale, hh_out, r_out, q_out)
    check(lib.svae_ce_prob_bwd_prep(hh.data_ptr(), hh.stride(0), lse.data_ptr(), row_off.data_ptr(),
                                    chunk_w.data_ptr(), labels.data_ptr(), gscale.data_ptr(), rows, seq, nchunks,
                                    chunk_len, D, hh_out.data_ptr(), r_out.data_ptr(), q_out.data_ptr(), ptr(dbias),
                                    stream()), 'svae_ce_prob_bwd_prep')


def embedding_bwd_ce(ids, dout, dtable, rows, D, seq, hh, q):
    check(lib.svae_embedding_bwd_ce(ids.data_ptr(), dout.data_ptr(), dtable.data_ptr(), rows, D, seq, hh.data_ptr(),
                                    q.data_ptr(), stream()), 'svae_embedding_bwd_ce')


def mutual_info(stats, kl, B, Z, seed, out, ws, eps=None, S=10):
    _dev(stats, kl, out, ws)
    assert ws.numel() >= 2 * S * B
    check(lib.svae_mutual_info(stats.data_ptr(), ptr(eps), seed & 0xFFFFFFFFFFFFFFFF, kl.data_ptr(), B, Z, S,
                               ws.data_ptr(), out.data_ptr(), stream()), 'svae_mutual_info')


def ce_seq_logprob(part, ntile, label_logit, labels, rows, seq, out):
    _dev(part, label_logit, labels, out)
    assert out.dtype == f32 and out.numel() == rows // seq and out.is_contiguous()
    check(lib.svae_ce_seq_logprob(part.data_ptr(), ntile, label_logit.data_ptr(), labels.data_ptr(), rows, seq,
                                  out.data_ptr(), stream()), 'svae_ce_seq_logprob')


def ce_grad(logits, ld, lse, chunk_w, labels, gscale, rows, V, seq, nchunks, chunk_len, dbias=None):
    check(lib.svae_ce_grad(logits.data_ptr(), ld, lse.data_ptr(), chunk_w.data_ptr(), labels.data_ptr(),
                           gscale.data_ptr(), ptr(dbias), rows, V, seq, nchunks, chunk_len, stream()), 'svae_ce_grad')


def prep_tokens(ids, pad, B, L, ids32, labels, padm=None, ntok=None, ntok_out=None):
    assert ids.dtype == torch.int64 and ids.is_contiguous() and ids.numel() == B * L
    mode = 0 if pad is None or pad is False else (1 if pad is True else 2)
    if mode == 2:
        assert pad.dtype == torch.bool and pad.is_contiguous() and pad.numel() == B * L
    if ntok is not None:
        assert ntok.dtype == torch.int64 and ntok.is_contiguous() and ntok.numel() == B
    _dev(ids, ids32, labels)
    check(lib.svae_prep_tokens(ids.data_ptr(), pad.data_ptr() if mode == 2 else None, mode, B, L, ids32.data_ptr(),
                               labels.data_ptr(), ptr(padm), ptr(ntok), ptr(ntok_out), stream()), 'svae_prep_tokens')


def step_scalars(kl_weight, nll=None, kl=None, loss=None, gloss=None, gs=None):
# ... 210 lines not shown
```

Measured before the change: 2.677 million tokens/s.

## Defer backward weight-gradient GEMMs and launch them as grouped kernels

During backward, weight-gradient GEMMs are queued instead of launched one by one, then flushed at the end as a few grouped launches. The launches are driven by a device-side table of GEMM parameters and a block-to-GEMM map that spreads blocks across XCDs, with a single list kernel reducing the split-K slabs. Activation-gradient workspace buffers get per-layer names so the deferred GEMMs still read valid data. This removes many small launches and improves CU occupancy for the dW GEMMs, at the cost of extra workspace memory, lost overlap with the side stream, and a host sync whenever the table changes.

New measurement: 2.826 million tokens/s, median of 6. +5.6%, better.

```diff
diff --git a/include/svae.h b/include/svae.h
--- a/include/svae.h
+++ b/include/svae.h
@@ -59,6 +59,12 @@
 
 int svae_gemm_pair(const svae_gemm_desc* d0, const svae_gemm_desc* d1, svae_stream_t stream);
 
+#define SVAE_GROUP_MAX 256
+#define SVAE_GROUP_MAX_BLOCKS 1024
+int64_t svae_gemm_group_table_bytes(int32_t n);
+int svae_gemm_group(const svae_gemm_desc* d, int32_t n, int32_t max_blocks, void* table, void* table_host,
+                    int64_t table_bytes, svae_stream_t stream);
+
 int svae_resid_ln_fwd(const float* x, const void* y, int32_t y_dtype, int64_t ldy, float drop_p, uint64_t seed,
                       const float* zrows, int32_t zmod, const float* w, const float* b, float* xo, void* h, float* mean,
                       float* rstd, int32_t rows, int32_t D, svae_stream_t stream);
diff --git a/sparse-vae_amd/csrc/gemm.hip b/sparse-vae_amd/csrc/gemm.hip
--- a/sparse-vae_amd/csrc/gemm.hip
+++ b/sparse-vae_amd/csrc/gemm.hip
@@ -1,7 +1,9 @@
 #include "common.h"
 #include "../../include/svae.h"
 #include <stdlib.h>
+#include <string.h>
 #include <algorithm>
+#include <vector>
 
 using namespace svae;
 
@@ -1085,7 +1087,7 @@
 }
 
 template <bool AT, bool BT, int EPI>
-__device__ __forceinline__ void gemm256_run(const GP& p, int blk, int nwg) {
+__device__ __forceinline__ void gemm256_run(const GP& p, int blk, int nwg, bool remap = true) {
   static_assert(g3_epi_vmem_ops<EPI>() >= G3_EPI_STORES, "the relaxed first wait would not cover the prefetch DMA");
   constexpr bool IS_KW = EPI == G3_EPI_ACC_KW || EPI == G3_EPI_F32_KW;
   constexpr int KW_FORM = IS_KW ? SVAE_KW_FORM : 0;
@@ -1102,7 +1104,7 @@
   const int wave = __builtin_amdgcn_readfirstlane(tid >> 6);
   const int wr = wave >> 2, wc = wave & 3;
   int bid = blk;
-  if (nwg >= 16) {
+  if (remap && nwg >= 16) {
     const int q = nwg / 8, r = nwg % 8, xcd = bid % 8, idx = bid / 8;
     bid = (xcd < r ? xcd * (q + 1) : r * (q + 1) + (xcd - r) * q) + idx;
   }
@@ -1346,6 +1348,35 @@
   gemm256_run<AT, BT, EPI>(q.p[sel], sel ? b - q.nb0 : b, sel ? (int)gridDim.x - q.nb0 : q.nb0);
 }
 
+struct alignas(16) GPSlot {
+  GP p;
+};
+struct alignas(16) GMap {
+  int gemm, blk, nblk, pad;
+};
+
+template <class T>
+__device__ __forceinline__ T load_uniform(const T* src) {
+  static_assert(sizeof(T) % 4 == 0, "whole dwords");
+  typedef const unsigned __attribute__((address_space(4))) * cu32p;
+  struct W {
+    unsigned w[sizeof(T) / 4];
+  } r;
+  const cu32p c = (cu32p)(uintptr_t)src;
+#pragma unroll
+  for (unsigned i = 0; i < sizeof(T) / 4; ++i) r.w[i] = c[i];
+  return __builtin_bit_cast(T, r);
+}
+
+template <int EPI>
+__global__ __launch_bounds__(512, 1) void gemm256_group_kernel(const GPSlot* __restrict__ tab,
+                                                               const GMap* __restrict__ map) {
+  const GMap e = load_uniform(map + blockIdx.x);
+  if (e.gemm < 0) return;
+  const GP p = load_uniform(&tab[e.gemm].p);
+  gemm256_run<true, true, EPI>(p, e.blk, e.nblk, false);
+}
+
 constexpr int SK_BN = 32, SK_WAVES = 16;
 
 template <int EPI>
@@ -1456,6 +1487,15 @@
 __global__ __launch_bounds__(256) void slab_reduce2_kernel(SlabRed r0, SlabRed r1, int nb0) {
   if ((int)blockIdx.x < nb0) slab_reduce_range(r0, blockIdx.x, nb0);
   else slab_reduce_range(r1, blockIdx.x - nb0, (int)gridDim.x - nb0);
+}
+struct alignas(16) SlabRedSlot {
+  SlabRed r;
+};
+__global__ __launch_bounds__(256) void slab_reduce_list_kernel(const SlabRedSlot* __restrict__ list, int n) {
+  for (int e = 0; e < n; ++e) {
+    const SlabRed r = load_uniform(&list[e].r);
+    slab_reduce_range(r, blockIdx.x, gridDim.x);
+  }
 }
 
 }
@@ -1784,6 +1824,157 @@
   return SVAE_OK;
 }
 
+namespace {
+
+struct GroupHeader {
+  unsigned long long bytes, dev;
+  int n, grid_a, grid_b, nred;
+};
+static_assert(sizeof(GroupHeader) == 32, "table header");
+
+constexpr long long group_align(long long x) { return (x + 15) / 16 * 16; }
+
+void place_blocks(const std::vector<int>& gemm, const std::vector<int>& nb, std::vector<GMap>& map) {
+  long long total = 0;
+  for (int x : nb) total += x;
+  const int grid = (int)((total + 7) / 8 * 8), per = grid / 8;
+  map.assign(grid, GMap{-1, 0, 0, 0});
+  int used[8] = {0, 0, 0, 0, 0, 0, 0, 0};
+  std::vector<int> order(nb.size());
+  for (size_t i = 0; i < order.size(); ++i) order[i] = (int)i;
+  std::stable_sort(order.begin(), order.end(), [&](int a, int b) { return nb[a] > nb[b]; });
+  for (int i : order) {
+    int x = 0;
+    while (x < 8 && per - used[x] < nb[i]) ++x;
+    int blk = 0;
+    for (int y = x < 8 ? x : 0; blk < nb[i] && y < 8; ++y)
+      while (blk < nb[i] && used[y] < per) map[(size_t)used[y]++ * 8 + y] = GMap{gemm[i], blk++, nb[i], 0};
+  }
+}
+
+int device_cus() {
+  static const int ncu = [] {
+    int dev = 0, n = 0;
+    if (hipGetDevice(&dev) != hipSuccess || hipDeviceGetAttribute(&n, hipDeviceAttributeMultiprocessorCount, dev) != hipSuccess)
+      n = 256;
+    return n > 0 ? n : 256;
+  }();
+  return ncu;
+}
+
+}
+
+SVAE_EXPORT int64_t svae_gemm_group_table_bytes(int32_t n) {
+  if (n <= 0 || n > SVAE_GROUP_MAX) return 0;
+  return (int64_t)(sizeof(GroupHeader) + n * (sizeof(GPSlot) + sizeof(SlabRedSlot)) +
+                   2 * (SVAE_GROUP_MAX_BLOCKS + 8) * sizeof(GMap));
+}
+
+SVAE_EXPORT int svae_gemm_group(const svae_gemm_desc* d, int32_t n, int32_t max_blocks, void* table, void* table_host,
+                                int64_t table_bytes, svae_stream_t stream) {
+  if (!d || n <= 0 || n > SVAE_GROUP_MAX || max_blocks < 0 || max_blocks > SVAE_GROUP_MAX_BLOCKS || !table ||
+      !table_host || ((uintptr_t)table & 15) || table_bytes < svae_gemm_group_table_bytes(n))
+    return SVAE_EINVAL;
+  const int cap = max_blocks ? max_blocks : std::min(device_cus(), (int)SVAE_GROUP_MAX_BLOCKS);
+  std::vector<GPSlot> gp(n);
+  std::vector<SlabRedSlot> red;
+  std::vector<int> idx[2], units[2], nb[2];
+  std::vector<double> work[2];
+  long long red_elems = 0;
+  for (int i = 0; i < n; ++i) {
+    const svae_gemm_desc* di = d + i;
+    if (const int rc = validate_desc(di)) return rc;
+    const bool split = di->epi == SVAE_EPI_F32_ATOMIC;
+    if (!di->a_t || !di->b_t || di->batch != 1 || di->k_weight || di->bias || di->resid ||
+        (!split && (di->epi != SVAE_EPI_F32_ACC || di->splits != 1)) || (split && (!di->aux || ((uintptr_t)di->aux & 15))))
+      return SVAE_EINVAL;
+    GP& p = gp[i].p;
+    memset(&gp[i], 0, sizeof(GPSlot));
+    fill_gp(di, p);
+    p.bias = nullptr; p.resid = nullptr; p.aux = nullptr;
+    if (split) {
+      p.C = di->aux; p.ldc = di->N; p.sC = 0; p.slab = (long long)di->M * di->N;
+      p.epi = G3_EPI_SLAB;
+    }
+    const int kc3 = (di->K + di->splits - 1) / di->splits;
+    p.kchunk = (kc3 + 63) / 64 * 64;
+    p.tn2 = (di->N + 255) / 256;
+    p.tm2 = (di->M + 255) / 256;
+    p.group = 0;
+    const long long u = (long long)p.tn2 * p.tm2 * di->splits;
+    if (u > (1 << 24)) return SVAE_EINVAL;
+    p.total3 = (int)u;
+    p.relaxed = 1;
+    p.dma_stagger = split ? 0 : 1;
+    const int c = split ? 1 : 0;
+    idx[c].push_back(i);
+    units[c].push_back((int)u);
+    work[c].push_back((double)u * ((p.kchunk + 63) / 64 + 8));
+    if (split) {
+      SlabRedSlot s;
+      memset(&s, 0, sizeof(s));
+      s.r = slab_red(di);
+      red.push_back(s);
+      red_elems += (long long)di->M * (di->N / 4);
+    }
+  }
+  std::vector<GMap> map[2];
+  for (int c = 0; c < 2; ++c) {
+    const int m = (int)idx[c].size();
+    if (!m) continue;
+    long long total = 0;
+    double wsum = 0;
+    for (int k = 0; k < m; ++k) total += units[c][k], wsum += work[c][k];
+    if (c == 0 && !max_blocks && total > cap) return SVAE_EINVAL;
+    if (cap < m) return SVAE_EINVAL;
+    nb[c].resize(m);
+    if (total <= cap) nb[c] = units[c];
+    else
+      for (int k = 0; k < m; ++k)
+        nb[c][k] = std::min(units[c][k], 1 + (int)((cap - m) * (work[c][k] / wsum)));
+    place_blocks(idx[c], nb[c], map[c]);
+  }
+  const long long o_gp = sizeof(GroupHeader), o_ma = o_gp + (long long)n * sizeof(GPSlot);
+  const long long o_mb = o_ma + (long long)map[0].size() * sizeof(GMap);
+  const long long o_red = o_mb + (long long)map[1].size() * sizeof(GMap);
+  const long long bytes = o_red + (long long)red.size() * sizeof(SlabRedSlot);
+  if (bytes > table_bytes) return SVAE_EINVAL;
+  std::vector<char> img((size_t)bytes, 0);
+  const GroupHeader h{(unsigned long long)bytes, (unsigned long long)(uintptr_t)table, n, (int)map[0].size(),
+                      (int)map[1].size(), (int)red.size()};
+  memcpy(img.data(), &h, sizeof(h));
+  memcpy(img.data() + o_gp, gp.data(), (size_t)n * sizeof(GPSlot));
+  if (!map[0].empty()) memcpy(img.data() + o_ma, map[0].data(), map[0].size() * sizeof(GMap));
+  if (!map[1].empty()) memcpy(img.data() + o_mb, map[1].data(), map[1].size() * sizeof(GMap));
+  if (!red.empty()) memcpy(img.data() + o_red, red.data(), red.size() * sizeof(SlabRedSlot));
+  hipStream_t s = (hipStream_t)stream;
+  if (memcmp(table_host, img.data(), (size_t)bytes) != 0) {
+    memcpy(table_host, img.data(), (size_t)bytes);
+    if (hipMemcpyAsync(table, table_host, (size_t)bytes, hipMemcpyHostToDevice, s) != hipSuccess ||
+        hipStreamSynchronize(s) != hipSuccess) {
+      memset(table_host, 0, sizeof(GroupHeader));
+      return SVAE_ELAUNCH;
+    }
+  }
+  const char* t = (const char*)table;
+  const GPSlot* tab = (const GPSlot*)(t + o_gp);
+  if (!map[0].empty()) {
+    hipLaunchKernelGGL((gemm256_group_kernel<SVAE_EPI_F32_ACC>), dim3((unsigned)map[0].size()), dim3(512), 0, s, tab,
+                       (const GMap*)(t + o_ma));
+    SVAE_LAUNCH_CHECK();
+  }
+  if (!map[1].empty()) {
+    hipLaunchKernelGGL((gemm256_group_kernel<G3_EPI_SLAB>), dim3((unsigned)map[1].size()), dim3(512), 0, s, tab,
+                       (const GMap*)(t + o_mb));
+    SVAE_LAUNCH_CHECK();
+    const long long rb = std::max(1LL, std::min(2048LL, (red_elems + 255) / 256));
+    hipLaunchKernelGGL(slab_reduce_list_kernel, dim3((unsigned)rb), dim3(256), 0, s, (const SlabRedSlot*)(t + o_red),
+                       (int)red.size());
+    SVAE_LAUNCH_CHECK();
+  }
+  return SVAE_OK;
+}
+
 #ifdef SVAE_STAMPS
 extern "C" __attribute__((visibility("default"))) int svae_debug_stamps(unsigned long long* host) {
   return hipMemcpyFromSymbol(host, HIP_SYMBOL(svae_stamps), sizeof(svae_stamps)) == hipSuccess ? 0 : -1;
diff --git a/sparse-vae_amd/sparse_vae/_native.py b/sparse-vae_amd/sparse_vae/_native.py
--- a/sparse-vae_amd/sparse_vae/_native.py
+++ b/sparse-vae_amd/sparse_vae/_native.py
@@ -61,6 +61,7 @@
     ]
 
 
+GROUP_MAX = 256
 COLSUM_MAX = 8
 LN_MULTI_MAX = 4
 
@@ -83,6 +84,8 @@
 _SIGS = {
     'svae_gemm': [ctypes.POINTER(GemmDesc), c_void_p],
     'svae_gemm_pair': [ctypes.POINTER(GemmDesc), ctypes.POINTER(GemmDesc), c_void_p],
+    'svae_gemm_group_table_bytes': [c_int32],
+    'svae_gemm_group': [ctypes.POINTER(GemmDesc), c_int32, c_int32, c_void_p, c_void_p, c_int64, c_void_p],
     'svae_resid_ln_fwd': [c_void_p, c_void_p, c_int32, c_int64, c_float, c_uint64, c_void_p, c_int32, c_void_p,
                           c_void_p, c_void_p, c_void_p, c_void_p, c_void_p, c_int32, c_int32, c_void_p],
     'svae_layernorm_fwd': [c_void_p, c_int32, c_void_p, c_void_p, c_void_p, c_void_p, c_void_p, c_int32, c_int32,
@@ -186,7 +189,8 @@
         fn.argtypes = argtypes
         fn.restype = {'svae_version': ctypes.c_char_p, 'svae_attn_dq_part_elems': c_int64,
                       'svae_attn_dq_part_elems_w': c_int64, 'svae_attn_fwd_ws_elems': c_int64,
-                      'svae_latent_topk_ws_bytes': c_int64}.get(name, ctypes.c_int)
+                      'svae_latent_topk_ws_bytes': c_int64,
+                      'svae_gemm_group_table_bytes': c_int64}.get(name, ctypes.c_int)
     return lib
 
 
diff --git a/sparse-vae_amd/sparse_vae/engine.py b/sparse-vae_amd/sparse_vae/engine.py
--- a/sparse-vae_amd/sparse_vae/engine.py
+++ b/sparse-vae_amd/sparse_vae/engine.py
@@ -5,7 +5,7 @@
 import torch
 
 from . import kernels as K
-from ._native import COLSUM_MAX, LN_MULTI_MAX, ZPROJ_MAX
+from ._native import COLSUM_MAX, GROUP_MAX, LN_MULTI_MAX, ZPROJ_MAX
 from ._native import EPI_BF16, EPI_F32, EPI_F32_ACC, EPI_GELU, EPI_GELU_BWD, EPI_DROPOUT_RESID, \
     EPI_ROTARY_BF16, EPI_CE_STATS, EPI_F32_ATOMIC, EPI_CE_PROB, EPI_ROWSCALE_GATHER
 
@@ -213,6 +213,11 @@
         self.head_mode = os.environ.get('SVAE_HEAD', 'prob')
         assert self.head_mode in ('prob', 'logits'), self.head_mode
         self.dw_pair = os.environ.get('SVAE_DW_PAIR', '1') != '0'
+        self.dw_group = os.environ.get('SVAE_DW_GROUP', '1') != '0'
+        self._dw_jobs = []
+        self._dwq = None
+        self._dw_names = False
+        self._dwg_states, self._dwg_sched = [], {}
         self.fuse_ln = os.environ.get('SVAE_FUSE_LN', '0') != '0'
         self.delta_fused = os.environ.get('SVAE_DELTA_FUSED', '0') != '0'
         self.o32_mode = os.environ.get('SVAE_ATTN_O32', '0') != '0'
@@ -292,6 +297,9 @@
             off = self.P.offsets[bias][0]
             bg = self.P.grad[off:off + n_out]
         side = self.side if on_side else None
+        if self._dwq is not None and on_side and rows >= K.GROUP_MIN_ROWS:
+            self._dwq.append((dY, X, self.P.g(wname), rows, n_out, n_in, ldy, ldx, bg))
+            return
         if side is None:
             K.linear_dw(dY, X, self.P.g(wname), rows, n_out, n_in, ldy, ldx, bgrad=bg)
             return
@@ -312,7 +320,7 @@
         return 2 if tiles >= ncu and eff(2) > eff(1) + 0.1 else 1
 
     def _dw_pair(self, j0, j1):
-        if self.side is not None or not self.dw_pair:
+        if self._dwq is not None or self.side is not None or not self.dw_pair:
             for j in (j0, j1):
                 self._dw(*j[:6], *(tuple(j[6:]) + (None,) * (9 - len(j))))
             return
@@ -326,6 +334,23 @@
                 bg = self.P.grad[off:off + n_out]
             args.append((dY, X, self.P.g(wname), rows, n_out, n_in, ldy, ldx, bg))
         K.linear_dw_pair(*args)
+
+    def _bname(self, name, st):
+        return f'{name}.{st["tag"]}' if self._dw_names else name
+
+    def flush_dw(self):
+        q, self._dw_jobs = self._dw_jobs, []
+        k = 0
+        for c in range(0, len(q), GROUP_MAX):
+            jobs = q[c:c + GROUP_MAX]
+            key = tuple((j[4], j[5], j[3]) for j in jobs)
+            if key not in self._dwg_sched:
+                self._dwg_sched[key] = K.group_schedule(key, self.ncu)
+            for idx, splits, slab in self._dwg_sched[key]:
+                if len(self._dwg_states) <= k:
+                    self._dwg_states.append(K.DwGroupState(self.P.device))
+                K.linear_dw_group([jobs[i] for i in idx], splits, self._dwg_states[k], slab=slab)
+                k += 1
 
     def join_side(self):
         if self.side is not None:
@@ -458,17 +483,19 @@
         return t if t is not None and t.numel() >= n else self.ws.get('b.dqpart', (n,), f32)
 
     def layer_bwd(self, st, dout, dx_out, *, dx_accumulate=False, dctx=None, g2_ready=False, next_drop=None,
-                  zsplice=None):
+                  zsplice=None, next_st=None):
         d, ws, P = self.d, self.ws, self.P
         pre, B, Sx, L, Lq = st['pre'], st['B'], st['Sx'], st['L'], st['Lq']
         heads, hd = st['heads'], st['hd']
         rows_x, rows_q = B * Sx, st['rows_q']
         rot = self.rot(max(Sx, L), st['window'])
         a = pre + 'attention.'
-        g2 = ws.get('b.g2', (rows_q, d))
+        bn = lambda name: self._bname(name, st)
+        self._dwq = self._dw_jobs if self._dw_names else None
+        g2 = ws.get(bn('b.g2'), (rows_q, d))
         if not g2_ready:
             K.dropout_bwd_cast(dout, g2, st['drop_p'], st['seed'], rows_q, d)
-        dpre = ws.get('b.dpre', (rows_q, 4 * d))
+        dpre = ws.get(bn('b.dpre'), (rows_q, 4 * d))
         K.gemm(g2, P.wT(pre + 'ffn.2.weight', d, 4 * d), dpre, rows_q, 4 * d, d, epi=EPI_GELU_BWD, aux=st['gprime'],
                ldaux=4 * d)
         self._dw_pair((g2, st['f'], pre + 'ffn.2.weight', rows_q, d, 4 * d),
@@ -476,7 +503,7 @@
         dh2 = ws.get('b.dh2', (rows_q, d))
         K.gemm(dpre, P.wT(pre + 'ffn.0.weight', 4 * d, d), dh2, rows_q, d, 4 * d, epi=EPI_BF16)
         dxc = ws.get('b.dxc', (rows_q, d), f32)
-        gxc = ws.get('b.gxc', (rows_q, d))
+        gxc = ws.get(bn('b.gxc'), (rows_q, d))
         self._ln_bwd(pre + 'ffn_layer_norm', dh2, st['ln_f'], rows_q, dout, dxc, gxc)
         dx1, gx1 = dxc, gxc
         if st['cross']:
@@ -486,8 +513,8 @@
             delta = ws.get('b.delta', (B, heads, Lq), f32)
             K.gemm(gxc, P.wT(c + 'output_linear.weight', d, d), dOc, rows_q, d, d, epi=EPI_BF16, delta=delta if self.delta_fused else None,
                    delta_o32=st['Ocx'].get('o32'), ld_o32=d, delta_hd=hd, delta_seq=Lq)
-            dqc = ws.get('b.dqc', (rows_q, d))
-            dkvc = ws.get('b.dkvc', (rows_c, 2 * d))
+            dqc = ws.get(bn('b.dqc'), (rows_q, d))
+            dkvc = ws.get(bn('b.dkvc'), (rows_c, 2 * d))
             K.attention(st['qc'], st['kvc'], st['kvc'][:, d:], st['Oc'], st['lsec'], B=B, H=heads, Lq=Lq, Lk=L,
                         hd=hd, sq=d, bq=Lq * d, sk=2 * d, sv=2 * d, bk=L * 2 * d, bv=L * 2 * d, so=d, bo=Lq * d,
                         key_pad=st['pad_ctx'], causal=False, backward=True, delta_ready=self.delta_fused,
@@ -503,7 +530,7 @@
             dcx = ws.get('b.dcx.' + st['tag'] if st.get('ctx_deferred') else 'b.dcx', (rows_c, d))
             K.gemm(dkvc, P.wT(c + 'k_linear.weight', 2 * d, d), dcx, rows_c, d, 2 * d, epi=EPI_BF16)
             dx1 = ws.get('b.dx1', (rows_q, d), f32)
-            gx1 = ws.get('b.gx1', (rows_q, d))
+            gx1 = ws.get(bn('b.gx1'), (rows_q, d))
             self._ln_bwd(pre + 'cross_attn_layer_norm', dhq, st['ln_cross'], rows_q, dxc, dx1, gx1)
             if st.get('ctx_deferred'):
                 st['dcx'] = dcx
@@ -517,7 +544,7 @@
         if st['learned']:
             kv = st['kv']
             dq32 = ws.get('b.dq32', (B * Lq, d), f32)
-            dkv = ws.get('b.dkv', (rows_x, 2 * d))
+            dkv = ws.get(bn('b.dkv'), (rows_x, 2 * d))
             K.attention(P.w(a + 'learned_queries').view(Lq, d), kv, kv[:, d:], st['O'], st['lse'], B=B, H=heads,
                         Lq=Lq, Lk=Sx, hd=hd, sq=d, bq=0, sk=2 * d, sv=2 * d, bk=Sx * 2 * d, bv=Sx * 2 * d, so=d,
                         bo=Lq * d, key_pad=st['pad_k'], causal=False, backward=True, dout=dO, sdo=d, bdo=Lq * d,
@@ -531,7 +558,7 @@
             K.gemm(dkv, P.wT(a + 'k_linear.weight', 2 * d, d), dh, rows_x, d, 2 * d, epi=EPI_BF16)
         else:
             qkv = st['qkv']
-            dqkv = ws.get('b.dqkv', (rows_x, 3 * d))
+            dqkv = ws.get(bn('b.dqkv'), (rows_x, 3 * d))
             K.attention(qkv, qkv[:, d:], qkv[:, 2 * d:], st['O'], st['lse'], B=B, H=heads, Lq=Lq, Lk=Sx, hd=hd,
                         sq=3 * d, bq=Sx * 3 * d, sk=3 * d, sv=3 * d, bk=Sx * 3 * d, bv=Sx * 3 * d, so=d, bo=Lq * d,
                         key_pad=st['pad_k'], causal=st['causal'], window=st['window'], backward=True, dout=dO,
@@ -545,12 +572,14 @@
             K.gemm(dqkv, P.wT(a + 'q_linear.weight', 3 * d, d), dh, rows_x, d, 3 * d, epi=EPI_BF16)
         if st['resid']:
             self._ln_bwd(pre + 'attn_layer_norm', dh, st['ln_a'], rows_x, dx1, dx_out,
-                         dx_bf=ws.get('b.g2', (rows_x, d)) if next_drop is not None else None, bf_drop=next_drop,
+                         dx_bf=(ws.get(self._bname('b.g2', next_st or st), (rows_x, d)) if next_drop is not None
+                                else None), bf_drop=next_drop,
                          zsplice=zsplice)
             if dx_accumulate:
                 raise NotImplementedError('residual + accumulate is handled by the caller')
         else:
             self._ln_bwd(pre + 'attn_layer_norm', dh, st['ln_a'], rows_x, dx_out if dx_accumulate else None, dx_out)
+        self._dwq = None
 
     def forward(self, ids, ntok, *, pad=True, eps=None, seed=0, kl_weight=1.0, dropout=0.1, need_logits=False):
         hp, d, ws, P = self.hp, self.d, self.ws, self.P
@@ -919,6 +948,8 @@
                 user_ready(end)
         if sv is None:
             raise RuntimeError('backward() without a saved forward')
+        self._dwq, self._dw_jobs = None, []
+        self._dw_names = self.dw_group and user_ready is None and self.side is None
         B, L = sv['B'], sv['L']
         T, V, Z, N = B * L, hp.vocab_size, hp.latent_depth, hp.num_latents
         gs = ws.get('gscale', (2,), f32)
@@ -968,7 +999,7 @@
         top = sv['dec_layers'][-1]
         g2_pre = self.head_g2 and top['rows_q'] == T
         K.gemm(dpre0, P.wT('output_layer.0.weight', d, d), dx, T, d, d, epi=EPI_F32,
-               aux=ws.get('b.g2', (T, d)) if g2_pre else None, ldaux=d if g2_pre else 0,
+               aux=ws.get(self._bname('b.g2', top), (T, d)) if g2_pre else None, ldaux=d if g2_pre else 0,
                drop_p=top['drop_p'] if g2_pre else 0.0, seed=top['seed'] if g2_pre else 0)
         ready(P.end('output_layer.3.bias'))
 
@@ -985,7 +1016,8 @@
                 nd = (nst['drop_p'], nst['seed'], L)
             dzh_i = ws.get('b.dzh_all', (hp.num_layers, B, d), f32)[i] if self.zp_batch else dzh
             zs = (L, dzh_i, None) if st['resid'] and st['rows_q'] == T else None
-            self.layer_bwd(st, dx, dx_prev, g2_ready=g2_ready, next_drop=nd, zsplice=zs)
+            self.layer_bwd(st, dx, dx_prev, g2_ready=g2_ready, next_drop=nd, zsplice=zs,
+                           next_st=sv['dec_layers'][i - 1] if nd is not None else None)
             g2_ready = nd is not None
             wz, bz = f'z_projections.{i}.weight', f'z_projections.{i}.bias'
             if zs is not None and self.zp_batch:
@@ -1032,10 +1064,12 @@
         if st0['resid']:
             tmp = ws.get('b.dfirst', (T, d), f32)
             self.layer_bwd(st0, dcur, tmp)
+            self.flush_dw()
             self.join_side()
             K.embedding_bwd(sv['ids32'], tmp, P.g('input_layer.0.weight'), T, d)
         else:
             self.layer_bwd(st0, dcur, dx_emb, dx_accumulate=True)
+            self.flush_dw()
 
         ready(P.end('encoder.first_layer.ffn_layer_norm.bias'))
         self.join_side()
diff --git a/sparse-vae_amd/sparse_vae/kernels.py b/sparse-vae_amd/sparse_vae/kernels.py
--- a/sparse-vae_amd/sparse_vae/kernels.py
+++ b/sparse-vae_amd/sparse_vae/kernels.py
@@ -144,6 +144,86 @@
                    dict(a_t=True, b_t=True, lda=ldy or n_out, ldb=ldx or n_in, ldc=n_in, epi=N.EPI_F32_ATOMIC,
                         splits=s, a_rowsum=bg, aux=aux)))
     gemm_pair(*gs)
+
+
+GROUP_SLICE_MAX = 16384
+GROUP_MIN_ROWS = 128
+
+
+def group_schedule(shapes, ncu=256):
+    n = len(shapes)
+    tiles = [-(-m // 256) * -(-k // 256) for m, k, _ in shapes]
+    rows = [r for _, _, r in shapes]
+    splits, slab = [0] * n, [True] * n
+    rmax, calls = max(rows), []
+    while True:
+        used, rnd = 0, []
+        for i in range(n):
+            if splits[i] == 0 and rows[i] == rmax and used + tiles[i] <= ncu:
+                rnd.append(i)
+                used += tiles[i]
+        if 4 * used < 3 * ncu:
+            break
+        for i in rnd:
+            splits[i], slab[i] = 1, False
+        calls.append(rnd)
+    rest = [i for i in range(n) if splits[i] == 0]
+    if rest:
+        units = lambda sl: sum(tiles[i] * -(-rows[i] // sl) for i in rest)
+        work = sum(tiles[i] * rows[i] for i in rest)
+        sl = min(GROUP_SLICE_MAX, max(512, -(-work // (ncu * 64)) * 64))
+        while sl < GROUP_SLICE_MAX and units(sl) > ncu:
+            sl += 64
+        for i in rest:
+            s = -(-rows[i] // sl)
+            kchunk = -(-(-(-rows[i] // s)) // 64) * 64
+            splits[i] = -(-rows[i] // kchunk)
+        if calls:
+            calls[-1] = calls[-1] + rest
+        else:
+            calls.append(rest)
+    for c in calls:
+        assert sum(tiles[i] for i in c if not slab[i]) <= ncu, 'a second round of whole-K tiles in one launch'
+    return [(c, [splits[i] for i in c], [slab[i] for i in c]) for c in calls]
+
+
+class DwGroupState:
+
+    def __init__(self, device):
+        self.device, self.n = device, 0
+
+    def ensure(self, n):
+        if n > self.n:
+            self.n = max(n, 2 * self.n)
+            self.bytes = lib.svae_gemm_group_table_bytes(min(self.n, N.GROUP_MAX))
+            self.descs = (N.GemmDesc * self.n)()
+            self.table = torch.empty(self.bytes, dtype=torch.uint8, device=self.device)
+            self.host = ctypes.create_string_buffer(self.bytes)
+
+
+def linear_dw_group(jobs, splits, state, slab=None, max_blocks=0):
+    n = len(jobs)
+    if n == 0:
+        return
+    if n > N.GROUP_MAX:
+        raise RuntimeError(f'linear_dw_group: {n} GEMMs (at most {N.GROUP_MAX})')
+    slab = [s > 1 for s in splits] if slab is None else slab
+    need = sum(s * j[4] * j[5] for j, s, sb in zip(jobs, splits, slab) if sb)
+    ws = _slab_workspace(need, jobs[0][0].device) if need else None
+    state.ensure(n)
+    off = 0
+    for i, (j, s, sb) in enumerate(zip(jobs, splits, slab)):
+        dY, X, Wg, rows, n_out, n_in, ldy, ldx, bg = j
+        aux = None
+        if sb:
+            aux = ws[off:off + s * n_out * n_in]
+            off += s * n_out * n_in
+        elif s != 1:
+            raise RuntimeError('linear_dw_group: a GEMM without a slab has one split')
+        _fill_desc(state.descs[i], dY, X, Wg, n_out, n_in, rows, a_t=True, b_t=True, lda=ldy or n_out, ldb=ldx or n_in,
+                   ldc=n_in, epi=N.EPI_F32_ATOMIC if sb else N.EPI_F32_ACC, splits=s, a_rowsum=bg, aux=aux)
+    check(lib.svae_gemm_group(state.descs, n, max_blocks, state.table.data_ptr(), state.host, state.bytes, stream()),
+          'svae_gemm_group')
 
 
 _slabs = {}
```
